# mozack/vdjer

Measured on AMD Instinct MI355X. Metric: M paired-reads/sec (k-mer build + contig score), IgH 50bp PE, higher is better.
Workload: dtype u8/u64 (2-bit packed bases, integer counts)

## Files before the change

### vdjer_amd/csrc/vdjx_kmer.hip

```cpp
#include "vdjx_common.h"
#include "vdjx_scan.h"
#include "vdjx_part.h"

#include <algorithm>
#include <numeric>
#include <type_traits>
#include <string.h>
#include <stdlib.h>

#define HIST_THREADS 512
#define HIST_BLOCKS 512u
#define LOCAL_SLOTS 2048u
#define K3_SUB_TUPLES g_sub_tuples
__device__ u32 g_sub_tuples = 262144u;
#define NONE32 0xFFFFFFFFu
#define INST_MASK 0x7FFFFFFFu

struct RecView {
	u64 bhi, blo, nm, lq;
};

__device__ inline RecView load_rec(const u64* __restrict__ bases, const u64* __restrict__ nmask,
                                   const u64* __restrict__ lowq, size_t r) {
	RecView v;
	const ulonglong2 b = ((const ulonglong2*) bases)[r];
	v.bhi = b.x; v.blo = b.y;
	v.nm = nmask[r];
	v.lq = lowq ? lowq[r] : 0ull;
	return v;
}

__global__ void k_pick_u32(const u32* __restrict__ src, u32 step, u32 n, u32* __restrict__ out) {
	const u32 i = blockIdx.x * blockDim.x + threadIdx.x;
	if (i < n) out[i] = src[(size_t) i * step];
}

template <typename THI, u32 SLOTS>
__device__ inline int lds_insert(u64* s_klo, THI* s_khi, u64 lo, THI hi, u32 h) {
	const THI EMPTY = (THI) ~(THI) 0, LOCKED = (THI) (EMPTY - 1);
	u32 slot = h & (SLOTS - 1);
	u32 probes = 0;
	while (probes < SLOTS) {
		THI cur = vdjx_peek_acquire(&s_khi[slot]);
		if (cur == EMPTY) {
			THI old = atomicCAS(&s_khi[slot], EMPTY, LOCKED);
			if (old == EMPTY) {
				vdjx_poke(&s_klo[slot], lo);
				vdjx_poke_release(&s_khi[slot], hi);
				return (int) slot;
			}
			cur = old;
			if (cur != LOCKED) cur = vdjx_peek_acquire(&s_khi[slot]);
		}
		if (cur == LOCKED) continue;
		if (cur == hi && vdjx_peek(&s_klo[slot]) == lo) return (int) slot;
		slot = (slot + 1) & (SLOTS - 1);
		probes++;
	}
	return -1;
}

template <typename THI, u32 SLOTS>
__device__ inline int lds_lookup(const u64* s_klo, const THI* s_khi, u64 lo, THI hi, u32 h) {
	const THI EMPTY = (THI) ~(THI) 0;
	u32 slot = h & (SLOTS - 1);
	for (u32 probes = 0; probes < SLOTS; probes++) {
		THI cur = s_khi[slot];
		if (cur == EMPTY) return -1;
		if (cur == hi && s_klo[slot] == lo) return (int) slot;
		slot = (slot + 1) & (SLOTS - 1);
	}
	return -1;
}

#define INST_BITS 38
#define INST_MASK64 ((1ull << INST_BITS) - 1ull)
#define NONE64 0xFFFFFFFFFFFFFFFFull

struct Tup16 {
	u64 lo, x;
	typedef u32 hi_t;
	__device__ inline u64 hi() const { return x >> INST_BITS; }
	__device__ inline u64 inst() const { return x & INST_MASK64; }
	__device__ static inline Tup16 make(u64 lo, u64 hi, u64 inst) { Tup16 t; t.lo = lo; t.x = (hi << INST_BITS) | inst; return t; }
	__device__ static inline Tup16 load(const Tup16* p) { const ulonglong2 v = *(const ulonglong2*) p; Tup16 t; t.lo = v.x; t.x = v.y; return t; }
	__device__ static inline void store(Tup16* p, const Tup16& t) { *(ulonglong2*) p = make_ulonglong2(t.lo, t.x); }
};
struct Tup24 {
	u64 lo, h, i;
	typedef u64 hi_t;
	__device__ inline u64 hi() const { return h; }
	__device__ inline u64 inst() const { return i; }
	__device__ static inline Tup24 make(u64 lo, u64 hi, u64 inst) { Tup24 t; t.lo = lo; t.h = hi; t.i = inst; return t; }
	__device__ static inline Tup24 load(const Tup24* p) { return *p; }
	__device__ static inline void store(Tup24* p, const Tup24& t) { *p = t; }
};

__device__ inline u64 vdjx_clean_offsets(u64 bad, int k, int P) {
	u64 inv = bad;
	int cur = 1;
	while (cur * 2 <= k) { inv |= inv >> cur; cur *= 2; }
	inv |= inv >> (k - cur);
	return ~inv & (P >= 64 ? ~0ull : (1ull << P) - 1ull);
}

#define GL_WAVE_BYTES 3072u

#define GL_ROW_LONG (VDJX_LONG_W + 2)
#define GL_WAVE_BYTES_LONG (64u * GL_ROW_LONG * 8u + 2048u)
struct GateView { u64 bhi, blo, bad; };
__device__ inline GateView load_gate(const u64* __restrict__ bases, const u64* __restrict__ gate, size_t r) {
	GateView v;
	const ulonglong2 b = ((const ulonglong2*) bases)[r];
	v.bhi = b.x; v.blo = b.y;
	v.bad = gate[r];
	return v;
}
__device__ inline vdjx_mask3 load_gate3(const u64* __restrict__ gate, size_t r) {
	vdjx_mask3 b;
	b.w0 = gate[r * VDJX_LONG_M]; b.w1 = gate[r * VDJX_LONG_M + 1]; b.w2 = gate[r * VDJX_LONG_M + 2];
	return b;
}
__device__ inline vdjx_mask3 load_bad3(const u64* __restrict__ nmask, const u64* __restrict__ lowq, size_t r) {
	vdjx_mask3 b;
	b.w0 = nmask[r * VDJX_LONG_M] | (lowq ? lowq[r * VDJX_LONG_M] : 0ull);
	b.w1 = nmask[r * VDJX_LONG_M + 1] | (lowq ? lowq[r * VDJX_LONG_M + 1] : 0ull);
	b.w2 = nmask[r * VDJX_LONG_M + 2] | (lowq ? lowq[r * VDJX_LONG_M + 2] : 0ull);
	return b;
}
__device__ inline void stage_row_long(u64* row, const u64* __restrict__ bases, size_t r) {
#pragma unroll
	for (int w = 0; w < VDJX_LONG_W; w++) row[w] = bases[r * VDJX_LONG_W + w];
	row[VDJX_LONG_W] = 0; row[VDJX_LONG_W + 1] = 0;
}

__device__ inline bool sym_canonical(const ulonglong2 f, int rl, int k, int o, u64& khi, u64& klo) {
	u64 xh, xl, yh, yl;
	vdjx_kmer_at_lane(f.x, f.y, rl, k, o, xh, xl);
	vdjx_kmer_rc(xh, xl, k, yh, yl);
	const bool flip = yh < xh || (yh == xh && yl < xl);
	khi = flip ? yh : xh;
	klo = flip ? yl : xl;
	return flip;
}

template <bool LONG, bool SYM = false>
__global__ __launch_bounds__(HIST_THREADS) void k_gated_hist(const u64* __restrict__ bases, const u64* __restrict__ nmask,
                                                             const u64* __restrict__ lowq, size_t R, int rl, int k, u32 nb_bits,
                                                             size_t rpb, u32* __restrict__ bucket_cnt, u32 dbg_in) {
#ifdef VDJX_ABLATE
	const u32 dbg = dbg_in;
#else
	const u32 dbg = 0u;
#endif
	u32 sink = 0;
	extern __shared__ __attribute__((aligned(16))) u32 hist[];
	const u32 NB = 1u << nb_bits;
	for (u32 i = threadIdx.x; i < NB; i += HIST_THREADS) hist[i] = 0;
	__syncthreads();
	static_assert(!(LONG && SYM), "SYM is the short-read form");
	uint8_t* wv = (uint8_t*) (hist + NB) + (threadIdx.x >> 6) * (LONG ? GL_WAVE_BYTES_LONG : GL_WAVE_BYTES);
	ulonglong2* wb = (ulonglong2*) wv;
	u64* wrow = (u64*) wv;
	uint16_t* wl = (uint16_t*) (wv + (LONG ? 64u * GL_ROW_LONG * 8u : 1024u));
	const u32 lane = threadIdx.x & 63u;
	const size_t r0 = (size_t) blockIdx.x * rpb;
	const size_t r1 = r0 + rpb < R ? r0 + rpb : R;
	const int P = rl - k + 1;
	for (size_t rb = r0; rb < r1; rb += HIST_THREADS) {
		const size_t r = rb + threadIdx.x;
		u64 G = 0;
		vdjx_mask3 bad{~0ull, ~0ull, ~0ull};
		if (r < r1) {
			if (LONG) { bad = load_gate3(lowq, r); stage_row_long(wrow + lane * GL_ROW_LONG, bases, r); }
			else {
				const GateView v = load_gate(bases, lowq, SYM ? 2 * r : r);
				G = vdjx_clean_offsets(v.bad, k, P);
				wb[lane] = make_ulonglong2(v.bhi, v.blo);
			}
		}
		constexpr int LSTEP = 16;
		for (int ob = 0; ob < P; ob += LSTEP) {
			const u32 g = LONG ? vdjx_clean16(bad, ob, k, P) : (u32) (G >> ob) & 0xFFFFu;
			const u32 c = (u32) __popc(g);
			const u32 incl = (u32) vdjx_wave_scan_add((int) c);
			const u32 total = (u32) __builtin_amdgcn_readlane((int) incl, 63);
			if (dbg == 1) { sink += incl; continue; }
			if (!total) continue;
			u32 at = incl - c;
			for (u32 gg = g; gg; gg &= gg - 1) wl[at++] = (uint16_t) ((lane << (LONG ? 8 : 6)) | (u32) (ob + __builtin_ctz(gg)));
			vdjx_wave_lds_fence();
			if (dbg == 2) { sink += wl[lane]; vdjx_wave_lds_fence(); continue; }
			for (u32 i = lane; i < total; i += 64) {
				const u32 e = wl[i];
				u64 khi, klo;
				if (LONG) vdjx_kmer_at_words(wrow + (e >> 8) * GL_ROW_LONG, k, (int) (e & 255u), khi, klo);
				else if (SYM) (void) sym_canonical(wb[e >> 6], rl, k, (int) (e & 63u), khi, klo);
				else {
					const ulonglong2 bb = wb[e >> 6];
					vdjx_kmer_at_lane(bb.x, bb.y, rl, k, (int) (e & 63u), khi, klo);
				}
				if (dbg == 3) { sink += (u32) (vdjx_bucket_mix(klo, khi) >> (64 - nb_bits)); continue; }
				atomicAdd(&hist[(u32) (vdjx_bucket_mix(klo, khi) >> (64 - nb_bits))], 1u);
			}
			vdjx_wave_lds_fence();
		}
	}
	__syncthreads();
	if (dbg) { if (sink == 0x12345u) bucket_cnt[0] = sink; return; }
	for (u32 i = threadIdx.x; i < NB; i += HIST_THREADS) if (hist[i]) atomicAdd(&bucket_cnt[i], hist[i]);
}

template <typename TUP> struct TupBucket {
	u32 shift, mask;
	__device__ inline u32 operator()(const TUP& t) const { return (u32) (vdjx_bucket_mix(t.lo, t.hi()) >> shift) & mask; }
};

#define PARTR_STAGE_BYTES 98304u
template <typename TUP, bool LONG, bool SYM = false>
__global__ __launch_bounds__(PART_THREADS) void k_part_records_g(const u64* __restrict__ bases, const u64* __restrict__ nmask,
                                                                 const u64* __restrict__ lowq, size_t R, u64 rec_base, int rl, int k,
                                                                 u32 shift, u32 nbk, size_t rpb, u32 rr0, u32* __restrict__ gcur,
                                                                 TUP* __restrict__ out) {
	extern __shared__ __attribute__((aligned(16))) uint8_t smem[];
	TUP* stage = (TUP*) smem;
	u32* desc = (u32*) (smem + PARTR_STAGE_BYTES);
	__shared__ part_round pr;
	__shared__ u32 s_n;
	constexpr u32 ROUND = PARTR_STAGE_BYTES / sizeof(TUP);
	constexpr int OB = LONG ? 8 : 6;
	const int P = rl - k + 1;
	const u32 rr_min = ROUND / (u32) P;
	u32 rr = rr0 > rr_min ? rr0 : rr_min;
	const u32 mask = nbk - 1;
	const u32 lane = threadIdx.x & 63u, wave = threadIdx.x >> 6;
	static_assert(!(LONG && SYM), "SYM is the short-read form");
	uint8_t* wv = smem + wave * (LONG ? GL_WAVE_BYTES_LONG : GL_WAVE_BYTES);
	ulonglong2* wb = (ulonglong2*) wv;
	u64* wrow = (u64*) wv;
	uint16_t* wl = (uint16_t*) (wv + (LONG ? 64u * GL_ROW_LONG * 8u : 1024u));
	const size_t r0 = (size_t) blockIdx.x * rpb;
	const size_t r1 = r0 + rpb < R ? r0 + rpb : R;
	size_t rs = r0;
	while (rs < r1) {
		const size_t re = rs + rr < r1 ? rs + rr : r1;
		if (threadIdx.x == 0) s_n = 0;
		pr.begin(nbk);
		for (size_t rb = rs; rb < re; rb += PART_THREADS) {
			const size_t r = rb + threadIdx.x;
			u64 G = 0;
			vdjx_mask3 bad{~0ull, ~0ull, ~0ull};
			if (r < re) {
				if (LONG) { bad = load_gate3(lowq, r); stage_row_long(wrow + lane * GL_ROW_LONG, bases, r); }
				else {
					const GateView v = load_gate(bases, lowq, SYM ? 2 * r : r);
					G = vdjx_clean_offsets(v.bad, k, P);
					wb[lane] = make_ulonglong2(v.bhi, v.blo);
				}
			}
			const u32 loc0 = (u32) (rb - rs) + wave * 64u;
			constexpr int LSTEP = 16;
			for (int ob = 0; ob < P; ob += LSTEP) {
				const u32 g = LONG ? vdjx_clean16(bad, ob, k, P) : (u32) (G >> ob) & 0xFFFFu;
				const u32 c = (u32) __popc(g);
				const u32 incl = (u32) vdjx_wave_scan_add((int) c);
				const u32 total = (u32) __builtin_amdgcn_readlane((int) incl, 63);
				if (!total) continue;
				u32 at = incl - c;
				for (u32 gg = g; gg; gg &= gg - 1) wl[at++] = (uint16_t) ((lane << OB) | (u32) (ob + __builtin_ctz(gg)));
				vdjx_wave_lds_fence();
				u32 dbase = 0;
				if (lane == 0) dbase = atomicAdd(&s_n, total);
				dbase = (u32) __builtin_amdgcn_readlane((int) dbase, 0);
				for (u32 i = lane; i < total; i += 64) {
					const u32 e = wl[i];
					u64 khi, klo;
					if (LONG) vdjx_kmer_at_words(wrow + (e >> 8) * GL_ROW_LONG, k, (int) (e & 255u), khi, klo);
					else if (SYM) (void) sym_canonical(wb[e >> 6], rl, k, (int) (e & 63u), khi, klo);
					else {
						const ulonglong2 bb = wb[e >> 6];
						vdjx_kmer_at_lane(bb.x, bb.y, rl, k, (int) (e & 63u), khi, klo);
					}
					const u32 b = (u32) (vdjx_bucket_mix(klo, khi) >> shift) & mask;
					pr.count(b);
					if (dbase + i < ROUND) desc[dbase + i] = ((loc0 + (e >> OB)) << (OB + 10)) | ((e & ((1u << OB) - 1u)) << 10) | b;
				}
				vdjx_wave_lds_fence();
			}
		}
		__syncthreads();
		if (s_n > ROUND) {
			rr = rr / 2 > rr_min ? rr / 2 : rr_min;
			__syncthreads();
			continue;
		}
		const u32 n = pr.reserve(nbk, gcur);
		for (u32 i = threadIdx.x; i < n; i += PART_THREADS) {
			const u32 d = desc[i];
			const size_t r = rs + (d >> (OB + 10));
			const u32 o = (d >> 10) & ((1u << OB) - 1u);
			u64 khi, klo;
			u64 inst = ((rec_base + (u64) r) << OB) | (u64) o;
			if (LONG) vdjx_kmer_at_words(bases + r * VDJX_LONG_W, k, (int) o, khi, klo);
			else if (SYM) {
				const bool flip = sym_canonical(((const ulonglong2*) bases)[2 * r], rl, k, (int) o, khi, klo);
				inst = flip ? ((rec_base + 2 * (u64) r + 1) << OB) | (u64) (rl - k - (int) o) : ((rec_base + 2 * (u64) r) << OB) | (u64) o;
			} else {
				const ulonglong2 bb = ((const ulonglong2*) bases)[r];
				vdjx_kmer_at_lane(bb.x, bb.y, rl, k, (int) o, khi, klo);
			}
			TUP::store(&stage[pr.slot(d & 1023u)], TUP::make(klo, khi, inst));
		}
		__syncthreads();
		pr.flush(stage, n, out, TupBucket<TUP>{shift, mask});
		rs = re;
	}
}

template <typename TUP>
__global__ __launch_bounds__(512) void k_seg_hist_g(const TUP* __restrict__ in, const u32* __restrict__ seg_start, u32 seg_shift, u32 slices,
                                                    u32 shift, u32 sub_bits, u32* __restrict__ fine_cnt) {
	__shared__ u32 h[PART_MAXB];
	const u32 nbk = 1u << sub_bits;
	for (u32 i = threadIdx.x; i < nbk; i += 512) h[i] = 0;
	__syncthreads();
	size_t t0, t1;
	const u32 seg = part_slice(seg_start, seg_shift, slices, t0, t1);
	for (size_t t = t0 + threadIdx.x; t < t1; t += 512) {
		const TUP x = TUP::load(&in[t]);
		atomicAdd(&h[(u32) (vdjx_bucket_mix(x.lo, x.hi()) >> shift) & (nbk - 1)], 1u);
	}
	__syncthreads();
	for (u32 i = threadIdx.x; i < nbk; i += 512) if (h[i]) atomicAdd(&fine_cnt[((size_t) seg << sub_bits) | i], h[i]);
}

#ifndef RD_THREADS
#define RD_THREADS 768
// ... 535 lines not shown
	__shared__ u32 s_over, s_ndist, s_total, s_ns, s_np, s_sbase, s_pbase;
	__shared__ u32 s_pend[MERGE_SLOTS / 32];
	const THI EMPTY = (THI) ~(THI) 0;
	const u32 b = blockIdx.x;
	const u32 tid = threadIdx.x;
	if (tid == 0) {
		u32 tot = 0;
		for (u32 s = 0; s < G; s++) tot += seg_off[(size_t) s * (NBo + 1) + (b + 1) * MG] - seg_off[(size_t) s * (NBo + 1) + b * MG];
		s_total = tot;
	}
	__syncthreads();
	const u32 total = s_total;
	if (total == 0) return;
	u32 S = 1;
	while ((u64) S * (MERGE_SLOTS * 3 / 4) < total) S <<= 1;
	S *= s_mult;
	if (SYM && S > PS_MAX_SPLIT) { if (tid == 0) atomicAdd(g_err, 1u); return; }
	auto key_of = [&](u32 at, u64& lo, u64& hi, u32& h) {
		if (SYM) { const PartialS q = ((const PartialS*) recv)[at]; lo = q.lo; hi = ps_hi(q); h = ps_h(q); }
		else { const Partial q = recv[at]; lo = q.lo; hi = q.hi; h = q.h; }
	};
	{
		if (tid == 0) { s_over = 0; s_ndist = 0; }
		for (u32 sp = 0; sp < S; sp++) {
			for (u32 i = tid; i < MERGE_SLOTS; i += MERGE_THREADS) { s_khi[i] = EMPTY; s_cg[i] = 0; s_mg[i] = NONE64; s_st[i] = 0; if (SYM) s_mgr[i] = NONE64; }
			__syncthreads();
			for (u32 s = 0; s < G; s++) {
				const u32 off = seg_off[(size_t) s * (NBo + 1) + b * MG], cnt = seg_off[(size_t) s * (NBo + 1) + (b + 1) * MG] - off;
				for (u32 i = tid; i < cnt; i += MERGE_THREADS) {
					u64 lo, hi, fg, fgr = 0;
					u32 h, cg;
					if (SYM) { const PartialS q = ((const PartialS*) recv)[off + i]; lo = q.lo; hi = ps_hi(q); h = ps_h(q); cg = ps_cg(q); fg = ps_fg(q); fgr = q.fgr; }
					else { const Partial q = recv[off + i]; lo = q.lo; hi = q.hi; h = q.h; cg = q.cg; fg = q.fg; }
					if (((h >> 12) & (S - 1)) != sp) continue;
					const int slot = lds_insert<THI, MERGE_SLOTS>(s_klo, s_khi, lo, (THI) hi, h);
					if (slot < 0) { s_over = 1; continue; }
					atomicAdd(&s_cg[slot], cg & ~PART_FLAG);
					atomicMin((unsigned long long*) &s_mg[slot], (unsigned long long) fg);
					if (SYM) atomicMin((unsigned long long*) &s_mgr[slot], (unsigned long long) fgr);
					atomicAdd(&s_st[slot], 1u | ((cg & PART_FLAG) ? MS_FLAG : 0u));
				}
			}
			__syncthreads();
			if (s_over) break;
			if (tid == 0) { s_ns = 0; s_np = 0; }
			for (u32 i = tid; i < MERGE_SLOTS / 32; i += MERGE_THREADS) s_pend[i] = 0;
			__syncthreads();
			for (u32 i0 = 0; i0 < MERGE_SLOTS; i0 += MERGE_THREADS) {
				const u32 i = i0 + tid;
				u32 need = 0, cg = 0;
				bool live = s_khi[i] != EMPTY;
				if (live) {
					cg = s_cg[i];
					atomicAdd(&s_ndist, SYM ? 2u : 1u);
					if (cg < cmin) live = false;
				}
				const u32 st0 = s_st[i];
				if (live && !(st0 >> 16)) {
					if ((st0 & 0xFFFFu) < 2) live = false;
					else need |= NEED_SEQ;
				}
				if (live && cg < tlow) need |= NEED_Q;
				if (live && !need) s_st[i] = atomicAdd(&s_ns, SYM ? 2u : 1u);
				else s_st[i] = NONE32;
				if (live && need) {
					s_st[i] = atomicAdd(&s_np, 1u) | (need << 30);
					const u32 hm = rd_hash(s_klo[i], (u64) s_khi[i]) & (MERGE_SLOTS - 1);
					atomicOr(&s_pend[hm >> 5], 1u << (hm & 31));
				}
			}
			__syncthreads();
			if (tid == 0) {
				s_sbase = s_ns ? atomicAdd(so.n, s_ns) : 0;
				s_pbase = s_np ? atomicAdd(po.n, s_np) : 0;
			}
			__syncthreads();
			for (u32 i0 = 0; i0 < MERGE_SLOTS; i0 += MERGE_THREADS) {
				const u32 i = i0 + tid;
				const u32 st = s_st[i];
				if (st != NONE32 && !(st >> 30)) {
					const u32 pos = s_sbase + st;
					if (pos < so.cap) {
						const u32 cg = s_cg[i];
						so.lo[pos] = s_klo[i]; so.hi[pos] = (u64) s_khi[i];
						so.gcnt[pos] = cg > CNT_CAP ? CNT_CAP : cg; so.gfirst[pos] = s_mg[i];
					}
					if (SYM && pos + 1 < so.cap) {
						const u32 cg = s_cg[i];
						u64 rh, rlo;
						vdjx_kmer_rc((u64) s_khi[i], s_klo[i], k, rh, rlo);
						so.lo[pos + 1] = rlo; so.hi[pos + 1] = rh;
						so.gcnt[pos + 1] = cg > CNT_CAP ? CNT_CAP : cg; so.gfirst[pos + 1] = s_mgr[i];
					}
				} else if (st != NONE32) {
					const u32 need = st >> 30;
					const u32 pid = s_pbase + (st & PID_MASK);
					if (pid < po.cap) {
						po.lo[pid] = s_klo[i]; po.hi[pid] = (u64) s_khi[i];
						po.cg[pid] = s_cg[i]; po.mg[pid] = s_mg[i];
						if (SYM) po.mgr[pid] = s_mgr[i];
						po.need[pid] = need;
					}
					s_st[i] = pid | (need << 30);
				}
			}
			__syncthreads();
			for (u32 s = 0; s < G; s++) {
				const u32 off = seg_off[(size_t) s * (NBo + 1) + b * MG], cnt = seg_off[(size_t) s * (NBo + 1) + (b + 1) * MG] - off;
				if (tid == 0) s_ns = 0;
				__syncthreads();
				u32 mine = 0;
				for (u32 i = tid; i < cnt; i += MERGE_THREADS) {
					u64 lo, hi;
					u32 h;
					key_of(off + i, lo, hi, h);
					if (((h >> 12) & (S - 1)) != sp) continue;
					if (!((s_pend[(h & (MERGE_SLOTS - 1)) >> 5] >> (h & 31)) & 1u)) continue;
					const int slot = lds_lookup<THI, MERGE_SLOTS>(s_klo, s_khi, lo, (THI) hi, h);
					if (slot >= 0 && ms_open(s_st[slot])) mine++;
				}
				if (mine) atomicAdd(&s_ns, mine);
				__syncthreads();
				if (tid == 0) { s_sbase = s_ns ? atomicAdd(&g_nq[s], s_ns) : 0; s_np = 0; }
				__syncthreads();
				if (s_ns) {
					for (u32 i = tid; i < cnt; i += MERGE_THREADS) {
						u64 lo, hi;
						u32 h;
						key_of(off + i, lo, hi, h);
						if (((h >> 12) & (S - 1)) != sp) continue;
						if (!((s_pend[(h & (MERGE_SLOTS - 1)) >> 5] >> (h & 31)) & 1u)) continue;
						const int slot = lds_lookup<THI, MERGE_SLOTS>(s_klo, s_khi, lo, (THI) hi, h);
						if (slot < 0) continue;
						const u32 pid = s_st[slot];
						if (ms_open(pid)) queries[src_base[s] + s_sbase + atomicAdd(&s_np, 1u)] = make_uint2(off + i - src_base[s], pid);
					}
				}
				__syncthreads();
			}
			__syncthreads();
		}
		if (s_over && tid == 0) atomicAdd(g_err, 1u);
	}
	if (tid == 0) atomicAdd(g_distinct, (u64) s_ndist);
}

#define REPLY_Q0 80
#define REPLY_R0 240
#define REPLY_RQ0 248
template <bool SYM>
__global__ __launch_bounds__(64) void k_shard_reply(const uint2* __restrict__ queries, u32 nq, const u32* __restrict__ owner_off, u32 G,
                                                    const Partial* __restrict__ dense, const u32* __restrict__ dense_ref,
                                                    const u32* __restrict__ dstart, u32 NBo, const u64* __restrict__ low_inst,
                                                    const u64* __restrict__ bases, const u64* __restrict__ nmask,
                                                    vdjx_qrows quals, u64 rec_base, const u32* __restrict__ scan, u32 n_local, int k, int rl, int ob,
                                                    uint8_t* __restrict__ replies) {
	const u32 qi = blockIdx.x;
	if (qi >= nq) return;
	const u32 lane = threadIdx.x;
	u32 o = 0;
	while (o + 1 < G && owner_off[o + 1] <= qi) o++;
	const uint2 q = queries[qi];
	const u32 di = dstart[(size_t) o * NBo] + q.x;
	u64 finst, finst_r = 0;
	u32 p_cg;
	if (SYM) { const PartialS p = ((const PartialS*) dense)[di]; finst = ps_fg(p); finst_r = p.fgr; p_cg = ps_cg(p); }
	else { const Partial p = dense[di]; finst = p.fg; p_cg = p.cg; }
	const u32 need = q.y >> 30;
	const u32 om = (1u << ob) - 1u;
	auto local_rec = [&](u64 inst) -> u64 {
		if (!scan) return (inst >> ob) - rec_base;
		const u32 g = (u32) (inst >> ob);
		u32 lo = 0, hi = n_local;
		while (lo + 1 < hi) { const u32 mid = lo + ((hi - lo) >> 1); if (scan[mid] <= g) lo = mid; else hi = mid; }
		return lo;
	};
	const u64 frec = local_rec(finst);
	const u32 foff = (u32) finst & om;
	const u64 finst_local = (frec << ob) | foff;
	const u64 frec_r = SYM ? local_rec(finst_r) : 0;
	const u32 foff_r = (u32) finst_r & om;
	const u64 finst_r_local = (frec_r << ob) | foff_r;
	uint8_t* out = replies + (size_t) qi * REPLY_BYTES;
	if (lane == 0) {
		((u32*) out)[0] = q.y;
		((u32*) out)[1] = 0;
		((u64*) out)[1] = finst;
		if (SYM) ((u64*) out)[REPLY_R0 / 8] = finst_r;
	}
	if (!SYM && lane < (REPLY_BYTES - REPLY_R0) / 4) ((u32*) (out + REPLY_R0))[lane] = 0;
	if (lane < 8) {
		const int W = rl <= VDJX_SHORT_READ_LEN ? 2 : VDJX_LONG_W, M = rl <= VDJX_SHORT_READ_LEN ? 1 : VDJX_LONG_M;
		((u64*) out)[2 + lane] = (int) lane < W ? bases[frec * W + lane] : ((int) lane < W + M ? nmask[frec * M + (lane - W)] : 0ull);
	}
	if ((int) lane >= k) return;
	u32 acc = 0, acc_r = 0;
	const u32 ref = dense_ref[di];
	if ((need & NEED_Q) && ref != NONE32) {
		const u32 cg = p_cg & ~PART_FLAG;
		for (u32 i = 0; i < cg; i++) {
			const u64 inst = low_inst[ref + i];
			if (inst != (scan ? finst_local : finst)) acc += (u32) (uint8_t) (quals.row((inst >> ob) - rec_base)[((u32) inst & om) + lane] - 33);
			if (SYM) {
				const u64 m = vdjx_inst_mirror(inst, ob, rl, k);
				if (m != (scan ? finst_r_local : finst_r)) acc_r += (u32) (uint8_t) (quals.row((m >> ob) - rec_base)[((u32) m & om) + lane] - 33);
			}
		}
	}
	const uint8_t* fr = quals.row(frec);
	out[REPLY_Q0 + lane] = (uint8_t) (acc > 255u ? 255u : acc);
	out[REPLY_Q0 + REPLY_KQ + lane] = (uint8_t) (fr[foff + lane] - 33);
	out[REPLY_Q0 + 2 * REPLY_KQ + lane] = (uint8_t) (fr[lane] - 33);
	if (SYM) {
		const uint8_t* frr = quals.row(frec_r);
		out[REPLY_RQ0 + lane] = (uint8_t) (acc_r > 255u ? 255u : acc_r);
		out[REPLY_RQ0 + REPLY_KQ + lane] = (uint8_t) (frr[foff_r + lane] - 33);
		out[REPLY_RQ0 + 2 * REPLY_KQ + lane] = (uint8_t) (frr[lane] - 33);
	}
}

__global__ void k_resolve_first(const uint8_t* __restrict__ replies, u32 nr, const u64* __restrict__ p_mg, u32* __restrict__ p_r0,
                                const u64* __restrict__ p_mgr, u32 np) {
	const u32 r = blockIdx.x * blockDim.x + threadIdx.x;
	if (r >= nr) return;
	const uint8_t* me = replies + (size_t) r * REPLY_BYTES;
	const u32 pid = ((const u32*) me)[0] & PID_MASK;
	if (((const u64*) me)[1] == p_mg[pid]) p_r0[pid] = r;
	if (p_mgr && ((const u64*) me)[REPLY_R0 / 8] == p_mgr[pid]) p_r0[np + pid] = r;
}

__global__ __launch_bounds__(256) void k_resolve_add(const uint8_t* __restrict__ replies, u32 nr, const u32* __restrict__ p_r0, int k, u32* __restrict__ p_fl,
                                                     u32* __restrict__ p_S, u32 np) {
	const u32 r = blockIdx.x * 4u + (threadIdx.x >> 6);
	const u32 lane = threadIdx.x & 63u;
	if (r >= nr) return;
	const uint8_t* me = replies + (size_t) r * REPLY_BYTES;
	const u32 w0 = ((const u32*) me)[0];
	const u32 pid = w0 & PID_MASK, need = w0 >> 30;
	const u32 r0 = p_r0[pid];
	if (r0 == NONE32) return;
	if ((need & NEED_SEQ) && r != r0 && lane == 0) {
		const u64* a = (const u64*) me;
		const u64* b = (const u64*) (replies + (size_t) r0 * REPLY_BYTES);
		u64 d = 0;
#pragma unroll
		for (int w = 2; w < 10; w++) d |= a[w] ^ b[w];
		if (d) p_fl[pid] = 1;
	}
	if ((need & NEED_Q) && (int) lane < k) {
		const uint8_t* first = me + REPLY_Q0 + (r == r0 ? 2 * REPLY_KQ : REPLY_KQ);
		atomicAdd(&p_S[(size_t) pid * 64 + lane], (u32) me[REPLY_Q0 + lane] + (u32) first[lane]);
		if (np) {
			const uint8_t* first_r = me + REPLY_RQ0 + (r == p_r0[np + pid] ? 2 * REPLY_KQ : REPLY_KQ);
			atomicAdd(&p_S[((size_t) np + pid) * 64 + lane], (u32) me[REPLY_RQ0 + lane] + (u32) first_r[lane]);
		}
	}
}

template <bool SYM>
__global__ void k_resolve_keep(PendOut po, u32 np, const u32* __restrict__ p_fl, const u32* __restrict__ p_S, int k, u32 mf, u32 mqq, u32 tlow,
                               SurvOutG so) {
	const u32 p = blockIdx.x * blockDim.x + threadIdx.x;
	const bool in = p < np;
	const u32 need = in ? po.need[p] : 0u;
	bool keep = in && ((need & NEED_SEQ) ? p_fl[p] != 0 : true);
	const u32 cg = in ? po.cg[p] : 0u;
	const u32 cgc = cg > CNT_CAP ? CNT_CAP : cg;
	keep = keep && cgc >= mf;
	bool keep_r = keep;
	if (keep && cg < tlow) {
		for (int j = 0; j < k; j++) if (p_S[(size_t) p * 64 + j] < mqq) { keep = false; break; }
		if (SYM) for (int j = 0; j < k; j++) if (p_S[((size_t) np + p) * 64 + j] < mqq) { keep_r = false; break; }
	}
	if (!SYM) {
		const u32 pos = vdjx_wave_inc(so.n, keep);
		if (keep && pos < so.cap) {
			so.lo[pos] = po.lo[p]; so.hi[pos] = po.hi[p];
			so.gcnt[pos] = cgc; so.gfirst[pos] = po.mg[p];
		}
		return;
	}
	const bool any = keep || keep_r;
	const u32 pos = vdjx_wave_inc(so.n, any, 2u);
	if (any && pos + 1 < so.cap) {
		so.lo[pos] = po.lo[p]; so.hi[pos] = po.hi[p];
		so.gcnt[pos] = cgc | (keep ? 0u : GC_SHADOW); so.gfirst[pos] = po.mg[p];
		u64 rh, rlo;
		vdjx_kmer_rc(po.hi[p], po.lo[p], k, rh, rlo);
		so.lo[pos + 1] = rlo; so.hi[pos + 1] = rh;
		so.gcnt[pos + 1] = cgc | (keep_r ? 0u : GC_SHADOW); so.gfirst[pos + 1] = po.mgr[p];
	}
}

__global__ void k_first_to_scan(u64* __restrict__ a, size_t na, u64* __restrict__ b, size_t nb, const u32* __restrict__ scan, int ob) {
	const size_t i = (size_t) blockIdx.x * blockDim.x + threadIdx.x;
	if (i >= na + nb) return;
	u64* p = i < na ? a + i : b + (i - na);
	const u64 v = *p;
	if (v != NONE64) *p = ((u64) scan[v >> ob] << ob) | (v & ((1ull << ob) - 1ull));
}

__global__ void k_node_flags(const u64* __restrict__ s_lo, const u64* __restrict__ s_hi, u32 n, int k,
                             const u32* __restrict__ vbits, const u32* __restrict__ jbits,
                             uint8_t* __restrict__ has_v, uint8_t* __restrict__ has_j) {
	u32 i = blockIdx.x * blockDim.x + threadIdx.x;
	if (i >= n) return;
	if (k <= 16) { has_v[i] = 1; has_j[i] = 1; return; }
	u128 key = ((u128) s_hi[i] << 64) | s_lo[i];
	u32 code = (u32) (key >> (2 * (k - 16)));
	has_v[i] = code ? (vbits[code >> 5] >> (code & 31)) & 1u : 0;
	has_j[i] = code ? (jbits[code >> 5] >> (code & 31)) & 1u : 0;
}


#define IT_INST_BITS 35
#define IT_INST_MASK ((1ull << IT_INST_BITS) - 1ull)
#define IT_SURV_SHIFT 38
#define IT_HOLE 0xFFFFFFFFFFFFFFFFull
#define WALK_THREADS 256

#define SLOT_HI_BITS 36
#define SLOT_HI_MASK ((1ull << SLOT_HI_BITS) - 1ull)
struct SurvTable { const ulonglong2* slots; u32 mask; const ulonglong2* skey; const u32* bloom; u32 bloom_mask; };

struct ItemFmt {
	u32 pmask;
	u32 len_shift;
	u32 maxlen;
	u32 mul, inv;
	u32 bmask;
	u32 ns;
};
__device__ inline u32 it_surv(const ItemFmt& f, u64 x) { return (u32) (x >> IT_SURV_SHIFT) & f.pmask; }
__device__ inline u32 it_len(const ItemFmt& f, u64 x) { return f.maxlen > 1 ? (u32) (x >> f.len_shift) + 1u : 1u; }
__device__ inline u32 it_scat(const ItemFmt& f, u32 p) { return ((((p >> 4) * f.mul) & f.bmask) << 4) | (p & 15u); }

__global__ void k_surv_table2(const u64* __restrict__ s_lo, const u64* __restrict__ s_hi, u32 n, ulonglong2* __restrict__ slots, u32 mask,
                              ulonglong2* __restrict__ skey, u32* __restrict__ bloom, u32 bloom_mask) {
	const u32 i = blockIdx.x * blockDim.x + threadIdx.x;
	if (i >= n) return;
	const u64 lo = s_lo[i], hi = s_hi[i];
	skey[i] = make_ulonglong2(lo, hi);
	const u64 h = vdjx_mix(lo, hi);
	{
		const u32 bit = (u32) (h >> 40) & bloom_mask;
		atomicOr(&bloom[bit >> 5], 1u << (bit & 31));
	}
	u32 slot = (u32) (h >> 20) & mask;
	const unsigned long long entry = hi | ((unsigned long long) (i + 1) << SLOT_HI_BITS);
	while (atomicCAS((unsigned long long*) &slots[slot].y, 0ull, entry) != 0ull) slot = (slot + 1) & mask;
	slots[slot].x = lo;
}

__device__ inline int surv_lookup2f(const SurvTable& t, u64 lo, u64 hi);

__device__ inline int surv_lookup2(const SurvTable& t, u64 lo, u64 hi) {
	u32 slot = (u32) (vdjx_mix(lo, hi) >> 20) & t.mask;
	for (;;) {
		const ulonglong2 v = t.slots[slot];
		if (!v.y) return -1;
		if (v.x == lo && (v.y & SLOT_HI_MASK) == hi) return (int) (v.y >> SLOT_HI_BITS) - 1;
		slot = (slot + 1) & t.mask;
	}
}

__device__ inline int surv_lookup2f(const SurvTable& t, u64 lo, u64 hi) {
	const u64 h = vdjx_mix(lo, hi);
	const u32 bit = (u32) (h >> 40) & t.bloom_mask;
	if (!((t.bloom[bit >> 5] >> (bit & 31)) & 1u)) return -1;
	return surv_lookup2(t, lo, hi);
}

__global__ void k_succ_links2(SurvTable t, u32 n, int k, const u32* __restrict__ gcnt, u32* __restrict__ succ, unsigned long long* __restrict__ pred,
                              u32* __restrict__ bestsucc) {
	const u32 u = blockIdx.x * blockDim.x + threadIdx.x;
	if (u >= n) return;
	const ulonglong2 kk = t.skey[u];
	const u128 base = (((u128) kk.y << 64) | kk.x) << 2;
	const u128 km = k < 64 ? (((u128) 1) << (2 * k)) - 1 : ~(u128) 0;
	const int sh = 2 * (k - 1);
	const u32 fb = (u32) (sh < 64 ? kk.x >> sh : kk.y >> (sh - 64)) & 3u;
	const unsigned long long mine = ((unsigned long long) (gcnt[u] & GC_MASK) << 32) | ((unsigned long long) (fb ^ 1u) << 30) | (unsigned long long) u;
	u32 best = NONE32, best_g = 0;
	for (u32 b = 0; b < 4; b++) {
		const u128 key = (base | (u128) b) & km;
		const int s = surv_lookup2(t, (u64) key, (u64) (key >> 64));
		succ[u * 4 + b] = s >= 0 ? (u32) s : NONE32;
		if (s >= 0 && (u32) s != u) {
			const u32 g = gcnt[s] & GC_MASK;
			if (best == NONE32 || g >= best_g) { best = (u32) s; best_g = g; }
			atomicMax(&pred[s], mine);
		}
	}
	bestsucc[u] = best;
}

#define CHAIN_JUMPS 31
__global__ void k_chain_init(const unsigned long long* __restrict__ pred, const u32* __restrict__ bestsucc, u32 n, u64* __restrict__ pd) {
	const u32 v = blockIdx.x * blockDim.x + threadIdx.x;
	if (v >= n) return;
	const unsigned long long x = pred[v];
	const u32 u = (u32) x & 0x3FFFFFFFu;
	pd[v] = x != 0ull && bestsucc[u] == v ? ((u64) u << 32) | 1ull : ((u64) NONE32 << 32);
}

__global__ void k_partner(SurvTable t, u32 n, int k, u32* __restrict__ partner) {
	const u32 p = blockIdx.x * blockDim.x + threadIdx.x;
	if (p >= n) return;
	const ulonglong2 kk = t.skey[p];
	u64 rh, rlo;
	vdjx_kmer_rc(kk.y, kk.x, k, rh, rlo);
	const int q = surv_lookup2(t, rlo, rh);
	partner[p] = q >= 0 ? (u32) q : NONE32;
}
__global__ void k_partner_check(const u32* __restrict__ partner, const u64* __restrict__ linw, u32 n, u32* __restrict__ bad) {
	const u32 p = blockIdx.x * blockDim.x + threadIdx.x;
	if (p >= n) return;
	bool wrong = partner[p] == NONE32;
	const bool linked = (linw[p >> 4] >> (15u - (p & 15u))) & 1ull;
	if (!wrong && linked && (p + 1 >= n || partner[p + 1] != partner[p] - 1u)) wrong = true;
	const u64 m = __ballot(wrong);
	if (m && __lane_id() == 0) atomicAdd(bad, (u32) __popcll(m));
}

__global__ void k_chain_jump(u64* __restrict__ pd, u32 n, const u32* __restrict__ open_prev, u32* __restrict__ open_now) {
	if (open_prev && *open_prev == 0) return;
	const u32 v = blockIdx.x * blockDim.x + threadIdx.x;
	bool open = false;
	if (v < n) {
		u64 x = __atomic_load_n(&pd[v], __ATOMIC_RELAXED);
		for (int it = 0; it < CHAIN_JUMPS; it++) {
			const u32 p = (u32) (x >> 32);
			if (p == NONE32) break;
			const u64 y = __atomic_load_n(&pd[p], __ATOMIC_RELAXED);
			const u32 pp = (u32) (y >> 32);
			if (pp == NONE32) break;
			x = ((u64) pp << 32) | (u64) ((u32) x + (u32) y);
			__atomic_store_n(&pd[v], x, __ATOMIC_RELAXED);
			open = true;
		}
	}
	if (__ballot(open) && __lane_id() == 0) atomicAdd(open_now, 1u);
}

__device__ inline void chain_of(const u64* pd, u32 v, u32& head, u32& dist) {
	const u64 x = pd[v];
	const u32 p = (u32) (x >> 32);
	head = v; dist = 0;
	if (p == NONE32) return;
	if ((u32) (pd[p] >> 32) != NONE32) return;
	head = p; dist = (u32) x;
}
__global__ void k_chain_len(const u64* __restrict__ pd, u32 n, u32* __restrict__ len) {
	const u32 v = blockIdx.x * blockDim.x + threadIdx.x;
	if (v >= n) return;
	u32 h, d;
	chain_of(pd, v, h, d);
	atomicAdd(&len[h], 1u);
}

__global__ void k_chain_place(const u64* __restrict__ pd, const u32* __restrict__ off, u32 n, u32* __restrict__ newidx) {
	const u32 v = blockIdx.x * blockDim.x + threadIdx.x;
	if (v >= n) return;
	u32 h, d;
	chain_of(pd, v, h, d);
	newidx[v] = off[h] + d;
}
__global__ void k_chain_permute(const u32* __restrict__ newidx, u32 n, const u64* __restrict__ lo, const u64* __restrict__ hi, const u32* __restrict__ gcnt,
                                const u64* __restrict__ gfirst, const u32* __restrict__ succ, u64* __restrict__ lo2, u64* __restrict__ hi2,
                                u32* __restrict__ gcnt2, u64* __restrict__ gfirst2, ulonglong2* __restrict__ skey2, u32* __restrict__ succ2) {
	const u32 v = blockIdx.x * blockDim.x + threadIdx.x;
	if (v >= n) return;
	const u32 q = newidx[v];
	const u64 l = lo[v], h = hi[v];
	lo2[q] = l; hi2[q] = h; gcnt2[q] = gcnt[v]; gfirst2[q] = gfirst[v];
	skey2[q] = make_ulonglong2(l, h);
	const uint4 s = *(const uint4*) &succ[(size_t) v * 4];
	uint4 r;
	r.x = s.x == NONE32 ? NONE32 : newidx[s.x];
	r.y = s.y == NONE32 ? NONE32 : newidx[s.y];
	r.z = s.z == NONE32 ? NONE32 : newidx[s.z];
	r.w = s.w == NONE32 ? NONE32 : newidx[s.w];
	*(uint4*) &succ2[(size_t) q * 4] = r;
}
__global__ void k_table_remap(ulonglong2* __restrict__ slots, u32 n_slots, const u32* __restrict__ newidx) {
	const u32 i = blockIdx.x * blockDim.x + threadIdx.x;
	if (i >= n_slots) return;
	const u64 y = slots[i].y;
	if (!y) return;
	slots[i].y = (y & SLOT_HI_MASK) | ((u64) (newidx[(u32) (y >> SLOT_HI_BITS) - 1] + 1u) << SLOT_HI_BITS);
}

__global__ void k_chain_words(const u32* __restrict__ succ, const ulonglong2* __restrict__ skey, u32 n, int k, u64* __restrict__ linw, u32* __restrict__ fbw,
                              const u32* __restrict__ partner) {
	const u32 p = blockIdx.x * blockDim.x + threadIdx.x;
	const u32 j = p & 15u;
	u64 w = 0;
	u32 fb = 0;
	if (p < n) {
		const uint4 s = *(const uint4*) &succ[(size_t) p * 4];
		const u32 sv[4] = {s.x, s.y, s.z, s.w};
		const bool mirrored = !partner || (p + 1 < n && partner[p] != NONE32 && partner[p + 1] == partner[p] - 1u);
		for (u32 b = 0; b < 4; b++) if (sv[b] != NONE32) {
			if (sv[b] == p + 1 && mirrored) w |= (1ull << (15u - j)) | ((u64) b << (32u + 2u * (15u - j)));
			else w |= 1ull << (31u - j);
		}
		const ulonglong2 kk = skey[p];
		const int sh = 2 * (k - 1);
		fb = (u32) (sh < 64 ? kk.x >> sh : kk.y >> (sh - 64)) & 3u;
	}
	u32 fw = fb << (2 * j);
	for (int d = 1; d < 16; d <<= 1) {
		w |= ((u64) (u32) __shfl_xor((int) (w >> 32), d) << 32) | (u32) __shfl_xor((int) (u32) w, d);
		fw |= (u32) __shfl_xor((int) fw, d);
	}
	if (j == 0 && p < n) { linw[p >> 4] = w; fbw[p >> 4] = fw; }
}

struct WalkRecS {
	u64 bhi, blo; int rl;
	__device__ inline void kmer_u(int k, int o, u64& hi, u64& lo) const { vdjx_kmer_at(bhi, blo, rl, k, o, hi, lo); }
	__device__ inline void kmer_l(int k, int o, u64& hi, u64& lo) const { vdjx_kmer_at_lane(bhi, blo, rl, k, o, hi, lo); }
	__device__ inline u32 bases16(int bi) const {
		const int sh = 2 * (rl - 16 - bi);
		const u32 rw_dn = vdjx_bits_at_lane(bhi, blo, (u32) (sh > 0 ? sh : 0));
		const u32 up = (u32) (sh < 0 ? -sh : 0);
		return (rw_dn << (up & 31u)) & (0u - (u32) (up < 32u));
	}
	__device__ inline u32 base(int i) const { return vdjx_base_at_lane(bhi, blo, rl, i); }
};
struct WalkRecL {
	const u64* row;
	__device__ inline void kmer_u(int k, int o, u64& hi, u64& lo) const { vdjx_kmer_at_words(row, k, o, hi, lo); }
	__device__ inline void kmer_l(int k, int o, u64& hi, u64& lo) const { vdjx_kmer_at_words(row, k, o, hi, lo); }
	__device__ inline u32 bases16(int bi) const { return vdjx_bases16_words(row, bi); }
	__device__ inline u32 base(int i) const { return vdjx_base_words(row, i); }
};
__device__ inline bool wm_test(u64 m, int i) { return (m >> i) & 1ull; }
__device__ inline bool wm_test(const vdjx_mask3& m, int i) { return m.test(i); }
__device__ inline void wm_set(u64& m, int i) { m |= 1ull << i; }
__device__ inline void wm_set(vdjx_mask3& m, int i) { m.set(i); }
__device__ inline int wm_next(u64 m, int from, int none) { const u64 x = from < 64 ? m & (~0ull << from) : 0ull; return x ? __builtin_ctzll(x) : none; }
__device__ inline int wm_next(const vdjx_mask3& m, int from, int none) { return m.next(from, none); }
__device__ inline u32 wm_slice32(u64 m, int from) { return from < 64 ? (u32) (m >> from) : 0u; }
__device__ inline u32 wm_slice32(const vdjx_mask3& m, int from) { return (u32) m.slice(from); }

template <bool LONG, bool SYM = false>
__global__ __launch_bounds__(WALK_THREADS) void k_walk_items(const u64* __restrict__ bases, const u64* __restrict__ nmask, size_t R, int rl, int ob_bits, int k,
                                                             SurvTable t, const u32* __restrict__ succ, const u64* __restrict__ linw, ItemFmt f,
                                                             u32 range_shift, u32 n_ranges,
                                                             u64* __restrict__ raw, u64 raw_cap, u32 blk_items,
                                                             unsigned long long* __restrict__ g_cursor,
                                                             u32* __restrict__ range_cnt, u32* __restrict__ g_err, u32 dbg_in,
                                                             const u32* __restrict__ partner) {
	static_assert(!(LONG && SYM), "SYM is the short-read form");
#ifdef VDJX_ABLATE
	const u32 dbg = dbg_in;
#else
	(void) dbg_in;
	constexpr u32 dbg = 0u;
#endif
	extern __shared__ u32 hist[];
	typedef typename std::conditional<LONG, vdjx_mask3, u64>::type MaskT;
	typedef typename std::conditional<LONG, WalkRecL, WalkRecS>::type RecT;
	for (u32 i = threadIdx.x; i < n_ranges; i += WALK_THREADS) hist[i] = 0;
	__syncthreads();
	u64* myrow = (u64*) (hist + ((n_ranges + 1u) & ~1u)) + threadIdx.x * GL_ROW_LONG;
	const int P = rl - k + 1;
	const size_t per = ((R + gridDim.x - 1) / gridDim.x + WALK_THREADS - 1) / WALK_THREADS * WALK_THREADS;
	const size_t r0 = (size_t) blockIdx.x * per;
	const size_t r1 = r0 + per < R ? r0 + per : R;
	const int lane = __lane_id();
	u64 blk = 0;
	u32 fill = blk_items;
#ifdef WALK_STATS
	u32 st_rows = 0, st_rounds = 0, st_filter = 0, st_lookup = 0, st_items = 0, st_chain = 0;
#define WST(x) x
#else
#define WST(x)
#endif
	bool have_blk = false, dead = false;
	__shared__ u64 dq[WALK_THREADS / 64][128];
	__shared__ ulonglong2 dq_b[LONG ? 1 : WALK_THREADS / 64][LONG ? 1 : 128];
	__shared__ u64 dq_v[LONG ? 1 : WALK_THREADS / 64][LONG ? 1 : 128];
	const u32 wq = threadIdx.x >> 6;
	u32 qn = 0;
	auto walk_row = [&](auto fresh_tag, const size_t r, const bool live, const int o_from, const ulonglong2 qb, const u64 qv) {
		constexpr bool FRESH = decltype(fresh_tag)::value;
		RecT v;
		MaskT V{};
		if constexpr (LONG) {
			v.row = myrow;
			if (live) {
				stage_row_long(myrow, bases, r);
				const vdjx_mask3 nm = load_bad3(nmask, nullptr, r);
				for (int o16 = 0; o16 < P; o16 += 16) {
					const u64 g = (u64) vdjx_clean16(nm, o16, k, P) << (o16 & 63);
					if ((o16 >> 6) == 0) V.w0 |= g; else if ((o16 >> 6) == 1) V.w1 |= g; else V.w2 |= g;
				}
			} else
				for (int w = 0; w < GL_ROW_LONG; w++) myrow[w] = 0;
		} else {
			v.bhi = v.blo = 0; v.rl = rl;
			if (!FRESH) { if (live) { v.bhi = qb.x; v.blo = qb.y; V = qv; } }
			else if (live) {
				const RecView rv = load_rec(bases, nmask, nullptr, r);
				v.bhi = rv.bhi; v.blo = rv.blo;
				u64 inv = rv.nm;
				int cur = 1;
				while (cur * 2 <= k) { inv |= inv >> cur; cur *= 2; }
				inv |= inv >> (k - cur);
				V = ~inv & (P >= 64 ? ~0ull : (1ull << P) - 1ull);
			}
		}
		int o = wm_next(V, o_from, P);
		int s = -1;
		u32 in = 0;
		bool first = FRESH, have_c = false;
		MaskT C{};
		WST(st_rows++;)
		while (__ballot(o < P)) {
			WST(st_rounds++;)
			bool need = o < P && s < 0;
			if (FRESH) {
				const bool later = need && !first;
				const u64 lm = __ballot(later);
				if (lm) {
					if (later) {
						const u32 qi = qn + (u32) __popcll(lm & ((1ull << lane) - 1ull));
						dq[wq][qi] = ((u64) r << 8) | (u64) (u32) o;
						if constexpr (!LONG) { dq_b[wq][qi] = make_ulonglong2(v.bhi, v.blo); dq_v[wq][qi] = V; }
						o = P; need = false;
					}
					qn += (u32) __popcll(lm);
				}
			}
			WST(if (__ballot(need)) st_lookup++;)
			if (!FRESH && __ballot(need && !first && !have_c)) {
				WST(st_filter++;)
				const bool mine = need && !first && !have_c;
				for (int ob = 0; ob < P; ob += 4) {
					u32 wv[4], bt[4];
#pragma unroll
					for (int j = 0; j < 4; j++) {
						const int oo = ob + j;
						wv[j] = 0; bt[j] = 0;
						if (mine && oo >= o && oo < P && wm_test(V, oo)) {
							u64 khi, klo;
							v.kmer_u(k, oo, khi, klo);
							const u32 bit = (u32) (vdjx_mix(klo, khi) >> 40) & t.bloom_mask;
							bt[j] = bit & 31u;
							wv[j] = (dbg & 8u) ? 0xFFFFFFFFu : t.bloom[bit >> 5];
						}
					}
#pragma unroll
					for (int j = 0; j < 4; j++) if ((wv[j] >> bt[j]) & 1u) wm_set(C, ob + j);
				}
				if (mine) have_c = true;
			}
			if (need) {
				bool filtered = false;
				if (!first) {
					o = wm_next(C, o, P);
					filtered = true;
				}
				first = false;
				if (o < P) {
					u64 khi, klo;
					v.kmer_l(k, o, khi, klo);
					if (dbg & 8u) s = (klo & 3u) ? (int) ((u32) vdjx_mix(klo, khi) % f.ns) : -1;
					else s = (filtered || (dbg & 16u)) ? surv_lookup2(t, klo, khi) : surv_lookup2f(t, klo, khi);
					in = 0;
					if (s < 0) o++;
				}
			}
			const bool act = o < P && s >= 0;
			WST(if (__ballot(act)) st_chain++;)
			u32 rem = 0, pp = 0, po = 0;
			if (act) {
				const u32 a = (u32) s & 15u;
				const u64 w0 = linw[(u32) s >> 4], w1 = linw[((u32) s >> 4) + 1];
				const u32 lw = (((((u32) w0 & 0xFFFFu) << 16) | ((u32) w1 & 0xFFFFu)) << a) >> 16;
				const u32 ow = ((((u32) w0 & 0xFFFF0000u) | ((u32) w1 >> 16)) << a) >> 16;
				const u32 bw = (u32) (((((w0 >> 32) << 32) | (w1 >> 32)) << (2 * a)) >> 32);
				const u32 rw = v.bases16(o + k);
				const u32 x = bw ^ rw;
				const u32 nl = ~lw & 0xFFFFu;
				const u32 m_base = x ? (u32) __builtin_clz(x) >> 1 : 16u;
				const u32 m_lin = nl ? (u32) __builtin_clz(nl) - 16u : 16u;
				const u32 nv = ~wm_slice32(V, o + 1);
				const u32 m_valid = nv ? (u32) __builtin_ctz(nv) : 32u;
				u32 steps = m_base < m_lin ? m_base : m_lin;
				steps = steps < m_valid ? steps : m_valid;
				const bool capped = steps >= 16u;
				if (capped) steps = 15u;
				rem = steps + 1u; pp = (u32) s; po = (u32) o;
				const int o2 = o + (int) rem;
				int s2 = -1;
				if (o2 < P && wm_test(V, o2)) {
					if (capped) s2 = s + 16;
					else if ((ow >> (15u - steps)) & 1u) {
						const u32 bb = v.base(o2 + k - 1);
						const u32 nx = succ[((u32) s + steps) * 4u + bb];
						s2 = nx == NONE32 ? -1 : (int) nx;
					}
				}
				o = s2 >= 0 || o2 >= P ? o2 : o2 + 1;
				s = s2;
			}
			const u32 pin0 = in;
			if (act) in = s >= 0 ? (4u | v.base(o - 1)) : 0u;
			const u32 run_len = rem, run_pp = pp, run_po = po;
			u32 q_last = 0;
			if (SYM && act) q_last = partner[run_pp];
			auto emit = [&](auto mir_tag, u32 rem_, u32 pp_, u32 po_, u32 pin_, const size_t rec_) {
				constexpr bool MIR = decltype(mir_tag)::value;
				while (__ballot(rem_ > 0)) {
					WST(st_items++;)
					const bool close = rem_ > 0;
					u32 len = 16u - (pp_ & 15u);
					len = len < rem_ ? len : rem_;
					len = len < f.maxlen ? len : f.maxlen;
					const u64 item = (f.maxlen > 1 ? (u64) (len - 1) << f.len_shift : 0ull) | ((u64) pp_ << IT_SURV_SHIFT) | ((u64) pin_ << 35) | ((u64) rec_ << ob_bits) | (u64) po_;
					const u64 m = __ballot(close);
					const u32 cnt = (u32) __popcll(m);
					if (fill + cnt > blk_items) {
						if (have_blk) for (u32 i = fill + (u32) lane; i < blk_items; i += 64) raw[blk + i] = IT_HOLE;
						unsigned long long nb = 0;
						if (lane == 0) nb = atomicAdd(g_cursor, (unsigned long long) blk_items);
						nb = ((unsigned long long) (u32) __builtin_amdgcn_readlane((int) (nb >> 32), 0) << 32) | (u32) __builtin_amdgcn_readlane((int) nb, 0);
						if (nb + blk_items > raw_cap) { if (lane == 0 && !dead) atomicAdd(g_err, 1u); dead = true; have_blk = false; }
						else { blk = nb; have_blk = true; }
						fill = 0;
					}
					if (close && !dead) {
						if (!(dbg & 1u)) raw[blk + fill + (u32) __popcll(m & ((1ull << lane) - 1ull))] = item;
						if (!(dbg & 2u)) atomicAdd(&hist[it_scat(f, pp_) >> range_shift], 1u);
					}
					fill += cnt;
					if (close) {
						rem_ -= len; pp_ += len; po_ += len;
						pin_ = 4u | (MIR ? (v.base(rl - (int) po_) ^ 1u) : v.base((int) po_ - 1));
					}
				}
			};
			emit(std::false_type{}, rem, pp, po, pin0, r);
			if constexpr (SYM) {
				u32 mrem = 0, mpp = 0, mpo = 0, mpin = 0;
				if (act) {
					if (q_last == NONE32 || q_last + 1u < run_len) { if (!dead) atomicAdd(g_err + 2, 1u); }
					else {
						mrem = run_len; mpp = q_last - (run_len - 1u);
						mpo = (u32) (rl - k) - (run_po + run_len - 1u);
						mpin = s >= 0 ? (4u | (v.base(rl - (int) mpo) ^ 1u)) : 0u;
					}
				}
				emit(std::true_type{}, mrem, mpp, mpo, mpin, r + 1);
			}
		}
	};
	auto walk_queued = [&](u32 take) {
		vdjx_wave_lds_fence();
		const bool live = (u32) lane < take;
		const u64 e = live ? dq[wq][qn - take + (u32) lane] : 0ull;
		ulonglong2 qb = make_ulonglong2(0ull, 0ull);
		u64 qv = 0;
		if constexpr (!LONG) if (live) { qb = dq_b[wq][qn - take + (u32) lane]; qv = dq_v[wq][qn - take + (u32) lane]; }
		vdjx_wave_lds_fence();
		qn -= take;
		walk_row(std::false_type{}, (size_t) (e >> 8), live, (int) (e & 255u), qb, qv);
	};
	for (size_t rb = r0; rb < r1; rb += WALK_THREADS) {
		const size_t r = rb + threadIdx.x;
		walk_row(std::true_type{}, SYM ? 2 * r : r, r < r1, 0, make_ulonglong2(0ull, 0ull), 0ull);
		while (qn >= 64) walk_queued(64);
	}
	if (qn) walk_queued(qn);
	if (have_blk) for (u32 i = fill + (u32) lane; i < blk_items; i += 64) raw[blk + i] = IT_HOLE;
#ifdef WALK_STATS
	if ((dbg & 32u) && lane == 0) {
		atomicAdd(&g_cursor[1], (unsigned long long) st_rows); atomicAdd(&g_cursor[2], (unsigned long long) st_rounds); atomicAdd(&g_cursor[3], (unsigned long long) st_filter);
		atomicAdd(&g_cursor[4], (unsigned long long) st_lookup); atomicAdd(&g_cursor[5], (unsigned long long) st_chain); atomicAdd(&g_cursor[6], (unsigned long long) st_items);
	}
#endif
	__syncthreads();
	for (u32 i = threadIdx.x; i < n_ranges; i += WALK_THREADS) if (hist[i]) atomicAdd(&range_cnt[i], hist[i]);
}

static_assert(IT_HOLE == PART_HOLE, "the holes of the walk's blocks are what the partition drops");
struct ItemRange {
	ItemFmt f;
	u32 range_shift, mask;
	__device__ inline u32 operator()(u64 x) const { return (it_scat(f, it_surv(f, x)) >> range_shift) & mask; }
};

#define RC_THREADS 1024
#define RC_UNR 4
template <typename IT> struct RcNone;
template <> struct RcNone<u32> { static constexpr u32 v = 0xFFFFFFFFu; };
template <> struct RcNone<u64> { static constexpr u64 v = 0xFFFFFFFFFFFFFFFFull; };
__device__ inline void rc_min(u32* p, u32 v) { atomicMin(p, v); }
__device__ inline void rc_min(u64* p, u64 v) { atomicMin((unsigned long long*) p, (unsigned long long) v); }

#define RC_CS 17u
#define RC_MS 77u
__device__ inline u32 rc_win(u32 k, u32 s) { return 31u + ((0x261B0E00u >> (8u * k)) & 0xFFu) + s - 1u; }
template <u32 SB, typename IT>
__global__ __launch_bounds__(RC_THREADS) void k_recount(const u64* __restrict__ items, const u32* __restrict__ range_start, ItemFmt f, u32 ns, u64 rec_base, int ob,
                                                        const u32* __restrict__ fbw, u32* __restrict__ ucnt, u64* __restrict__ ufirst, u64* __restrict__ in_first,
                                                        unsigned long long* __restrict__ n_inst) {
	__shared__ u32 c[SB / 16 * RC_CS];
	__shared__ IT mv[SB / 16 * RC_MS];
	__shared__ IT ef[SB * 4];
	__shared__ u32 fbl[SB / 16];
	__shared__ unsigned long long tot;
	constexpr IT NONE = RcNone<IT>::v;
	const u32 b = blockIdx.x;
	const u32 s0 = b * SB;
	const u32 nb = (ns + 15u) >> 4;
	for (u32 i = threadIdx.x; i < SB / 16 * RC_CS; i += RC_THREADS) c[i] = 0;
	for (u32 i = threadIdx.x; i < SB / 16 * RC_MS; i += RC_THREADS) mv[i] = NONE;
	for (u32 i = threadIdx.x; i < SB * 4; i += RC_THREADS) ef[i] = NONE;
	for (u32 i = threadIdx.x; i < SB / 16; i += RC_THREADS) {
		const u32 sb = (s0 >> 4) + i;
		const u32 blk = (sb * f.inv) & f.bmask;
		fbl[i] = sb <= f.bmask && blk < nb ? fbw[blk] : 0u;
	}
	if (threadIdx.x == 0) tot = 0;
	__syncthreads();
	const u32 i0 = range_start[b], i1 = range_start[b + 1];
	const u32 iend = i0 + (i1 - i0 + RC_THREADS * RC_UNR - 1) / (RC_THREADS * RC_UNR) * (RC_THREADS * RC_UNR);
	for (u32 ib = i0 + threadIdx.x; ib < iend; ib += RC_THREADS * RC_UNR) {
		u64 xs[RC_UNR];
#pragma unroll
		for (int u = 0; u < RC_UNR; u++) { const u32 i = ib + (u32) u * RC_THREADS; xs[u] = i < i1 ? items[i] : IT_HOLE; }
#pragma unroll
		for (int u = 0; u < RC_UNR; u++) {
			const u64 x = xs[u];
			const bool live = x != IT_HOLE;
			const u32 p = it_surv(f, x);
			const u32 len = live ? it_len(f, x) : 1u;
			const u32 sl = live ? it_scat(f, p) - s0 : 0u;
			const u32 a = sl & 15u, e = a + len - 1u;
			const u64 inst = x & IT_INST_MASK;
			const bool shaped = live && (a == 0u || e == 15u);
			const u32 cb = (sl >> 4) * RC_CS, mb = (sl >> 4) * RC_MS;
			const u32 slot = mb + (a == 0u ? e : 15u + a);
			const IT val = (IT) (inst + 15u - a);
			bool mine = shaped;
			const u64 act = __ballot(shaped);
			if (act) {
				const int leader = __ffsll((long long) act) - 1;
				const u32 lslot = (u32) __builtin_amdgcn_readlane((int) slot, leader);
				const bool same = shaped && slot == lslot;
				const u64 m = __ballot(same);
				if (__popcll(m) >= 8) {
					const u64 v64 = inst + 15u - a;
					const u32 hi_min = vdjx_wave_min(same ? (u32) (v64 >> 32) : 0xFFFFFFFFu);
					const u32 lo_min = vdjx_wave_min(same && (u32) (v64 >> 32) == hi_min ? (u32) v64 : 0xFFFFFFFFu);
					if (__lane_id() == leader) {
						const u32 n = (u32) __popcll(m);
						atomicAdd(&c[cb + e], n);
						if (a) atomicAdd(&c[cb + a - 1u], 0u - n);
						rc_min(&mv[lslot], (IT) (((u64) hi_min << 32) | lo_min));
					}
					mine = shaped && !same;
				}
			}
			if (live && (mine || !shaped)) {
				atomicAdd(&c[cb + e], 1u);
				if (a) atomicAdd(&c[cb + a - 1u], 0xFFFFFFFFu);
			}
			if (mine) rc_min(&mv[slot], val);
			if (live && !shaped) {
				const u32 k = 31u - (u32) __builtin_clz(len), w = 1u << k;
				rc_min(&mv[mb + rc_win(k, a)], val);
				if (len != w) rc_min(&mv[mb + rc_win(k, e + 1u - w)], val);
			}
			if (live && ((x >> 37) & 1ull)) {
				IT* ep = &ef[sl * 4 + (u32) ((x >> 35) & 3ull)];
				if (vdjx_peek(ep) > (IT) inst) rc_min(ep, (IT) inst);
			}
		}
	}
	__syncthreads();
	const u64 add = rec_base << ob;
	u32 my_cnt = 0;
	for (u32 i = threadIdx.x; i < SB; i += RC_THREADS) {
		const u32 sb = (s0 + i) >> 4;
		const u32 blk = (sb * f.inv) & f.bmask;
		const u32 x = i & 15u, p = (blk << 4) | x;
		if (sb > f.bmask || blk >= nb || p >= ns) continue;
		const u32 cbase = (i >> 4) * RC_CS, mbase = (i >> 4) * RC_MS;
		u32 cc = 0;
		IT mm = NONE;
		IT me = NONE;
		for (u32 e = x; e < 16; e++) { cc += c[cbase + e]; const IT t = mv[mbase + e]; mm = t < mm ? t : mm; if (x) me = t < me ? t : me; }
		for (u32 a = 1; a <= x; a++) { const IT t = mv[mbase + 15 + a]; mm = t < mm ? t : mm; if (a < x) me = t < me ? t : me; }
#pragma unroll
		for (u32 k = 0; k < 4; k++) {
			const u32 w = 1u << k;
			const u32 lo = x >= w ? x - w + 1u : 1u, hi = x < 15u - w ? x : 15u - w;
			for (u32 s = lo ? lo : 1u; s <= hi; s++) { const IT t = mv[mbase + rc_win(k, s)]; mm = t < mm ? t : mm; if (s < x) me = t < me ? t : me; }
		}
		my_cnt += cc;
		ucnt[p] = cc;
		ufirst[p] = mm == NONE ? NONE64 : (u64) mm - 15u + x + add;
		IT e4[4] = {ef[i * 4], ef[i * 4 + 1], ef[i * 4 + 2], ef[i * 4 + 3]};
		if (x && me != NONE) {
			const u32 pa = (fbl[i >> 4] >> (2 * (x - 1))) & 3u;
			const IT t = (IT) (me - 15u + x);
			if (t < e4[pa]) e4[pa] = t;
		}
		for (u32 q = 0; q < 4; q++) in_first[(size_t) p * 4 + q] = e4[q] == NONE ? NONE64 : (u64) e4[q] + add;
	}
	if (my_cnt) atomicAdd(&tot, (unsigned long long) my_cnt);
	__syncthreads();
	if (threadIdx.x == 0 && tot) atomicAdd(n_inst, tot);
}

__global__ void k_count_unseen(const u64* __restrict__ ufirst, u32 n, u32* __restrict__ out) {
	const u32 i = blockIdx.x * blockDim.x + threadIdx.x;
	const bool un = i < n && ufirst[i] == NONE64;
	const u64 m = __ballot(un);
	if (m && __lane_id() == 0) atomicAdd(out, (u32) __popcll(m));
}

__global__ void k_edges_from_in(SurvTable t, u32 n, int k, const u64* __restrict__ in_first, u32* __restrict__ in_from,
                                u64* __restrict__ edge_first, u32* __restrict__ edge_to) {
	const u32 e = blockIdx.x * blockDim.x + threadIdx.x;
	if (e >= n * 4u) return;
	const u64 fs = in_first[e];
	if (fs == NONE64) { in_from[e] = NONE32; return; }
	const u32 v = e >> 2, a = e & 3u;
	const ulonglong2 kk = t.skey[v];
	const u128 kv = ((u128) kk.y << 64) | kk.x;
	const u128 ku = (kv >> 2) | ((u128) a << (2 * (k - 1)));
	const int u = surv_lookup2(t, (u64) ku, (u64) (ku >> 64));
	in_from[e] = u >= 0 ? (u32) u : NONE32;
	if (u >= 0) {
		const u32 oe = (u32) u * 4u + ((u32) kk.x & 3u);
		edge_first[oe] = fs;
		edge_to[oe] = v;
	}
}

struct SurvRec { u64 lo, hi; u32 gcnt, pad; u64 gfirst; };

__global__ void k_surv_pack(const u64* __restrict__ lo, const u64* __restrict__ hi, const u32* __restrict__ gcnt,
                            const u64* __restrict__ gfirst, u32 n, SurvRec* __restrict__ out) {
	u32 i = blockIdx.x * blockDim.x + threadIdx.x;
	if (i >= n) return;
	SurvRec r{lo[i], hi[i], gcnt[i], 0u, gfirst[i]};
	out[i] = r;
}

__global__ void k_surv_unpack(const SurvRec* __restrict__ in, u32 n, u64* __restrict__ lo, u64* __restrict__ hi, u32* __restrict__ gcnt,
                              u64* __restrict__ gfirst, u32* __restrict__ n_real) {
	u32 i = blockIdx.x * blockDim.x + threadIdx.x;
	const bool in_range = i < n;
	SurvRec r{0, 0, GC_SHADOW, 0, 0};
	if (in_range) {
		r = in[i];
		lo[i] = r.lo; hi[i] = r.hi; gcnt[i] = r.gcnt; gfirst[i] = r.gfirst;
	}
	(void) vdjx_wave_inc(n_real, in_range && !(r.gcnt & GC_SHADOW));
}

struct NodeOut {
	u64* first_inst; u32* gcnt; u32* freq; uint8_t* hv; uint8_t* hj; u64* klo; u64* khi; char* kmers;
	uint8_t* to_deg; u32* to_ids; uint8_t* from_deg; u32* from_ids;
};

__global__ void k_rank_keys(const u64* __restrict__ ufirst, const u32* __restrict__ gcnt, u32 n, u64* __restrict__ key, u32* __restrict__ idx) {
	const u32 i = blockIdx.x * blockDim.x + threadIdx.x;
	if (i < n) { key[i] = (gcnt[i] & GC_SHADOW) ? NONE64 : ufirst[i]; idx[i] = i; }
}
__global__ void k_rank_scatter(const u64* __restrict__ key, const u32* __restrict__ idx, u32 n, u32* __restrict__ rank) {
	const u32 j = blockIdx.x * blockDim.x + threadIdx.x;
	if (j >= n) return;
	const u32 i = idx[j];
	rank[i] = key[j] == NONE64 ? i : j;
}

__global__ __launch_bounds__(256) void k_root_count(const uint8_t* __restrict__ from_deg, u32 n, u32* __restrict__ block_cnt) {
	__shared__ u32 cnt;
	if (threadIdx.x == 0) cnt = 0;
	__syncthreads();
	const u32 i = blockIdx.x * 256 + threadIdx.x;
	const bool r = i < n && from_deg[i] == 0;
	const u64 b = __ballot(r);
	if ((threadIdx.x & 63) == 0 && b) atomicAdd(&cnt, (u32) __popcll(b));
	__syncthreads();
	if (threadIdx.x == 0) block_cnt[blockIdx.x] = cnt;
}

__global__ __launch_bounds__(256) void k_root_list(const uint8_t* __restrict__ from_deg, u32 n, const u32* __restrict__ block_start,
                                                   u32* __restrict__ roots) {
	__shared__ u32 wave_cnt[4];
	const u32 i = blockIdx.x * 256 + threadIdx.x;
	const bool r = i < n && from_deg[i] == 0;
	const u64 b = __ballot(r);
	const u32 w = threadIdx.x >> 6, lane = threadIdx.x & 63;
	if (lane == 0) wave_cnt[w] = (u32) __popcll(b);
	__syncthreads();
	u32 base = block_start[blockIdx.x];
	for (u32 j = 0; j < w; j++) base += wave_cnt[j];
	if (r) roots[base + (u32) __popcll(b & ((1ull << lane) - 1))] = i;
}

__device__ inline void sort4_desc64(u64 (&f)[4], u32 (&id)[4]) {
#define CSW(a, b) { const bool sw = kk[a] < kk[b]; if (sw) { u64 t = kk[a]; kk[a] = kk[b]; kk[b] = t; u32 u = id[a]; id[a] = id[b]; id[b] = u; } }
	u64 kk[4];
	for (int i = 0; i < 4; i++) kk[i] = f[i] == NONE64 ? 0ull : f[i] + 1;
	CSW(0, 1) CSW(2, 3) CSW(0, 2) CSW(1, 3) CSW(1, 2)
	for (int i = 0; i < 4; i++) f[i] = kk[i] ? kk[i] - 1 : NONE64;
#undef CSW
}

__global__ void k_node_emit2(const u64* __restrict__ s_lo, const u64* __restrict__ s_hi, const u32* __restrict__ s_gcnt,
                             const u32* __restrict__ s_ucnt, const u64* __restrict__ s_ufirst, const uint8_t* __restrict__ hv,
                             const uint8_t* __restrict__ hj, const u32* __restrict__ rank, const u64* __restrict__ edge_first,
                             const u32* __restrict__ edge_to, const u64* __restrict__ in_first, const u32* __restrict__ in_from,
                             u32 n, int k, NodeOut o) {
	const u32 s = blockIdx.x * blockDim.x + threadIdx.x;
	if (s >= n) return;
	if (s_gcnt[s] & GC_SHADOW) return;
	const u32 r = rank[s];
	o.first_inst[r] = s_ufirst[s];
	o.gcnt[r] = s_gcnt[s];
	o.freq[r] = s_ucnt[s] > 32765u ? 32765u : s_ucnt[s];
	o.hv[r] = hv[s];
	o.hj[r] = hj[s];
	const u128 key = ((u128) s_hi[s] << 64) | s_lo[s];
	for (int j = 0; j < k; j++) {
		const u32 b = (u32) (key >> (2 * (k - 1 - j))) & 3u;
		o.kmers[(size_t) r * k + j] = b == 0 ? 'A' : (b == 1 ? 'T' : (b == 2 ? 'C' : 'G'));
	}
	u64 f[4];
	u32 id[4];
	for (int e = 0; e < 4; e++) {
		f[e] = edge_first[(size_t) s * 4 + e];
		if (f[e] != NONE64 && (s_gcnt[edge_to[(size_t) s * 4 + e]] & GC_SHADOW)) f[e] = NONE64;
		id[e] = f[e] != NONE64 ? rank[edge_to[(size_t) s * 4 + e]] + 1 : 0;
	}
	sort4_desc64(f, id);
	u32 deg = 0;
	for (int e = 0; e < 4; e++) { o.to_ids[(size_t) r * 4 + e] = f[e] != NONE64 ? id[e] : 0; deg += f[e] != NONE64; }
	o.to_deg[r] = (uint8_t) deg;
	for (int e = 0; e < 4; e++) {
		f[e] = in_first[(size_t) s * 4 + e];
		if (f[e] != NONE64 && (in_from[(size_t) s * 4 + e] == NONE32 || (s_gcnt[in_from[(size_t) s * 4 + e]] & GC_SHADOW))) f[e] = NONE64;
		id[e] = f[e] != NONE64 ? rank[in_from[(size_t) s * 4 + e]] + 1 : 0;
	}
	sort4_desc64(f, id);
	deg = 0;
	for (int e = 0; e < 4; e++) { o.from_ids[(size_t) r * 4 + e] = f[e] != NONE64 ? id[e] : 0; deg += f[e] != NONE64; }
	o.from_deg[r] = (uint8_t) deg;
}

namespace {

struct PersistAlloc {
	vdjx_ctx* c;
	explicit PersistAlloc(vdjx_ctx* ctx) : c(ctx) {}
	template <typename T> hipError_t alloc(T** out, size_t n) {
		*out = (T*) c->shard_arena.alloc((n ? n : 1) * sizeof(T));
		return *out ? hipSuccess : hipErrorOutOfMemory;
	}
	vdjx_arena::mark_t mark() const { return c->shard_arena.mark(); }
	void release_to(vdjx_arena::mark_t m) { c->shard_arena.release_to(m); }
};

struct PoolView { const u64* bases; const u64* nmask; vdjx_qrows quals; int rl; int ob; };

template <typename TUP> struct GTuples {
	TUP* t = nullptr;
	u32* bucket_start = nullptr;
	u32 NB = 0, N = 0;
};

struct SurvivorsG {
	u64 *lo = nullptr, *hi = nullptr, *gfirst = nullptr, *ufirst = nullptr;
	u32 *gcnt = nullptr, *ucnt = nullptr;
	u32 n = 0, n_real = 0;
	u64 ndist = 0;
};

inline u32 ceil_log2_u64(u64 x) { u32 b = 0; while ((1ull << b) < x) b++; return b; }

static bool sync_debug() { static const bool on = vdjx_env_set("VDJX_SYNC_DEBUG"); return on; }
static void dbg_sync(vdjx_ctx* c, const char* what) {
	if (!sync_debug()) return;
	const hipError_t e = hipStreamSynchronize(c->stream);
	fprintf(stderr, "[vdjx] %s: %s\n", what, hipGetErrorString(e));
}

struct GatedHist { u32 HB = 0, NBH = 0, N = 0; u32* hstart = nullptr; bool sym = false; };
static bool build_sym(const vdjx_pool* pool, int k) {
	return pool->sym && pool->W == 2 && (k & 1) && pool->n_records % 2 == 0;
}
static bool sym_walk_wanted() { static const bool on = !vdjx_env_set("VDJX_NO_SYM_WALK"); return on; }
static size_t gated_bucket_default() { static const size_t v = (size_t) vdjx_env_num("VDJX_GATED_BUCKET", 3072, 1, 1ll << 32); return v; }
template <typename A>
int stage_gated_hist(vdjx_ctx* c, A& db, const vdjx_pool* pool, int k, size_t per_bucket, u64 geometry_instances, GatedHist* gh, bool sym = false) {
	hipStream_t st = c->stream;
	const size_t R = sym ? pool->n_records / 2 : pool->n_records;
	const int P = pool->rl - k + 1;
	const u64 NI = geometry_instances ? geometry_instances : (u64) R * (u64) P;
	const size_t per = per_bucket ? per_bucket : gated_bucket_default();
	const u32 hb_max = pool->W > 2 ? 14u : 15u;
	u32 HB = ceil_log2_u64((NI + per - 1) / per);
	HB = std::max(8u, std::min(hb_max, HB));
	const u32 NBH = 1u << HB;
#ifdef VDJX_ABLATE
	static const u32 hist_dbg = (u32) vdjx_env_num("VDJX_HIST_DBG", 0, 0, 4);
#else
	constexpr u32 hist_dbg = 0;
#endif
	u32 nblk = (u32) std::min<size_t>(HIST_BLOCKS, (R + 4095) / 4096);
	if (nblk == 0) nblk = 1;
	size_t rpb = (R + nblk - 1) / nblk;
	u32 *hcnt, *hstart;
	HIP_TRY(db.alloc(&hcnt, NBH));
	HIP_TRY(db.alloc(&hstart, NBH + 1));
	HIP_TRY(hipMemsetAsync(hcnt, 0, (size_t) NBH * 4, st));
	const bool lng = pool->W > 2;
	const size_t lds_hist = (size_t) NBH * 4 + (HIST_THREADS / 64) * (lng ? GL_WAVE_BYTES_LONG : GL_WAVE_BYTES);
	HIP_TRY(hipFuncSetAttribute((const void*) k_gated_hist<false>, hipFuncAttributeMaxDynamicSharedMemorySize, (int) lds_hist));
	HIP_TRY(hipFuncSetAttribute((const void*) k_gated_hist<true>, hipFuncAttributeMaxDynamicSharedMemorySize, (int) lds_hist));
	HIP_TRY(hipFuncSetAttribute((const void*) k_gated_hist<false, true>, hipFuncAttributeMaxDynamicSharedMemorySize, (int) lds_hist));
	{
		vdjx_prof_scope ps(c, "k_gated_hist");
		if (lng) hipLaunchKernelGGL(k_gated_hist<true>, dim3(nblk), dim3(HIST_THREADS), lds_hist, st, pool->d_bases, pool->d_nmask, pool->d_lowq, R, pool->rl, k, HB, rpb, hcnt, hist_dbg);
		else if (sym) hipLaunchKernelGGL((k_gated_hist<false, true>), dim3(nblk), dim3(HIST_THREADS), lds_hist, st, pool->d_bases, pool->d_nmask, pool->d_lowq, R, pool->rl, k, HB, rpb, hcnt, hist_dbg);
		else hipLaunchKernelGGL(k_gated_hist<false>, dim3(nblk), dim3(HIST_THREADS), lds_hist, st, pool->d_bases, pool->d_nmask, pool->d_lowq, R, pool->rl, k, HB, rpb, hcnt, hist_dbg);
	}
	dbg_sync(c, "k_gated_hist");
	vdjx_scan_one(st, hcnt, NBH, hstart);
	HIP_TRY(hipMemcpyAsync(c->h_pin, hstart + NBH, 4, hipMemcpyDeviceToHost, st));
	HIP_TRY(hipStreamSynchronize(st));
	HIP_TRY(hipGetLastError());
#ifdef VDJX_ABLATE
	if (hist_dbg) return VDJX_ESTATE;
#endif
	const u32 N = *(const u32*) c->h_pin;
	c->stats["gated_instances"] = sym ? 2ull * N : N;
	gh->HB = HB; gh->NBH = NBH; gh->N = N; gh->hstart = hstart; gh->sym = sym;
	return VDJX_OK;
}

template <typename TUP, typename A>
int stage_gated_cut(vdjx_ctx* c, A& db, const vdjx_pool* pool, u64 rec_base, int k, size_t per_bucket, u64 geometry_instances, const GatedHist& gh, GTuples<TUP>* out) {
	hipStream_t st = c->stream;
	const bool sym = gh.sym;
	const size_t R = sym ? pool->n_records / 2 : pool->n_records;
	const int P = pool->rl - k + 1;
	const size_t per = per_bucket ? per_bucket : gated_bucket_default();
	const u32 hb_max = pool->W > 2 ? 14u : 15u;
	const bool lng = pool->W > 2;
	const u32 HB = gh.HB, NBH = gh.NBH, N = gh.N;
	u32* hstart = gh.hstart;
	size_t rpb;
	out->N = N;
	const u64 Ng = geometry_instances ? geometry_instances : (u64) N;
	static const size_t refine = (size_t) vdjx_env_num("VDJX_REFINE_TUPLES", 4096, 1, 1ll << 32);
	u32 T = 8;
	while (T < HB && ((u64) per << T) < Ng) T++;
	u32 extra = 0;
	const size_t refine_at = per_bucket ? std::max<size_t>(per_bucket, refine / 2) : refine;
	if (T == HB && HB == hb_max && Ng / NBH > refine_at) {
		extra = 1;
		while (extra < 5 && (Ng >> extra) / NBH > refine_at) extra++;
	}
	const u32 Tt = T + extra;
	const u32 NBt = 1u << Tt;
	HIP_TRY(db.alloc(&out->t, (size_t) N + 1));
	constexpr u32 stage_tuples = PARTR_STAGE_BYTES / (u32) sizeof(TUP);
	constexpr u32 lds_partr = PARTR_STAGE_BYTES + stage_tuples * 4;
	u32 cbits = Tt, fbits = 0;
	if (Tt > 10) { cbits = extra ? Tt - 10 : 8; fbits = Tt - cbits; }
	const u32 NBc = 1u << cbits;
	u32 nblk2 = (u32) std::min<size_t>(1024, (R + 2047) / 2048);
	if (nblk2 == 0) nblk2 = 1;
	rpb = (R + nblk2 - 1) / nblk2;
	u32* gcur;
	HIP_TRY(db.alloc(&gcur, NBc));
	TUP* l1 = out->t;
	if (fbits) HIP_TRY(db.alloc(&l1, (size_t) N + 1));
	{
		vdjx_prof_scope ps(c, "k_part_records");
		const u64 NIl = (u64) R * (u64) P;
		u64 rr = N ? (u64) stage_tuples * 3 / 4 * NIl / ((u64) N * (u64) P) : 1u << 16;
		rr = std::max<u64>(PART_THREADS, std::min<u64>(rr / PART_THREADS * PART_THREADS, lng ? 1u << 14 : 1u << 16));
		auto* part_records = lng ? k_part_records_g<TUP, true> : sym ? k_part_records_g<TUP, false, true> : k_part_records_g<TUP, false>;
		HIP_TRY(part_launch(st, part_records, nblk2, lds_partr, hstart, NBc, HB - cbits, gcur, l1, pool->d_bases, pool->d_nmask, pool->d_lowq, R, rec_base,
		                    pool->rl, k, 64 - cbits, NBc, rpb, (u32) rr));
	}
	dbg_sync(c, "k_part_records");
	u32* tstart;
	HIP_TRY(db.alloc(&tstart, NBt + 1));
	out->NB = NBt;
	out->bucket_start = tstart;
	constexpr u32 slices = PART_SLICES;
	if (extra) {
		u32* fine_cnt;
		HIP_TRY(db.alloc(&fine_cnt, NBt));
		HIP_TRY(hipMemsetAsync(fine_cnt, 0, (size_t) NBt * 4, st));
		vdjx_prof_scope ps(c, "k_seg_hist");
		hipLaunchKernelGGL(k_seg_hist_g<TUP>, dim3(NBc * slices), dim3(512), 0, st, l1, hstart, HB - cbits, slices, 64 - Tt, fbits, fine_cnt);
		vdjx_scan_one(st, fine_cnt, NBt, tstart);
	} else {
		hipLaunchKernelGGL(k_pick_u32, dim3((NBt + 1 + 255) / 256), dim3(256), 0, st, hstart, 1u << (HB - Tt), NBt + 1, tstart);
	}
	if (fbits) {
		u32* gcur2;
		HIP_TRY(db.alloc(&gcur2, NBt));
		vdjx_prof_scope ps(c, "k_part_tuples");
		HIP_TRY(part_launch(st, k_part<TUP, TupBucket<TUP>, part_segs>, NBc * slices, PART_LDS_BYTES, tstart, NBt, 0u, gcur2, out->t,
		                    l1, part_segs{hstart, HB - cbits, slices, fbits}, TupBucket<TUP>{64 - Tt, (1u << fbits) - 1u}));
	}
	return VDJX_OK;
}

template <typename TUP, typename A>
int stage_gated_partition(vdjx_ctx* c, A& db, const vdjx_pool* pool, u64 rec_base, int k, size_t per_bucket, u64 geometry_instances, GTuples<TUP>* out, bool sym = false) {
	GatedHist gh;
	int rc = stage_gated_hist(c, db, pool, k, per_bucket, geometry_instances, &gh, sym);
	if (rc) return rc;
	return stage_gated_cut<TUP>(c, db, pool, rec_base, k, per_bucket, geometry_instances, gh, out);
}

static int set_sub_tuples(vdjx_ctx* c) {
	static const u32 sub = (u32) vdjx_env_num("VDJX_SUB_TUPLES", 262144, 1, 0xFFFFFFFFll);
	if (c->sub_tuples_set != sub) {
		HIP_TRY(hipMemcpyToSymbolAsync(HIP_SYMBOL(g_sub_tuples), &sub, 4, 0, hipMemcpyHostToDevice, c->stream));
		c->sub_tuples_set = sub;
	}
	return VDJX_OK;
}
template <typename TUP, typename A>
int bucket_order(vdjx_ctx* c, A& db, const GTuples<TUP>& t, u32** order) {
	*order = nullptr;
	if (t.NB < 1024) return VDJX_OK;
	HIP_TRY(db.alloc(order, t.NB));
	hipLaunchKernelGGL(k_bucket_order, dim3(1), dim3(1024), 0, c->stream, t.bucket_start, t.NB, *order);
	return VDJX_OK;
}

template <typename TUP, typename A>
int stage_gated_reduce(vdjx_ctx* c, A& db, const GTuples<TUP>& t, const PoolView& pv, u64 rec_base, int k, int mf, int mq, SurvivorsG* sv, bool sym = false) {
	hipStream_t st = c->stream;
	int rc = set_sub_tuples(c);
	if (rc) return rc;
	if (mq >= 255) mq = 254;
	const u32 mqq = (u32) (mq < 0 ? 0 : (mq > 214 ? 214 : mq));
	const u32 tlow = 1 + (mqq + 19) / 20;
	const u32 cmin = (u32) std::max(mf, 2);
	const u32 mfu = (u32) std::max(mf, 0);
	const u32 cap = (sym ? t.N : t.N / 2) + 16;
	u32 *g_err, *n_surv;
	u64* g_distinct;
	HIP_TRY(db.alloc(&sv->lo, cap)); HIP_TRY(db.alloc(&sv->hi, cap)); HIP_TRY(db.alloc(&sv->gcnt, cap)); HIP_TRY(db.alloc(&sv->gfirst, cap));
	HIP_TRY(db.alloc(&g_distinct, 64 * 16 + 2));
	g_err = (u32*) (g_distinct + 64 * 16);
	n_surv = g_err + 1;
	u32* n_real = g_err + 2;
	HIP_TRY(hipMemsetAsync(g_distinct, 0, (64 * 16 + 2) * 8, st));
	SurvOutG so{sv->lo, sv->hi, sv->gcnt, sv->gfirst, n_surv, cap, n_real};
	static const u32 rd_dbg = (u32) vdjx_env_num("VDJX_RD_DBG", 0, 0, 9);
	if (t.N) {
		vdjx_prof_scope ps(c, "k_gated_reduce");
		u32* order;
		if ((rc = bucket_order(c, db, t, &order))) return rc;
		if (sym) hipLaunchKernelGGL((k_gated_reduce<TUP, true>), dim3(t.NB), dim3(RD_THREADS), 0, st, t.t, t.bucket_start, pv.bases, pv.nmask, pv.quals, pv.rl, pv.ob, k, rec_base,
		                            mfu, cmin, mqq, tlow, so, g_distinct, g_err, rd_dbg, (const u32*) order);
		else hipLaunchKernelGGL(k_gated_reduce<TUP>, dim3(t.NB), dim3(RD_THREADS), 0, st, t.t, t.bucket_start, pv.bases, pv.nmask, pv.quals, pv.rl, pv.ob, k, rec_base,
		                        mfu, cmin, mqq, tlow, so, g_distinct, g_err, rd_dbg, (const u32*) order);
	}
	u64* spread = (u64*) c->h_pin;
	u32* tail = (u32*) (spread + 64 * 16);
	static_assert((64 * 16 + 2) * 8 == VDJX_HPIN_SYNC_BYTES, "h_pin layout (vdjx_common.h)");
	HIP_TRY(hipMemcpyAsync(spread, g_distinct, VDJX_HPIN_SYNC_BYTES, hipMemcpyDeviceToHost, st));
	HIP_TRY(hipStreamSynchronize(st));
	HIP_TRY(hipGetLastError());
	const u32 ns = tail[1], err = tail[0];
	if (err) { vdjx_set_error("k_gated_reduce: %u buckets could not be split to fit LDS", err); return VDJX_EHIP; }
	if (ns > cap) { vdjx_set_error("survivor capacity logic failed (%u > %u)", ns, cap); return VDJX_EHIP; }
	sv->ndist = 0;
	for (int i = 0; i < 64; i++) sv->ndist += spread[i * 16];
	sv->n = ns;
	sv->n_real = sym ? tail[2] : ns;
	c->stats["kmer_build_shadows"] = ns - sv->n_real;
	return VDJX_OK;
}

struct RecountOut { u32* ucnt; u64* ufirst; u64* in_first; u32* in_from; u64* edge_first; u32* edge_to; };
struct RecountStatus { const u32* g_err = nullptr; const u32* n_items = nullptr; const unsigned long long* n_inst = nullptr; u32 ns = 0; };
#define VDJX_ESYMWALK (-1000)
static int recount_status_check(vdjx_ctx* c, const u32* hp, u32 ns) {
	if (hp[6] || hp[7]) { vdjx_set_error("the mirrored walk found %u + %u places where the chains are not mirror images", hp[6], hp[7]); return VDJX_ESYMWALK; }
	if (hp[0]) { vdjx_set_error("k_walk_items: item buffer too small (%u waves stopped)", hp[0]); return VDJX_EHIP; }
	if (hp[1]) { vdjx_set_error("internal error: %u of %u surviving k-mers were not met again in the records (VDJX_SYNC_DEBUG=1 names them)", hp[1], ns); return VDJX_EHIP; }
	c->stats["recount_items"] = hp[2];
	c->stats["recount_instances"] = *(const unsigned long long*) (hp + 4);
	return VDJX_OK;
}

template <typename A>
int stage_recount(vdjx_ctx* c, A& db, const vdjx_pool* pool, u64 rec_base, int k, SurvivorsG& sv, const RecountOut& ro,
                  bool derive_edges, SurvTable* table_out = nullptr, RecountStatus* defer = nullptr, bool sym_walk = false) {
	hipStream_t st = c->stream;
	const size_t R = pool->n_records;
	const int P = pool->rl - k + 1;
	const u32 ns = sv.n;
	if (ns >= (1u << 26)) { vdjx_set_error("more than 2^26 surviving k-mers: not supported by the recount items"); return VDJX_ELIMIT; }
	if (R >= (1ull << 29)) { vdjx_set_error("more than 2^29 records on one GPU: not supported by the recount items"); return VDJX_ELIMIT; }
	if ((u64) R * (u64) P >= (1ull << 32)) { vdjx_set_error("records*offsets = %llu >= 2^32 on one GPU: shard the pool over more GPUs", (unsigned long long) ((u64) R * (u64) P)); return VDJX_ELIMIT; }
	u32 tmask = 1023;
	while ((size_t) tmask + 1 < (size_t) ns * 2) tmask = tmask * 2 + 1;
	unsigned long long* pred;
	ulonglong2* table;
	u32 *succ0, *succ, *bloom, *clen, *coff, *newidx, *jump_open, *fbw, *gcnt2, *bestsucc, *partner = nullptr;
	u64 *pd, *lo2, *hi2, *gfirst2, *linw;
	ulonglong2 *skey0, *skey;
	u32 bloom_bits = 1u << 16;
	while (bloom_bits < (1u << 30) && (size_t) bloom_bits < (size_t) ns * 16) bloom_bits <<= 1;
	const u32 nb16 = (ns + 15u) >> 4;
	const u32 n_jump = (ceil_log2_u64((u64) ns + 1) + 4) / 5 + 1;
	{
		auto up = [](size_t b) { return (b + 255) & ~(size_t) 255; };
		const size_t b_bloom = up(bloom_bits / 8), b_table = up(((size_t) tmask + 1) * 16), b_pred = up((size_t) ns * 8), b_clen = up((size_t) ns * 4),
		             b_jump = up((size_t) (n_jump + 1) * 4), b_linw = up(((size_t) nb16 + 1) * 8);
		uint8_t* z;
		const size_t zb = b_bloom + b_table + b_pred + b_clen + b_jump + b_linw;
		HIP_TRY(db.alloc(&z, zb));
		HIP_TRY(hipMemsetAsync(z, 0, zb, st));
		table = (ulonglong2*) z; z += b_table;
		bloom = (u32*) z; z += b_bloom;
		pred = (unsigned long long*) z; z += b_pred;
		clen = (u32*) z; z += b_clen;
		jump_open = (u32*) z; z += b_jump;
		linw = (u64*) z;
	}
	HIP_TRY(db.alloc(&skey0, ns)); HIP_TRY(db.alloc(&skey, ns));
	HIP_TRY(db.alloc(&succ0, (size_t) ns * 4)); HIP_TRY(db.alloc(&succ, (size_t) ns * 4));
	HIP_TRY(db.alloc(&pd, ns)); HIP_TRY(db.alloc(&coff, (size_t) ns + 1)); HIP_TRY(db.alloc(&newidx, ns));
	HIP_TRY(db.alloc(&lo2, ns)); HIP_TRY(db.alloc(&hi2, ns)); HIP_TRY(db.alloc(&gcnt2, ns)); HIP_TRY(db.alloc(&gfirst2, ns));
	HIP_TRY(db.alloc(&fbw, nb16));
	HIP_TRY(db.alloc(&bestsucc, ns));
	if (sym_walk) HIP_TRY(db.alloc(&partner, ns));
	const SurvTable tb0{table, tmask, skey0, bloom, bloom_bits - 1};
	const SurvTable tb{table, tmask, skey, bloom, bloom_bits - 1};
	if (table_out) *table_out = tb;
	const dim3 gs((ns + 255) / 256), bs(256);
	{
		vdjx_prof_scope ps(c, "k_surv_table");
		hipLaunchKernelGGL(k_surv_table2, gs, bs, 0, st, sv.lo, sv.hi, ns, table, tmask, skey0, bloom, bloom_bits - 1);
		hipLaunchKernelGGL(k_succ_links2, gs, bs, 0, st, tb0, ns, k, sv.gcnt, succ0, pred, bestsucc);
	}
	{
		vdjx_prof_scope ps(c, "k_chain_order");
		hipLaunchKernelGGL(k_chain_init, gs, bs, 0, st, pred, bestsucc, ns, pd);
		for (u32 j = 0; j < n_jump; j++) hipLaunchKernelGGL(k_chain_jump, gs, bs, 0, st, pd, ns, j ? jump_open + j - 1 : (const u32*) nullptr, jump_open + j);
		hipLaunchKernelGGL(k_chain_len, gs, bs, 0, st, pd, ns, clen);
		{ const int rc_ = vdjx_scan_wide(db, st, clen, ns, coff); if (rc_) return rc_; }
		hipLaunchKernelGGL(k_chain_place, gs, bs, 0, st, pd, coff, ns, newidx);
		hipLaunchKernelGGL(k_chain_permute, gs, bs, 0, st, newidx, ns, sv.lo, sv.hi, sv.gcnt, sv.gfirst, succ0, lo2, hi2, gcnt2, gfirst2, skey, succ);
		hipLaunchKernelGGL(k_table_remap, dim3(tmask / 256 + 1), bs, 0, st, table, tmask + 1, newidx);
		if (sym_walk) hipLaunchKernelGGL(k_partner, gs, bs, 0, st, tb, ns, k, partner);
		hipLaunchKernelGGL(k_chain_words, gs, bs, 0, st, succ, skey, ns, k, linw, fbw, (const u32*) partner);
	}
	dbg_sync(c, "k_chain_order");
	if (sync_debug()) {
		std::vector<u32> ni(ns), seen(ns, 0);
		(void) hipMemcpy(ni.data(), newidx, (size_t) ns * 4, hipMemcpyDeviceToHost);
		u32 dup = 0, oob = 0;
		for (u32 i = 0; i < ns; i++) { if (ni[i] >= ns) oob++; else if (seen[ni[i]]++) dup++; }
		std::vector<u64> pdh(ns);
		std::vector<unsigned long long> prh(ns);
		(void) hipMemcpy(pdh.data(), pd, (size_t) ns * 8, hipMemcpyDeviceToHost);
		(void) hipMemcpy(prh.data(), pred, (size_t) ns * 8, hipMemcpyDeviceToHost);
		u32 unresolved = 0;
		for (u32 i = 0; i < ns; i++) { const u32 p0 = (u32) (pdh[i] >> 32); if (p0 != NONE32 && (u32) (pdh[p0] >> 32) != NONE32) unresolved++; }
		fprintf(stderr, "[vdjx] chain order: %u survivors, %u duplicate new indices, %u out of range, %u unresolved (cycles), %u jump launches\n", ns, dup, oob, unresolved, n_jump);
		for (u32 i = 0, shown = 0; i < ns && shown < 6; i++) if (ni[i] < ns && seen[ni[i]] > 1) {
			fprintf(stderr, "[vdjx]   old %u -> new %u: pd = (%u, %u), pred word %llx\n", i, ni[i], (u32) (pdh[i] >> 32), (u32) pdh[i], prh[i]);
			shown++;
		}
	}
	sv.lo = lo2; sv.hi = hi2; sv.gcnt = gcnt2; sv.gfirst = gfirst2;
	ItemFmt f;
	{
		const u32 sb = ceil_log2_u64(ns);
		static const u32 force_lb = (u32) vdjx_env_num("VDJX_RC_LEN_BITS", 4, 0, 4);
		const u32 lb = std::min(std::min(4u, 26u - sb), force_lb);
		const u32 pb = 26u - lb;
		f.pmask = (1u << pb) - 1u;
		f.len_shift = IT_SURV_SHIFT + pb;
		f.maxlen = 1u << lb;
		const u32 t = ceil_log2_u64(nb16);
		f.bmask = (1u << t) - 1u;
		f.mul = t ? ((0x9E3779B9u >> (32 - t)) | 1u) : 1u;
		u32 x = f.mul;
		for (int i = 0; i < 5; i++) x *= 2u - f.mul * x;
		f.inv = x & f.bmask;
		f.ns = ns;
	}
	const u32 nsp = (f.bmask + 1u) << 4;
	static const bool force_wide = vdjx_env_num("VDJX_RC_WIDE", 0, 0, 1) != 0;
	static const u32 cap_shift = (u32) vdjx_env_num("VDJX_RC_MAX_SHIFT", 12, 8, 12);
	const bool narrow = R < (1ull << (32 - pool->ob)) && !force_wide;
	static const u32 max_ranges = (u32) vdjx_env_num("VDJX_RC_MAX_RANGES", PART_MAXB, 2, PART_MAXB);
	const u32 max_shift = std::max(8u, std::min(narrow ? 11u : 10u, cap_shift));
	u32 range_shift = 8;
	while (range_shift < max_shift && (nsp >> range_shift) > max_ranges) range_shift++;
	const u32 n_ranges = std::max(1u, nsp >> range_shift);
	u32 l2bits = 0;
	while (((n_ranges + (1u << l2bits) - 1) >> l2bits) > max_ranges) l2bits++;
	if (l2bits) l2bits = std::min(10u, std::max(l2bits, (ceil_log2_u64(n_ranges) + 1u) / 2u));
	const u32 n_coarse = (n_ranges + (1u << l2bits) - 1) >> l2bits;
	const u32 n_ranges_p = n_coarse << l2bits;
	constexpr size_t walk_blocks = 7168;
	const size_t Rw = sym_walk ? R / 2 : R;
	u32 nblk = (u32) std::min<size_t>(walk_blocks, (Rw + WALK_THREADS * 8 - 1) / (WALK_THREADS * 8));
	constexpr u32 walk_resident = 1536;
	if (nblk > walk_resident && nblk < walk_blocks) nblk = nblk / walk_resident * walk_resident;
	if (nblk < walk_resident) nblk = (u32) std::min<size_t>(walk_resident, (Rw + WALK_THREADS - 1) / WALK_THREADS);
	if (nblk == 0) nblk = 1;
	const size_t nwaves = (size_t) nblk * (WALK_THREADS / 64);
	const size_t NI = R * (size_t) P;
	u32 blk_items = 4096;
	while (blk_items > 256 && nwaves * blk_items > NI / 2 + 65536) blk_items >>= 1;
	const u64 raw_cap = (u64) NI + (u64) NI / (blk_items / 64) + nwaves * (u64) blk_items + blk_items;
	u64 *raw, *items;
	unsigned long long *g_cursor, *n_inst;
	u32 *range_cnt, *range_start, *g_err, *gcur;
	const vdjx_arena::mark_t tmp_mark = db.mark();
	HIP_TRY(db.alloc(&raw, (size_t) raw_cap));
	HIP_TRY(db.alloc(&g_cursor, 4 + ((size_t) n_ranges_p + 1) / 2));
	n_inst = g_cursor + 1;
	g_err = (u32*) (g_cursor + 2);
	range_cnt = (u32*) (g_cursor + 4);
	HIP_TRY(db.alloc(&range_start, n_ranges_p + 1));
	HIP_TRY(hipMemsetAsync(g_cursor, 0, 32 + (size_t) n_ranges_p * 4, st));
	if (sym_walk) {
		vdjx_prof_scope ps(c, "k_chain_order");
		hipLaunchKernelGGL(k_partner_check, gs, bs, 0, st, partner, linw, ns, g_err + 3);
	}
	const bool lng = pool->W > 2;
	if (lng && R >= (1ull << 27)) { vdjx_set_error("more than 2^27 records of long reads on one GPU: not supported by the recount items"); return VDJX_ELIMIT; }
	const size_t lds_walk = (((size_t) n_ranges_p + 1) & ~(size_t) 1) * 4 + (lng ? (size_t) WALK_THREADS * GL_ROW_LONG * 8 : 0);
	if ((size_t) n_ranges_p * 4 > 64 * 1024) { vdjx_set_error("too many survivor ranges for the walk histogram"); return VDJX_ELIMIT; }
	HIP_TRY(hipFuncSetAttribute((const void*) k_walk_items<false>, hipFuncAttributeMaxDynamicSharedMemorySize, (int) lds_walk));
	HIP_TRY(hipFuncSetAttribute((const void*) k_walk_items<true>, hipFuncAttributeMaxDynamicSharedMemorySize, (int) lds_walk));
	HIP_TRY(hipFuncSetAttribute((const void*) k_walk_items<false, true>, hipFuncAttributeMaxDynamicSharedMemorySize, (int) lds_walk));
#ifdef VDJX_ABLATE
	static const u32 walk_dbg = (u32) vdjx_env_num("VDJX_WALK_DBG", 0, 0, 63);
#else
	constexpr u32 walk_dbg = 0;
#endif
	if (R && walk_dbg != 0u) {
		u64* raw2;
		unsigned long long* cur2;
		u32* cnt2;
		HIP_TRY(db.alloc(&raw2, (size_t) raw_cap));
		HIP_TRY(db.alloc(&cur2, 8));
		HIP_TRY(db.alloc(&cnt2, n_ranges_p));
		HIP_TRY(hipMemsetAsync(cur2, 0, 64, st));
		HIP_TRY(hipMemsetAsync(cnt2, 0, (size_t) n_ranges_p * 4, st));
		vdjx_prof_scope ps(c, "k_walk_dbg");
		if (lng) hipLaunchKernelGGL(k_walk_items<true>, dim3(nblk), dim3(WALK_THREADS), lds_walk, st, pool->d_bases, pool->d_nmask, R, pool->rl, pool->ob, k, tb, succ, linw, f, range_shift,
		                            n_ranges_p, raw2, raw_cap, blk_items, cur2, cnt2, g_err, walk_dbg, (const u32*) nullptr);
		else hipLaunchKernelGGL(k_walk_items<false>, dim3(nblk), dim3(WALK_THREADS), lds_walk, st, pool->d_bases, pool->d_nmask, R, pool->rl, pool->ob, k, tb, succ, linw, f, range_shift,
		                        n_ranges_p, raw2, raw_cap, blk_items, cur2, cnt2, g_err, walk_dbg, (const u32*) nullptr);
		HIP_TRY(hipMemsetAsync(g_err, 0, 4, st));
		if (walk_dbg & 32u) {
			unsigned long long hs[8];
			HIP_TRY(hipMemcpyAsync(hs, cur2, 64, hipMemcpyDeviceToHost, st));
			HIP_TRY(hipStreamSynchronize(st));
			const char* nm[] = {"", "rows", "rounds", "filter", "lookup", "chain", "item_trips"};
			for (int i = 1; i < 7; i++) c->stats[std::string("walk_dbg_") + nm[i]] = hs[i];
		}
	}
	if (R) {
		vdjx_prof_scope ps(c, "k_walk_items");
		if (lng) hipLaunchKernelGGL(k_walk_items<true>, dim3(nblk), dim3(WALK_THREADS), lds_walk, st, pool->d_bases, pool->d_nmask, R, pool->rl, pool->ob, k, tb, succ, linw, f, range_shift,
		                            n_ranges_p, raw, raw_cap, blk_items, g_cursor, range_cnt, g_err, 0u, (const u32*) nullptr);
		else if (sym_walk) hipLaunchKernelGGL((k_walk_items<false, true>), dim3(nblk), dim3(WALK_THREADS), lds_walk, st, pool->d_bases, pool->d_nmask, R / 2, pool->rl, pool->ob, k, tb, succ, linw, f, range_shift,
		                                      n_ranges_p, raw, raw_cap, blk_items, g_cursor, range_cnt, g_err, 0u, (const u32*) partner);
		else hipLaunchKernelGGL(k_walk_items<false>, dim3(nblk), dim3(WALK_THREADS), lds_walk, st, pool->d_bases, pool->d_nmask, R, pool->rl, pool->ob, k, tb, succ, linw, f, range_shift,
		                        n_ranges_p, raw, raw_cap, blk_items, g_cursor, range_cnt, g_err, 0u, (const u32*) nullptr);
	}
	dbg_sync(c, "k_walk_items");
	vdjx_scan_one(st, range_cnt, n_ranges_p, range_start);
	size_t items_cap = NI + 1;
	if (!defer) {
		u32* hp = (u32*) c->h_pin;
		HIP_TRY(hipMemcpyAsync(hp, range_start + n_ranges_p, 4, hipMemcpyDeviceToHost, st));
		HIP_TRY(hipStreamSynchronize(st));
		HIP_TRY(hipGetLastError());
		items_cap = (size_t) hp[0] + 1;
	}
	HIP_TRY(db.alloc(&items, items_cap));
	HIP_TRY(db.alloc(&gcur, n_ranges_p));
	{
		vdjx_prof_scope ps(c, "k_part_items");
		u32 npb = (u32) std::min<size_t>(1024, (NI / 4 + 65535) / 65536);
		if (npb == 0) npb = 1;
		const auto k_part_items = k_part<u64, ItemRange, part_share, true>;
		if (!l2bits) {
			HIP_TRY(part_launch(st, k_part_items, npb, PART_LDS_BYTES, range_start, n_ranges_p, 0u, gcur, items, raw, part_share{g_cursor, n_ranges_p},
			                    ItemRange{f, range_shift, ~0u}));
		} else {
			u64* l1;
			u32* gcur1;
			HIP_TRY(db.alloc(&l1, items_cap));
			HIP_TRY(db.alloc(&gcur1, n_coarse));
			HIP_TRY(part_launch(st, k_part_items, npb, PART_LDS_BYTES, range_start, n_coarse, l2bits, gcur1, l1, raw, part_share{g_cursor, n_coarse},
			                    ItemRange{f, range_shift + l2bits, ~0u}));
			const u32 sl2 = std::max(8u, std::min(64u, 2048u / n_coarse));
			HIP_TRY(part_launch(st, k_part<u64, ItemRange, part_segs>, n_coarse * sl2, PART_LDS_BYTES, range_start, n_ranges_p, 0u, gcur, items,
			                    l1, part_segs{range_start, l2bits, sl2, l2bits}, ItemRange{f, range_shift, (1u << l2bits) - 1u}));
		}
	}
	dbg_sync(c, "k_part_items");
	{
		vdjx_prof_scope ps(c, "k_recount");
#define RC_LAUNCH(SB, IT) hipLaunchKernelGGL((k_recount<SB, IT>), dim3(n_ranges), dim3(RC_THREADS), 0, st, items, range_start, f, ns, rec_base, pool->ob, fbw, ro.ucnt, ro.ufirst, ro.in_first, n_inst)
		if (narrow) {
			switch (range_shift) {
				case 8: RC_LAUNCH(256, u32); break;
				case 9: RC_LAUNCH(512, u32); break;
				case 10: RC_LAUNCH(1024, u32); break;
				default: RC_LAUNCH(2048, u32); break;
			}
		} else {
			switch (range_shift) {
				case 8: RC_LAUNCH(256, u64); break;
				case 9: RC_LAUNCH(512, u64); break;
				default: RC_LAUNCH(1024, u64); break;
			}
		}
#undef RC_LAUNCH
	}
	dbg_sync(c, "k_recount");
	if (derive_edges) {
		hipLaunchKernelGGL(k_count_unseen, dim3((ns + 255) / 256), dim3(256), 0, st, ro.ufirst, ns, g_err + 1);
		HIP_TRY(hipMemsetAsync(ro.edge_first, 0xFF, (size_t) ns * 32, st));
		hipLaunchKernelGGL(k_edges_from_in, dim3((ns * 4 + 255) / 256), dim3(256), 0, st, tb, ns, k, ro.in_first, ro.in_from, ro.edge_first, ro.edge_to);
	}
	if (defer && !sync_debug()) {
		defer->g_err = g_err; defer->n_items = range_start + n_ranges_p; defer->n_inst = n_inst; defer->ns = ns;
		return VDJX_OK;
	}
	if (defer) defer->g_err = nullptr;
	u32* hp = (u32*) c->h_pin;
	HIP_TRY(hipMemcpyAsync(hp, g_err, 8, hipMemcpyDeviceToHost, st));
	HIP_TRY(hipMemcpyAsync(hp + 2, range_start + n_ranges_p, 4, hipMemcpyDeviceToHost, st));
	HIP_TRY(hipMemcpyAsync(hp + 4, n_inst, 8, hipMemcpyDeviceToHost, st));
	HIP_TRY(hipMemcpyAsync(hp + 6, g_err + 2, 8, hipMemcpyDeviceToHost, st));
	HIP_TRY(hipStreamSynchronize(st));
	HIP_TRY(hipGetLastError());
	if (hp[6] || hp[7]) { vdjx_set_error("the mirrored walk found %u + %u places where the chains are not mirror images", hp[6], hp[7]); return VDJX_ESYMWALK; }
	const u32 err[2] = {hp[0], hp[1]}, n_items = hp[2];
	const unsigned long long inst = *(const unsigned long long*) (hp + 4);
	if (err[0]) { vdjx_set_error("k_walk_items: item buffer too small (%u waves stopped)", err[0]); return VDJX_EHIP; }
	if (err[1]) {
		if (sync_debug()) {
			std::vector<u64> uf(ns), lo(ns), hi(ns), gf(ns);
			std::vector<u32> gc(ns);
			(void) hipMemcpy(uf.data(), ro.ufirst, (size_t) ns * 8, hipMemcpyDeviceToHost);
			(void) hipMemcpy(lo.data(), sv.lo, (size_t) ns * 8, hipMemcpyDeviceToHost);
			(void) hipMemcpy(hi.data(), sv.hi, (size_t) ns * 8, hipMemcpyDeviceToHost);
			(void) hipMemcpy(gf.data(), sv.gfirst, (size_t) ns * 8, hipMemcpyDeviceToHost);
			(void) hipMemcpy(gc.data(), sv.gcnt, (size_t) ns * 4, hipMemcpyDeviceToHost);
			for (u32 i = 0, shown = 0; i < ns && shown < 8; i++) if (uf[i] == NONE64) {
				char txt[65];
				for (int j = 0; j < k; j++) { const int sh = 2 * (k - 1 - j); const u32 c2 = (u32) (sh < 64 ? lo[i] >> sh : hi[i] >> (sh - 64)) & 3u; txt[j] = "ATCG"[c2]; }
				txt[k] = 0;
				fprintf(stderr, "[vdjx] unseen survivor %u: %s gated count %u first gated instance record %llu offset %llu\n", i, txt, gc[i],
				        (unsigned long long) (gf[i] >> 6), (unsigned long long) (gf[i] & 63));
				shown++;
			}
		}
		vdjx_set_error("internal error: %u of %u surviving k-mers were not met again in the records", err[1], ns);
		return VDJX_EHIP;
	}
	c->stats["recount_items"] = n_items;
	c->stats["recount_instances"] = inst;
	db.release_to(tmp_mark);
	return VDJX_OK;
}

template <typename A>
int stage_finish2(vdjx_ctx* c, A& db, const SurvivorsG& sv, const RecountOut& ro, u64 n_records_total, int k, int P, int ob, vdjx_graph* g) {
	hipStream_t st = c->stream;
	const u32 ns = sv.n;
	const u32 nr = sv.n_real <= ns ? sv.n_real : ns;
	g->n = nr;
	g->k = k;
	g->ctx = c;
	g->device = c->device;
	if (ns == 0) return VDJX_OK;
	uint8_t *d_hv, *d_hj;
	HIP_TRY(db.alloc(&d_hv, ns));
	HIP_TRY(db.alloc(&d_hj, ns));
	{
		vdjx_prof_scope ps(c, "k_node_flags");
		hipLaunchKernelGGL(k_node_flags, dim3((ns + 255) / 256), dim3(256), 0, st, sv.lo, sv.hi, ns, k, c->d_vbits, c->d_jbits, d_hv, d_hj);
	}
	u64 *rk_key, *rk_key2;
	u32 *rk_idx, *rk_idx2, *rank;
	HIP_TRY(db.alloc(&rk_key, ns));
	HIP_TRY(db.alloc(&rk_key2, ns));
	HIP_TRY(db.alloc(&rk_idx, ns));
	HIP_TRY(db.alloc(&rk_idx2, ns));
	HIP_TRY(db.alloc(&rank, ns));
	unsigned rk_bits = 1;
	while (rk_bits < 64 && (1ull << rk_bits) <= ((n_records_total << ob) | 1ull)) rk_bits++;
	auto up = [](size_t b) { return (b + 255) & ~(size_t) 255; };
	const size_t need = up((size_t) ns * 8) + 5 * up((size_t) ns * 4) + 4 * up(ns) + 2 * up((size_t) ns * 16) + up((size_t) ns * k);
	{
		hipError_t e = c->blocks.acquire(need, &g->d_block, &g->block_cap);
		if (e != hipSuccess) { vdjx_set_error("graph alloc (%zu bytes): %s", need, hipGetErrorString(e)); return VDJX_EHIP; }
	}
	char* bp = g->d_block;
	auto carve = [&](size_t b) { char* r = bp; bp += up(b); return r; };
	NodeOut no;
	no.klo = no.khi = nullptr;
	no.first_inst = g->d_first_inst = (u64*) carve((size_t) ns * 8);
	no.gcnt = g->d_gcnt = (u32*) carve((size_t) ns * 4);
	no.freq = g->d_freq = (u32*) carve((size_t) ns * 4);
	no.to_ids = g->d_to_ids = (u32*) carve((size_t) ns * 16);
	no.from_ids = g->d_from_ids = (u32*) carve((size_t) ns * 16);
	no.hv = g->d_hv = (uint8_t*) carve(ns);
	no.hj = g->d_hj = (uint8_t*) carve(ns);
	no.to_deg = g->d_to_deg = (uint8_t*) carve(ns);
	no.from_deg = g->d_from_deg = (uint8_t*) carve(ns);
	no.kmers = g->d_kmers = carve((size_t) ns * k);
	g->export_bytes = (size_t) (bp - g->d_block);
	g->d_roots = (u32*) carve((size_t) ns * 4);
	{
		vdjx_prof_scope ps(c, "k_node_order");
		hipLaunchKernelGGL(k_rank_keys, dim3((ns + 255) / 256), dim3(256), 0, st, sv.ufirst, sv.gcnt, ns, rk_key, rk_idx);
		{
			size_t tb = 0;
			int rc_ = vdjx_sort_pairs_raw(nullptr, &tb, st, rk_key, rk_key2, rk_idx, rk_idx2, ns, rk_bits);
			if (rc_) return rc_;
			char* tmp;
			HIP_TRY(db.alloc(&tmp, tb + 256));
			if ((rc_ = vdjx_sort_pairs_raw(tmp, &tb, st, rk_key, rk_key2, rk_idx, rk_idx2, ns, rk_bits))) return rc_;
		}
		hipLaunchKernelGGL(k_rank_scatter, dim3((ns + 255) / 256), dim3(256), 0, st, rk_key2, rk_idx2, ns, rank);
		hipLaunchKernelGGL(k_node_emit2, dim3((ns + 255) / 256), dim3(256), 0, st, sv.lo, sv.hi, sv.gcnt, sv.ucnt, sv.ufirst, d_hv, d_hj, rank,
		                   ro.edge_first, ro.edge_to, ro.in_first, ro.in_from, ns, k, no);
	}
	u32 n_roots = 0;
	{
		const u32 nrb = (nr + 255) / 256;
		u32 *rb_cnt, *rb_start;
		HIP_TRY(db.alloc(&rb_cnt, nrb + 1));
		HIP_TRY(db.alloc(&rb_start, nrb + 1));
		vdjx_prof_scope ps(c, "k_root_list");
		if (nrb) hipLaunchKernelGGL(k_root_count, dim3(nrb), dim3(256), 0, st, no.from_deg, nr, rb_cnt);
		vdjx_scan_one(st, rb_cnt, nrb, rb_start);
		if (nrb) hipLaunchKernelGGL(k_root_list, dim3(nrb), dim3(256), 0, st, no.from_deg, nr, rb_start, g->d_roots);
		HIP_TRY(hipMemcpyAsync(c->h_pin, rb_start + nrb, 4, hipMemcpyDeviceToHost, st));
	}
	HIP_TRY(hipStreamSynchronize(st));
	HIP_TRY(hipGetLastError());
	n_roots = *(const u32*) c->h_pin;
	g->n_roots = n_roots;
	vdjx_prof_collect(c, false);
	return VDJX_OK;
}

template <typename TUP>
int kmer_build_impl2(vdjx_ctx* c, const vdjx_pool* pool, int k, int mf, int mq, vdjx_graph* g) {
	const int P = pool->rl - k + 1;
	vdjx_work db(c);
	GTuples<TUP> t;
	const bool sym = build_sym(pool, k);
	c->stats["kmer_build_sym"] = sym ? 1 : 0;
	int rc = stage_gated_partition<TUP>(c, db, pool, 0, k, 0, 0, &t, sym);
	if (rc) return rc;
	PoolView pv{pool->d_bases, pool->d_nmask, vdjx_qrows{pool->d_quals, pool->d_quals2, pool->q_split, pool->qstride}, pool->rl, pool->ob};
	SurvivorsG sv;
	rc = stage_gated_reduce<TUP>(c, db, t, pv, 0, k, mf, mq, &sv, sym);
	if (rc) return rc;
	vdjx_ri_open_gate(c);
	dbg_sync(c, "gated_reduce");
	g->pre_nodes = (size_t) sv.ndist;
	RecountOut ro{};
	if (sv.n) {
		HIP_TRY(db.alloc(&sv.ucnt, sv.n)); HIP_TRY(db.alloc(&sv.ufirst, sv.n));
		HIP_TRY(db.alloc(&ro.in_first, (size_t) sv.n * 4)); HIP_TRY(db.alloc(&ro.in_from, (size_t) sv.n * 4));
		HIP_TRY(db.alloc(&ro.edge_first, (size_t) sv.n * 4)); HIP_TRY(db.alloc(&ro.edge_to, (size_t) sv.n * 4));
		ro.ucnt = sv.ucnt; ro.ufirst = sv.ufirst;
		for (int attempt = 0; attempt < 2; attempt++) {
			const bool sym_walk = sym && sym_walk_wanted() && attempt == 0;
			c->stats["kmer_build_sym_walk"] = sym_walk ? 1 : 0;
			RecountStatus rs;
			rc = stage_recount(c, db, pool, 0, k, sv, ro, true, nullptr, &rs, sym_walk);
			if (rc == VDJX_ESYMWALK && sym_walk) { c->stats["kmer_build_sym_walk_retries"] += 1; continue; }
			if (rc) return rc;
			u32* hp = (u32*) c->h_pin + 1024;
			hp[6] = hp[7] = 0;
			if (rs.g_err) {
				HIP_TRY(hipMemcpyAsync(hp + 8, rs.n_inst, 24, hipMemcpyDeviceToHost, c->stream));
				HIP_TRY(hipMemcpyAsync(hp + 2, rs.n_items, 4, hipMemcpyDeviceToHost, c->stream));
			}
			rc = stage_finish2(c, db, sv, ro, pool->n_records, k, P, pool->ob, g);
			if (rc) return rc;
			if (rs.g_err) { hp[4] = hp[8]; hp[5] = hp[9]; hp[0] = hp[10]; hp[1] = hp[11]; hp[6] = hp[12]; hp[7] = hp[13]; }
			rc = rs.g_err ? recount_status_check(c, hp, rs.ns) : VDJX_OK;
			if (rc != VDJX_ESYMWALK || !sym_walk) return rc == VDJX_ESYMWALK ? VDJX_EHIP : rc;
			c->stats["kmer_build_sym_walk_retries"] += 1;
			if (g->d_block) { c->blocks.release(g->d_block, g->block_cap); g->d_block = nullptr; g->block_cap = 0; }
		}
		return VDJX_EHIP;
	}
	return stage_finish2(c, db, sv, ro, pool->n_records, k, P, pool->ob, g);
}

}

extern "C" int vdjx_kmer_build(vdjx_ctx* c, const vdjx_pool* pool, int k, int mf, int mq, vdjx_graph** out) {
	if (!c || !pool || !out) { vdjx_set_error("vdjx_kmer_build: NULL argument"); return VDJX_EINVAL; }
	*out = nullptr;
	if (pool->ctx != c) { vdjx_set_error("vdjx_kmer_build: pool belongs to another context"); return VDJX_EINVAL; }
	if (k < 1 || k > VDJX_MAX_KMER || k > pool->rl) { vdjx_set_error("k=%d outside [1,min(%d,rl=%d)]", k, VDJX_MAX_KMER, pool->rl); return VDJX_ELIMIT; }
	if (k > 16 && !c->anchors_loaded) { vdjx_set_error("vdjx_kmer_build: call vdjx_anchor_sets_load first (k > 16)"); return VDJX_ESTATE; }
	HIP_TRY(hipSetDevice(c->device));
	vdjx_clear_errors();
	vdjx_graph* g = new vdjx_graph();
	const int rc = k <= 45 ? kmer_build_impl2<Tup16>(c, pool, k, mf, mq, g) : kmer_build_impl2<Tup24>(c, pool, k, mf, mq, g);
	if (rc != VDJX_OK) { vdjx_graph_free(g); return rc; }
	*out = g;
	return VDJX_OK;
}

struct vdjx_shard {
	vdjx_ctx* c = nullptr;
	const vdjx_pool* pool = nullptr;
	int k = 0, mf = 0, mq = 0, rank = 0, nranks = 1;
	u64 rec_stride = 0;
	const u32* scan = nullptr;
	u64 total_records = 0;
	u64 rec_base() const { return scan ? 0 : rec_stride * (u64) rank; }
	u64 records_in_all() const { return scan ? total_records : rec_stride * (u64) nranks; }
	bool sym_capable = false, sym = false;
	bool wide = false;
	u32 NBf = 0, NBo = 0;
	u32 *nd = nullptr, *dstart = nullptr;
	Partial* dense = nullptr;
	u32* dense_ref = nullptr;
	u64* low_inst = nullptr;
	u32 n_dense = 0;
	SurvivorsG local_sv, all_sv;
	u32 sv_cap = 0;
	u32* n_surv = nullptr;
	PendOut po{};
	u32 n_pend = 0;
	uint2* queries = nullptr;
	std::vector<u32> src_base, nq;
	u32 *p_fl = nullptr, *p_S = nullptr, *p_r0 = nullptr;
	u32 mqq = 0, tlow = 0;
	SurvTable tb{};
	int phase = 0;
	bool have_hist = false;
	GatedHist gh;
	u64 agreed = 0;
	Partial* sparse = nullptr;
	u32* sparse_ref = nullptr;
	vdjx_arena::mark_t fill_mark{0, 0};
	const u32* tuple_bucket_start = nullptr;
	u32 NBt = 0;
};

static int shard_begin_impl(vdjx_ctx* c, const vdjx_pool* pool, int k, int mf, int mq, int rank, int nranks,
                            uint64_t rec_stride, const uint32_t* d_scan, uint64_t total_records, vdjx_shard** out) {
	if (!c || !pool || !out) { vdjx_set_error("vdjx_shard_begin: NULL argument"); return VDJX_EINVAL; }
	*out = nullptr;
	if (c->live_shard) { vdjx_set_error("vdjx_shard_begin: a sharded build is already in flight on this context"); return VDJX_ESTATE; }
	if (nranks < 1 || nranks > 256 || rank < 0 || rank >= nranks) { vdjx_set_error("1 <= nranks <= 256, 0 <= rank < nranks"); return VDJX_EINVAL; }
	if (k < 1 || k > VDJX_MAX_KMER || k > pool->rl) { vdjx_set_error("k=%d outside [1,min(%d,rl=%d)]", k, VDJX_MAX_KMER, pool->rl); return VDJX_ELIMIT; }
	if (d_scan) {
		if (total_records < pool->n_records) { vdjx_set_error("total_records %llu < local records %zu", (unsigned long long) total_records, pool->n_records); return VDJX_EINVAL; }
		if (total_records >= (1ull << 32) || total_records >= (1ull << (INST_BITS - pool->ob))) { vdjx_set_error("global record count %llu: scan positions are 32 bits and instance ids record << %d | offset in %d bits", (unsigned long long) total_records, pool->ob, INST_BITS); return VDJX_ELIMIT; }
		rec_stride = (total_records + (uint64_t) nranks - 1) / (uint64_t) nranks;
	} else {
		if (rec_stride < pool->n_records) { vdjx_set_error("rec_stride %llu < local records %zu", (unsigned long long) rec_stride, pool->n_records); return VDJX_EINVAL; }
		if (rec_stride * (uint64_t) nranks >= (1ull << (INST_BITS - pool->ob))) { vdjx_set_error("global record count %llu >= 2^%d (instance ids are record << %d | offset in %d bits)", (unsigned long long) (rec_stride * nranks), INST_BITS - pool->ob, pool->ob, INST_BITS); return VDJX_ELIMIT; }
	}
	if (k > 16 && !c->anchors_loaded) { vdjx_set_error("vdjx_shard_begin: call vdjx_anchor_sets_load first (k > 16)"); return VDJX_ESTATE; }
	if (pool->W > 2 && pool->n_records >= (1ull << 27)) { vdjx_set_error("more than 2^27 records of long reads on one GPU: not supported by the recount items"); return VDJX_ELIMIT; }
	vdjx_shard* s = new vdjx_shard();
	s->c = c; s->pool = pool; s->k = k; s->mf = mf; s->mq = mq; s->rank = rank; s->nranks = nranks;
	s->rec_stride = rec_stride;
	s->scan = d_scan; s->total_records = total_records;
	s->sym_capable = build_sym(pool, k) && s->rec_base() % 2 == 0;
	s->wide = k > 45;
	if (mq >= 255) mq = 254;
	s->mqq = (u32) (mq < 0 ? 0 : (mq > 214 ? 214 : mq));
	s->tlow = 1 + (s->mqq + 19) / 20;
	c->live_shard = s;
	*out = s;
	return VDJX_OK;
}

extern "C" int vdjx_shard_begin(vdjx_ctx* c, const vdjx_pool* pool, int k, int mf, int mq, int rank, int nranks,
                                uint64_t rec_stride, vdjx_shard** out) {
	return shard_begin_impl(c, pool, k, mf, mq, rank, nranks, rec_stride, nullptr, 0, out);
}

extern "C" int vdjx_shard_begin_share(vdjx_ctx* c, const vdjx_pool* pool, int k, int mf, int mq, int rank, int nranks,
                                      const uint32_t* d_scan_index, uint64_t total_records, vdjx_shard** out) {
	if (pool && pool->n_records && !d_scan_index) { vdjx_set_error("vdjx_shard_begin_share: NULL scan index"); return VDJX_EINVAL; }
	static const uint32_t none = 0;
	return shard_begin_impl(c, pool, k, mf, mq, rank, nranks, 0, d_scan_index ? d_scan_index : &none, total_records, out);
}

extern "C" void vdjx_shard_free(vdjx_shard* s) {
	if (!s) return;
	(void) hipSetDevice(s->c->device);
	(void) hipStreamSynchronize(s->c->stream);
	s->c->shard_arena.reset();
	s->c->live_shard = nullptr;
	delete s;
}

extern "C" size_t vdjx_shard_record_bytes(int kind) {
	return kind == 0 ? sizeof(Partial) : kind == 1 ? sizeof(uint2) : kind == 2 ? REPLY_BYTES : kind == 3 ? sizeof(SurvRec) : 0;
}

static u64 shard_geometry_bound(const vdjx_shard* s) {
	const int P = s->pool->rl - s->k + 1;
	return std::max<u64>(1, s->rec_stride * (u64) P / 4);
}

template <typename TUP>
static int shard_local_impl(vdjx_shard* s) {
	vdjx_ctx* c = s->c;
	hipStream_t st = c->stream;
	PersistAlloc db(c);
	const u64 rec_base = s->rec_base();
	GTuples<TUP> t;
	int rc = VDJX_OK;
	if (s->have_hist && s->gh.sym != s->sym) s->have_hist = false;
	const size_t per_b = 0;
	if (!s->have_hist) rc = stage_gated_hist(c, db, s->pool, s->k, per_b, shard_geometry_bound(s) / (s->sym ? 2 : 1), &s->gh, s->sym);
	if (rc) return rc;
	s->have_hist = true;
	const size_t cap = (size_t) s->gh.N + 1;
	const size_t nb_max = ((size_t) 1 << 20) + 16 * (size_t) s->nranks + 2;
	Partial* sparse;
	u32 *g_err, *sparse_ref;
	HIP_TRY(db.alloc(&s->low_inst, cap));
	HIP_TRY(db.alloc(&s->dense_ref, cap));
	HIP_TRY(db.alloc(&s->nd, nb_max));
	HIP_TRY(db.alloc(&s->dstart, nb_max + 1));
	HIP_TRY(db.alloc(&g_err, 1));
	u32* keep_starts;
	HIP_TRY(db.alloc(&keep_starts, nb_max + 1));
	s->fill_mark = db.mark();
	HIP_TRY(db.alloc(&sparse, cap));
	HIP_TRY(db.alloc(&sparse_ref, cap));
	const vdjx_arena::mark_t tuple_mark = db.mark();
	rc = stage_gated_cut<TUP>(c, db, s->pool, rec_base, s->k, per_b, (s->agreed ? s->agreed : shard_geometry_bound(s)) / (s->sym ? 2 : 1), s->gh, &t);
	if (rc) return rc;
	if (t.NB < (u32) s->nranks) { vdjx_set_error("vdjx_shard_local: fewer buckets (%u) than ranks", t.NB); return VDJX_ELIMIT; }
	s->NBo = t.NB / (u32) s->nranks;
	if (s->NBo * (u32) s->nranks != t.NB) s->NBo = (s->NBo + 1 + 15) & ~15u;
	s->NBf = s->NBo * (u32) s->nranks;
	if ((size_t) s->NBf + 1 > nb_max) { vdjx_set_error("vdjx_shard_local: %u buckets", s->NBf); return VDJX_ELIMIT; }
	HIP_TRY(hipMemsetAsync(g_err, 0, 4, st));
	if (s->NBf > t.NB) HIP_TRY(hipMemsetAsync(s->nd + t.NB, 0, (size_t) (s->NBf - t.NB) * 4, st));
	if ((rc = set_sub_tuples(c))) return rc;
	{
		vdjx_prof_scope ps(c, "k_gated_local");
		u32* order;
		if ((rc = bucket_order(c, db, t, &order))) return rc;
		if (s->sym) hipLaunchKernelGGL((k_gated_local<TUP, true>), dim3(t.NB), dim3(LG_THREADS), 0, st, t.t, t.bucket_start, s->pool->d_bases, s->pool->d_nmask, rec_base,
		                               s->k, s->pool->rl, s->pool->ob, s->tlow, sparse, sparse_ref, s->nd, s->low_inst, g_err, (const u32*) order);
		else hipLaunchKernelGGL(k_gated_local<TUP>, dim3(t.NB), dim3(LG_THREADS), 0, st, t.t, t.bucket_start, s->pool->d_bases, s->pool->d_nmask, rec_base,
		                        s->k, s->pool->rl, s->pool->ob, s->tlow, sparse, sparse_ref, s->nd, s->low_inst, g_err, (const u32*) order);
	}
	vdjx_scan_one(st, s->nd, s->NBf, s->dstart);
	u32* d_pick;
	const u32 G = (u32) s->nranks;
	HIP_TRY(db.alloc(&d_pick, G + 1));
	hipLaunchKernelGGL(k_pick_u32, dim3(1), dim3(512), 0, st, s->dstart, s->NBo, G + 1, d_pick);
	std::vector<u32> pick(G + 1);
	u32 err = 0;
	HIP_TRY(hipMemcpyAsync(pick.data(), d_pick, (G + 1) * 4, hipMemcpyDeviceToHost, st));
	HIP_TRY(hipMemcpyAsync(&err, g_err, 4, hipMemcpyDeviceToHost, st));
	HIP_TRY(hipMemcpyAsync(keep_starts, t.bucket_start, ((size_t) t.NB + 1) * 4, hipMemcpyDeviceToDevice, st));
	HIP_TRY(hipStreamSynchronize(st));
	HIP_TRY(hipGetLastError());
	if (err) { vdjx_set_error("k_gated_local: %u buckets could not be split to fit LDS", err); return VDJX_EHIP; }
	s->src_base.assign(pick.begin(), pick.end());
	s->n_dense = pick[G];
	s->sparse = sparse; s->sparse_ref = sparse_ref; s->NBt = t.NB;
	s->dense = nullptr;
	db.release_to(tuple_mark);
	s->tuple_bucket_start = keep_starts;
	return VDJX_OK;
}

extern "C" int vdjx_shard_local(vdjx_shard* s, uint64_t* send_counts, uint32_t* dir_len) {
	if (!s || !send_counts || !dir_len) { vdjx_set_error("vdjx_shard_local: NULL argument"); return VDJX_EINVAL; }
	if (s->phase != 0) { vdjx_set_error("vdjx_shard_local: already called"); return VDJX_ESTATE; }
	HIP_TRY(hipSetDevice(s->c->device));
	vdjx_clear_errors();
	int rc = s->wide ? shard_local_impl<Tup24>(s) : shard_local_impl<Tup16>(s);
	if (rc) return rc;
	vdjx_ri_open_gate(s->c);
	for (int g = 0; g < s->nranks; g++) send_counts[g] = s->src_base[g + 1] - s->src_base[g];
	*dir_len = s->NBo;
	s->phase = 1;
	return VDJX_OK;
}

extern "C" int vdjx_shard_local_fill(vdjx_shard* s, void* d_dir, void* d_partials) {
	if (!s || s->phase < 1) { vdjx_set_error("vdjx_shard_local_fill: call vdjx_shard_local first"); return VDJX_ESTATE; }
	if (!d_dir || (s->n_dense && !d_partials)) { vdjx_set_error("vdjx_shard_local_fill: NULL buffer"); return VDJX_EINVAL; }
	if (((uintptr_t) d_partials & 15u) != 0) { vdjx_set_error("vdjx_shard_local_fill: d_partials must be 16-byte aligned"); return VDJX_EINVAL; }
	HIP_TRY(hipSetDevice(s->c->device));
	vdjx_clear_errors();
	hipStream_t st = s->c->stream;
	HIP_TRY(hipMemcpyAsync(d_dir, s->nd, (size_t) s->NBf * 4, hipMemcpyDeviceToDevice, st));
	if (s->n_dense) {
		vdjx_prof_scope ps(s->c, "k_compact_partials");
		hipLaunchKernelGGL(k_compact_partials, dim3(s->NBt), dim3(256), 0, st, s->sparse, s->sparse_ref, s->tuple_bucket_start, s->nd, s->dstart, (Partial*) d_partials, s->dense_ref, s->scan, s->pool->ob, s->sym);
	}
	s->dense = (Partial*) d_partials;
	HIP_TRY(hipStreamSynchronize(st));
	HIP_TRY(hipGetLastError());
	if (s->sparse) {
		PersistAlloc db(s->c);
		db.release_to(s->fill_mark);
		s->sparse = nullptr; s->sparse_ref = nullptr; s->tuple_bucket_start = nullptr;
	}
	return VDJX_OK;
}

extern "C" int vdjx_shard_count(vdjx_shard* s, uint64_t* gated_instances) {
	if (!s || !gated_instances) { vdjx_set_error("vdjx_shard_count: NULL argument"); return VDJX_EINVAL; }
	if (s->phase != 0) { vdjx_set_error("vdjx_shard_count: call it before vdjx_shard_local"); return VDJX_ESTATE; }
	HIP_TRY(hipSetDevice(s->c->device));
	vdjx_clear_errors();
	if (!s->have_hist) {
		PersistAlloc db(s->c);
		const int rc = stage_gated_hist(s->c, db, s->pool, s->k, 0, shard_geometry_bound(s) / (s->sym_capable ? 2 : 1), &s->gh, s->sym_capable);
		if (rc) return rc;
		s->have_hist = true;
	}
	*gated_instances = (u64) s->gh.N * (s->gh.sym ? 2 : 1);
	return VDJX_OK;
}
extern "C" int vdjx_shard_symmetric(const vdjx_shard* s) { return s && s->sym_capable ? 1 : 0; }
extern "C" int vdjx_shard_geometry2(vdjx_shard* s, uint64_t agreed_instances, int all_symmetric) {
	if (!s) { vdjx_set_error("vdjx_shard_geometry2: NULL argument"); return VDJX_EINVAL; }
	if (all_symmetric && !s->sym_capable) { vdjx_set_error("vdjx_shard_geometry2: this rank's pool is not made of couples"); return VDJX_EINVAL; }
	const int rc = vdjx_shard_geometry(s, agreed_instances);
	if (rc) return rc;
	s->sym = all_symmetric != 0;
	s->c->stats["kmer_build_sym"] = s->sym ? 1 : 0;
	return VDJX_OK;
}
extern "C" int vdjx_shard_geometry(vdjx_shard* s, uint64_t agreed_instances) {
	if (!s) { vdjx_set_error("vdjx_shard_geometry: NULL argument"); return VDJX_EINVAL; }
	if (s->phase != 0) { vdjx_set_error("vdjx_shard_geometry: call it before vdjx_shard_local"); return VDJX_ESTATE; }
	if (agreed_instances < (u64) s->gh.N * (s->gh.sym ? 2 : 1)) { vdjx_set_error("vdjx_shard_geometry: %llu is less than this rank's own %llu gated instances", (unsigned long long) agreed_instances, (unsigned long long) s->gh.N * (s->gh.sym ? 2 : 1)); return VDJX_EINVAL; }
	s->agreed = agreed_instances ? agreed_instances : 1;
	return VDJX_OK;
}

template <typename THI>
static int shard_merge_impl(vdjx_shard* s, const u32* d_recv_dir, const Partial* d_recv, const uint64_t* recv_counts, uint64_t* query_counts) {
	vdjx_ctx* c = s->c;
	hipStream_t st = c->stream;
	PersistAlloc db(c);
	const u32 G = (u32) s->nranks, NBo = s->NBo;
	s->src_base.assign(G + 1, 0);
	for (u32 g = 0; g < G; g++) s->src_base[g + 1] = s->src_base[g] + (u32) recv_counts[g];
	const u32 total = s->src_base[G];
	u32 *d_src_base, *seg_off, *g_nq, *g_err, *n_pend;
	u64* g_distinct;
	HIP_TRY(db.alloc(&d_src_base, G + 1));
	HIP_TRY(db.alloc(&seg_off, (size_t) G * (NBo + 1)));
	HIP_TRY(db.alloc(&g_nq, G));
	HIP_TRY(db.alloc(&g_err, 1));
	HIP_TRY(db.alloc(&n_pend, 1));
	HIP_TRY(db.alloc(&s->n_surv, 1));
	HIP_TRY(db.alloc(&g_distinct, 1));
	HIP_TRY(db.alloc(&s->queries, (size_t) total + 1));
	const u32 cap = (s->sym ? 2 : 1) * total + 2;
	s->sv_cap = cap;
	SurvivorsG& v = s->local_sv;
	HIP_TRY(db.alloc(&v.lo, cap)); HIP_TRY(db.alloc(&v.hi, cap)); HIP_TRY(db.alloc(&v.gcnt, cap)); HIP_TRY(db.alloc(&v.gfirst, cap));
	PendOut& po = s->po;
	HIP_TRY(db.alloc(&po.lo, cap)); HIP_TRY(db.alloc(&po.hi, cap)); HIP_TRY(db.alloc(&po.cg, cap)); HIP_TRY(db.alloc(&po.mg, cap));
	HIP_TRY(db.alloc(&po.need, cap));
	po.mgr = nullptr;
	if (s->sym) HIP_TRY(db.alloc(&po.mgr, cap));
	po.n = n_pend; po.cap = cap;
	HIP_TRY(hipMemcpyAsync(d_src_base, s->src_base.data(), (G + 1) * 4, hipMemcpyHostToDevice, st));
	hipLaunchKernelGGL(k_seg_offsets, dim3(G), dim3(1024), 0, st, d_recv_dir, d_src_base, G, NBo, seg_off);
	const u32 cmin = (u32) std::max(s->mf, 2);
	SurvOutG so{v.lo, v.hi, v.gcnt, v.gfirst, s->n_surv, cap, nullptr};
	s->nq.assign(G, 0);
	u32 MG = 1;
	while (MG < NBo && NBo % (MG * 2) == 0 && (u64) total * (MG * 2) <= (u64) NBo * (MERGE_SLOTS * 3 / 8)) MG <<= 1;
	u32 np = 0, ns = 0, err = 0;
	u64 ndist = 0;
	for (u32 s_mult = 1;; s_mult *= 4) {
		HIP_TRY(hipMemsetAsync(g_nq, 0, (size_t) G * 4, st));
		HIP_TRY(hipMemsetAsync(g_err, 0, 4, st));
		HIP_TRY(hipMemsetAsync(n_pend, 0, 4, st));
		HIP_TRY(hipMemsetAsync(s->n_surv, 0, 4, st));
		HIP_TRY(hipMemsetAsync(g_distinct, 0, 8, st));
		if (total) {
			vdjx_prof_scope ps(c, "k_bucket_merge");
			if (s->sym) hipLaunchKernelGGL((k_bucket_merge<THI, true>), dim3(NBo / MG), dim3(MERGE_THREADS), 0, st, d_recv, seg_off, MG, G, NBo, d_src_base, s_mult, cmin,
			                               s->tlow, so, po, s->queries, g_nq, g_distinct, g_err, s->k);
			else hipLaunchKernelGGL(k_bucket_merge<THI>, dim3(NBo / MG), dim3(MERGE_THREADS), 0, st, d_recv, seg_off, MG, G, NBo, d_src_base, s_mult, cmin,
			                        s->tlow, so, po, s->queries, g_nq, g_distinct, g_err, s->k);
		}
		HIP_TRY(hipMemcpyAsync(s->nq.data(), g_nq, (size_t) G * 4, hipMemcpyDeviceToHost, st));
		HIP_TRY(hipMemcpyAsync(&np, n_pend, 4, hipMemcpyDeviceToHost, st));
		HIP_TRY(hipMemcpyAsync(&ns, s->n_surv, 4, hipMemcpyDeviceToHost, st));
		HIP_TRY(hipMemcpyAsync(&err, g_err, 4, hipMemcpyDeviceToHost, st));
		HIP_TRY(hipMemcpyAsync(&ndist, g_distinct, 8, hipMemcpyDeviceToHost, st));
		HIP_TRY(hipStreamSynchronize(st));
		HIP_TRY(hipGetLastError());
		if (!err) break;
		if (s_mult >= (1u << 16)) { vdjx_set_error("k_bucket_merge: %u buckets could not be split to fit LDS", err); return VDJX_EHIP; }
	}
	s->n_pend = np;
	c->stats["shard_partials_received"] = total;
	c->stats["shard_open_kmers"] = np;
	c->stats["shard_decided_at_merge"] = ns;
	{
		u64 nqs = 0;
		for (u32 q : s->nq) nqs += q;
		c->stats["shard_questions"] = nqs;
	}
	v.n = ns;
	v.ndist = ndist;
	for (u32 g = 0; g < G; g++) query_counts[g] = s->nq[g];
	const size_t sides = s->sym ? 2 : 1;
	HIP_TRY(db.alloc(&s->p_fl, (size_t) np + 1));
	HIP_TRY(db.alloc(&s->p_r0, sides * np + 1));
	HIP_TRY(db.alloc(&s->p_S, sides * np * 64 + 1));
	if (np) {
		HIP_TRY(hipMemsetAsync(s->p_fl, 0, (size_t) np * 4, st));
		HIP_TRY(hipMemsetAsync(s->p_r0, 0xFF, sides * np * 4, st));
		HIP_TRY(hipMemsetAsync(s->p_S, 0, sides * np * 256, st));
	}
	return VDJX_OK;
}

extern "C" int vdjx_shard_merge(vdjx_shard* s, const void* d_recv_dir, const void* d_recv_partials, const uint64_t* recv_counts,
                                uint64_t* query_counts) {
	if (!s || !recv_counts || !query_counts || !d_recv_dir) { vdjx_set_error("vdjx_shard_merge: NULL argument"); return VDJX_EINVAL; }
	if (s->phase != 1) { vdjx_set_error("vdjx_shard_merge: call vdjx_shard_local first (once)"); return VDJX_ESTATE; }
	uint64_t tot = 0;
	for (int g = 0; g < s->nranks; g++) tot += recv_counts[g];
	if (tot >= (1ull << 30)) { vdjx_set_error("vdjx_shard_merge: too many partial aggregates for one owner (%llu): use more ranks", (unsigned long long) tot); return VDJX_ELIMIT; }
	if (tot && !d_recv_partials) { vdjx_set_error("vdjx_shard_merge: NULL buffer"); return VDJX_EINVAL; }
	HIP_TRY(hipSetDevice(s->c->device));
	vdjx_clear_errors();
	int rc = s->wide ? shard_merge_impl<u64>(s, (const u32*) d_recv_dir, (const Partial*) d_recv_partials, recv_counts, query_counts)
	                 : shard_merge_impl<u32>(s, (const u32*) d_recv_dir, (const Partial*) d_recv_partials, recv_counts, query_counts);
	if (rc) return rc;
	s->phase = 2;
	return VDJX_OK;
}

extern "C" int vdjx_shard_queries(vdjx_shard* s, void* d_out) {
	if (!s || s->phase < 2) { vdjx_set_error("vdjx_shard_queries: call vdjx_shard_merge first"); return VDJX_ESTATE; }
	HIP_TRY(hipSetDevice(s->c->device));
	vdjx_clear_errors();
	hipStream_t st = s->c->stream;
	size_t at = 0;
	for (int g = 0; g < s->nranks; g++) {
		if (!s->nq[g]) continue;
		if (!d_out) { vdjx_set_error("vdjx_shard_queries: NULL buffer"); return VDJX_EINVAL; }
		HIP_TRY(hipMemcpyAsync((uint2*) d_out + at, s->queries + s->src_base[g], (size_t) s->nq[g] * sizeof(uint2), hipMemcpyDeviceToDevice, st));
		at += s->nq[g];
	}
	HIP_TRY(hipStreamSynchronize(st));
	return VDJX_OK;
}

extern "C" int vdjx_shard_reply(vdjx_shard* s, const void* d_queries, const uint64_t* counts, void* d_replies) {
	if (!s || !counts) { vdjx_set_error("vdjx_shard_reply: NULL argument"); return VDJX_EINVAL; }
	if (s->phase < 1 || (s->n_dense && !s->dense)) { vdjx_set_error("vdjx_shard_reply: call vdjx_shard_local and vdjx_shard_local_fill first"); return VDJX_ESTATE; }
	vdjx_ctx* c = s->c;
	HIP_TRY(hipSetDevice(c->device));
	vdjx_clear_errors();
	const u32 G = (u32) s->nranks;
	std::vector<u32> off(G + 1, 0);
	for (u32 g = 0; g < G; g++) off[g + 1] = off[g] + (u32) counts[g];
	const u32 nq = off[G];
	if (!nq) return VDJX_OK;
	if (!d_queries || !d_replies) { vdjx_set_error("vdjx_shard_reply: NULL buffer"); return VDJX_EINVAL; }
	PersistAlloc db(c);
	u32* d_off;
	HIP_TRY(db.alloc(&d_off, G + 1));
	hipStream_t st = c->stream;
	HIP_TRY(hipMemcpyAsync(d_off, off.data(), (G + 1) * 4, hipMemcpyHostToDevice, st));
	const vdjx_pool* p = s->pool;
	{
		vdjx_prof_scope ps(c, "k_shard_reply");
		if (s->sym) hipLaunchKernelGGL(k_shard_reply<true>, dim3(nq), dim3(64), 0, st, (const uint2*) d_queries, nq, d_off, G, s->dense, s->dense_ref, s->dstart, s->NBo,
		                               s->low_inst, p->d_bases, p->d_nmask, vdjx_qrows{p->d_quals, p->d_quals2, p->q_split, p->qstride}, s->rec_base(), s->scan, (u32) p->n_records, s->k, p->rl, p->ob, (uint8_t*) d_replies);
		else hipLaunchKernelGGL(k_shard_reply<false>, dim3(nq), dim3(64), 0, st, (const uint2*) d_queries, nq, d_off, G, s->dense, s->dense_ref, s->dstart, s->NBo,
		                        s->low_inst, p->d_bases, p->d_nmask, vdjx_qrows{p->d_quals, p->d_quals2, p->q_split, p->qstride}, s->rec_base(), s->scan, (u32) p->n_records, s->k, p->rl, p->ob, (uint8_t*) d_replies);
	}
	HIP_TRY(hipStreamSynchronize(st));
	HIP_TRY(hipGetLastError());
	return VDJX_OK;
}

extern "C" int vdjx_shard_resolve(vdjx_shard* s, const void* d_replies, uint64_t n_replies, uint64_t* n_survivors, uint64_t* n_distinct) {
	if (!s || !n_survivors || !n_distinct) { vdjx_set_error("vdjx_shard_resolve: NULL argument"); return VDJX_EINVAL; }
	if (s->phase != 2) { vdjx_set_error("vdjx_shard_resolve: call vdjx_shard_merge first (once)"); return VDJX_ESTATE; }
	uint64_t expect = 0;
	for (u32 q : s->nq) expect += q;
	if (n_replies != expect) { vdjx_set_error("vdjx_shard_resolve: %llu answers for %llu questions", (unsigned long long) n_replies, (unsigned long long) expect); return VDJX_EINVAL; }
	vdjx_ctx* c = s->c;
	HIP_TRY(hipSetDevice(c->device));
	vdjx_clear_errors();
	hipStream_t st = c->stream;
	SurvivorsG& v = s->local_sv;
	if (s->n_pend) {
		if (!d_replies) { vdjx_set_error("vdjx_shard_resolve: NULL buffer"); return VDJX_EINVAL; }
		const u32 nr = (u32) n_replies;
		SurvOutG so{v.lo, v.hi, v.gcnt, v.gfirst, s->n_surv, s->sv_cap, nullptr};
		vdjx_prof_scope ps(c, "k_shard_resolve");
		hipLaunchKernelGGL(k_resolve_first, dim3((nr + 255) / 256), dim3(256), 0, st, (const uint8_t*) d_replies, nr, s->po.mg, s->p_r0, (const u64*) s->po.mgr, s->n_pend);
		hipLaunchKernelGGL(k_resolve_add, dim3((nr + 3) / 4), dim3(256), 0, st, (const uint8_t*) d_replies, nr, s->p_r0, s->k, s->p_fl, s->p_S, s->sym ? s->n_pend : 0u);
		if (s->sym) hipLaunchKernelGGL(k_resolve_keep<true>, dim3((s->n_pend + 255) / 256), dim3(256), 0, st, s->po, s->n_pend, s->p_fl, s->p_S, s->k,
		                               (u32) std::max(s->mf, 0), s->mqq, s->tlow, so);
		else hipLaunchKernelGGL(k_resolve_keep<false>, dim3((s->n_pend + 255) / 256), dim3(256), 0, st, s->po, s->n_pend, s->p_fl, s->p_S, s->k,
		                        (u32) std::max(s->mf, 0), s->mqq, s->tlow, so);
	}
	u32 ns = 0;
	HIP_TRY(hipMemcpyAsync(&ns, s->n_surv, 4, hipMemcpyDeviceToHost, st));
	HIP_TRY(hipStreamSynchronize(st));
	HIP_TRY(hipGetLastError());
	c->stats["shard_kept_after_answers"] = ns - v.n;
	v.n = ns;
	*n_survivors = ns;
	*n_distinct = v.ndist;
	s->phase = 3;
	return VDJX_OK;
}

extern "C" int vdjx_shard_survivors(vdjx_shard* s, void* d_out) {
	if (!s || s->phase < 3) { vdjx_set_error("vdjx_shard_survivors: call vdjx_shard_resolve first"); return VDJX_ESTATE; }
	const SurvivorsG& v = s->local_sv;
	if (!v.n) return VDJX_OK;
	if (!d_out) { vdjx_set_error("vdjx_shard_survivors: NULL buffer"); return VDJX_EINVAL; }
	HIP_TRY(hipSetDevice(s->c->device));
	vdjx_clear_errors();
	hipLaunchKernelGGL(k_surv_pack, dim3((v.n + 255) / 256), dim3(256), 0, s->c->stream, v.lo, v.hi, v.gcnt, v.gfirst, v.n, (SurvRec*) d_out);
	HIP_TRY(hipStreamSynchronize(s->c->stream));
	HIP_TRY(hipGetLastError());
	return VDJX_OK;
}

extern "C" int vdjx_shard_edges(vdjx_shard* s, const void* d_surv_all, uint64_t ns_total, void* d_in_first, void* d_ucnt, void* d_ufirst) {
	if (!s || s->phase < 3) { vdjx_set_error("vdjx_shard_edges: call vdjx_shard_resolve first"); return VDJX_ESTATE; }
	if (ns_total >= (1ull << 26)) { vdjx_set_error("vdjx_shard_edges: too many survivors"); return VDJX_ELIMIT; }
	vdjx_ctx* c = s->c;
	HIP_TRY(hipSetDevice(c->device));
	vdjx_clear_errors();
	PersistAlloc db(c);
	SurvivorsG& a = s->all_sv;
	a.n = (u32) ns_total;
	a.n_real = a.n;
	s->phase = 4;
	if (!ns_total) return VDJX_OK;
	if (!d_surv_all || !d_in_first || !d_ucnt || !d_ufirst) { vdjx_set_error("vdjx_shard_edges: NULL buffer"); return VDJX_EINVAL; }
	HIP_TRY(db.alloc(&a.lo, a.n)); HIP_TRY(db.alloc(&a.hi, a.n)); HIP_TRY(db.alloc(&a.gcnt, a.n)); HIP_TRY(db.alloc(&a.gfirst, a.n));
	u32* d_nreal;
	HIP_TRY(db.alloc(&d_nreal, 1));
	HIP_TRY(hipMemsetAsync(d_nreal, 0, 4, c->stream));
	hipLaunchKernelGGL(k_surv_unpack, dim3((a.n + 255) / 256), dim3(256), 0, c->stream, (const SurvRec*) d_surv_all, a.n, a.lo, a.hi, a.gcnt, a.gfirst, d_nreal);
	u32* h_nreal = (u32*) c->h_pin + 1536;
	HIP_TRY(hipMemcpyAsync(h_nreal, d_nreal, 4, hipMemcpyDeviceToHost, c->stream));
	RecountOut ro{(u32*) d_ucnt, (u64*) d_ufirst, (u64*) d_in_first, nullptr, nullptr, nullptr};
	const bool sym_walk = s->sym && sym_walk_wanted();
	c->stats["kmer_build_sym_walk"] = sym_walk ? 1 : 0;
	const SurvivorsG a_in = a;
	int rc = stage_recount(c, db, s->pool, s->rec_base(), s->k, a, ro, false, &s->tb, nullptr, sym_walk);
	if (rc == VDJX_ESYMWALK && sym_walk) {
		c->stats["kmer_build_sym_walk_retries"] += 1;
		a = a_in;
		rc = stage_recount(c, db, s->pool, s->rec_base(), s->k, a, ro, false, &s->tb, nullptr, false);
	}
	if (rc == VDJX_OK) a.n_real = *h_nreal;
	if (rc || !s->scan) return rc == VDJX_ESYMWALK ? VDJX_EHIP : rc;
	hipLaunchKernelGGL(k_first_to_scan, dim3((a.n * 5 + 255) / 256), dim3(256), 0, c->stream, (u64*) d_in_first, (size_t) a.n * 4, (u64*) d_ufirst, (size_t) a.n, s->scan, s->pool->ob);
	HIP_TRY(hipStreamSynchronize(c->stream));
	HIP_TRY(hipGetLastError());
	return VDJX_OK;
}

extern "C" int vdjx_shard_finish(vdjx_shard* s, const void* d_in_first, const void* d_ucnt, const void* d_ufirst,
                                 uint64_t pre_nodes_total, vdjx_graph** out) {
	if (!s || !out || s->phase < 4) { vdjx_set_error("vdjx_shard_finish: call vdjx_shard_edges first"); return VDJX_ESTATE; }
	*out = nullptr;
	vdjx_ctx* c = s->c;
	HIP_TRY(hipSetDevice(c->device));
	vdjx_clear_errors();
	PersistAlloc db(c);
	const int P = s->pool->rl - s->k + 1;
	SurvivorsG& a = s->all_sv;
	RecountOut ro{};
	if (a.n) {
		if (!d_ucnt || !d_ufirst || !d_in_first) { vdjx_set_error("vdjx_shard_finish: NULL buffer"); return VDJX_EINVAL; }
		a.ucnt = (u32*) d_ucnt;
		a.ufirst = (u64*) d_ufirst;
		ro.ucnt = a.ucnt; ro.ufirst = a.ufirst; ro.in_first = (u64*) d_in_first;
		HIP_TRY(db.alloc(&ro.in_from, (size_t) a.n * 4));
		HIP_TRY(db.alloc(&ro.edge_first, (size_t) a.n * 4));
		HIP_TRY(db.alloc(&ro.edge_to, (size_t) a.n * 4));
		HIP_TRY(hipMemsetAsync(ro.edge_first, 0xFF, (size_t) a.n * 32, c->stream));
		hipLaunchKernelGGL(k_edges_from_in, dim3((a.n * 4 + 255) / 256), dim3(256), 0, c->stream, s->tb, a.n, s->k, ro.in_first, ro.in_from, ro.edge_first, ro.edge_to);
	}
	vdjx_graph* g = new vdjx_graph();
	g->pre_nodes = (size_t) pre_nodes_total;
	int rc = stage_finish2(c, db, a, ro, s->records_in_all(), s->k, P, s->pool->ob, g);
	if (rc) { vdjx_graph_free(g); return rc; }
	*out = g;
	return VDJX_OK;
}

extern "C" size_t vdjx_graph_nodes(const vdjx_graph* g) { return g ? g->n : 0; }
extern "C" size_t vdjx_graph_pre_nodes(const vdjx_graph* g) { return g ? g->pre_nodes : 0; }
extern "C" size_t vdjx_graph_roots(const vdjx_graph* g) { return g ? g->n_roots : 0; }

static int graph_export_on(const vdjx_graph* g, hipStream_t st, uint64_t* first_inst, uint32_t* gated_count, uint32_t* freq, uint8_t* has_v,
                           uint8_t* has_j, uint8_t* to_deg, uint32_t* to_ids, uint8_t* from_deg, uint32_t* from_ids, char* kmers) {
	const size_t n = g->n;
	if (first_inst) HIP_TRY(hipMemcpyAsync(first_inst, g->d_first_inst, n * 8, hipMemcpyDeviceToHost, st));
	if (gated_count) HIP_TRY(hipMemcpyAsync(gated_count, g->d_gcnt, n * 4, hipMemcpyDeviceToHost, st));
	if (freq) HIP_TRY(hipMemcpyAsync(freq, g->d_freq, n * 4, hipMemcpyDeviceToHost, st));
	if (has_v) HIP_TRY(hipMemcpyAsync(has_v, g->d_hv, n, hipMemcpyDeviceToHost, st));
	if (has_j) HIP_TRY(hipMemcpyAsync(has_j, g->d_hj, n, hipMemcpyDeviceToHost, st));
	if (to_deg) HIP_TRY(hipMemcpyAsync(to_deg, g->d_to_deg, n, hipMemcpyDeviceToHost, st));
	if (from_deg) HIP_TRY(hipMemcpyAsync(from_deg, g->d_from_deg, n, hipMemcpyDeviceToHost, st));
	if (to_ids) HIP_TRY(hipMemcpyAsync(to_ids, g->d_to_ids, n * 16, hipMemcpyDeviceToHost, st));
	if (from_ids) HIP_TRY(hipMemcpyAsync(from_ids, g->d_from_ids, n * 16, hipMemcpyDeviceToHost, st));
	if (kmers) HIP_TRY(hipMemcpyAsync(kmers, g->d_kmers, n * (size_t) g->k, hipMemcpyDeviceToHost, st));
	return VDJX_OK;
}

extern "C" int vdjx_graph_export(const vdjx_graph* g, uint64_t* first_inst, uint32_t* gated_count, uint32_t* freq,
                                 uint8_t* has_v, uint8_t* has_j, uint8_t* to_deg, uint32_t* to_ids,
                                 uint8_t* from_deg, uint32_t* from_ids, char* kmers) {
	if (!g) { vdjx_set_error("vdjx_graph_export: NULL graph"); return VDJX_EINVAL; }
	if (g->n == 0) return VDJX_OK;
	if (!g->d_block || !vdjx_ctx_alive(g->ctx)) { vdjx_set_error("vdjx_graph_export: the graph's context is gone"); return VDJX_ESTATE; }
	HIP_TRY(hipSetDevice(g->device));
	int rc = graph_export_on(g, g->ctx->stream, first_inst, gated_count, freq, has_v, has_j, to_deg, to_ids, from_deg, from_ids, kmers);
	if (rc) return rc;
	HIP_TRY(hipStreamSynchronize(g->ctx->stream));
	return VDJX_OK;
}

extern "C" int vdjx_graph_export_begin(const vdjx_graph* g, uint64_t* first_inst, uint32_t* gated_count, uint32_t* freq,
                                       uint8_t* has_v, uint8_t* has_j, uint8_t* to_deg, uint32_t* to_ids,
                                       uint8_t* from_deg, uint32_t* from_ids, char* kmers) {
	if (!g) { vdjx_set_error("vdjx_graph_export_begin: NULL graph"); return VDJX_EINVAL; }
	if (g->n == 0) return VDJX_OK;
	if (!g->d_block || !vdjx_ctx_alive(g->ctx)) { vdjx_set_error("vdjx_graph_export_begin: the graph's context is gone"); return VDJX_ESTATE; }
	HIP_TRY(hipSetDevice(g->device));
	return graph_export_on(g, g->ctx->copy_stream, first_inst, gated_count, freq, has_v, has_j, to_deg, to_ids, from_deg, from_ids, kmers);
}

extern "C" int vdjx_graph_block_layout(const vdjx_graph* g, uint64_t* offsets, uint64_t* bytes) {
	if (!g || !offsets || !bytes) { vdjx_set_error("vdjx_graph_block_layout: NULL argument"); return VDJX_EINVAL; }
	const char* b = g->d_block;
	const void* at[10] = {g->d_first_inst, g->d_gcnt, g->d_freq, g->d_hv, g->d_hj, g->d_to_deg, g->d_to_ids, g->d_from_deg, g->d_from_ids, g->d_kmers};
	for (int i = 0; i < 10; i++) offsets[i] = g->n ? (uint64_t) ((const char*) at[i] - b) : 0;
	*bytes = g->n ? g->export_bytes : 0;
	return VDJX_OK;
}
static int graph_block_on(const vdjx_graph* g, bool copy_stream, void* host_block, const char* who) {
	if (!g) { vdjx_set_error("%s: NULL graph", who); return VDJX_EINVAL; }
	if (g->n == 0) return VDJX_OK;
	if (!host_block) { vdjx_set_error("%s: NULL buffer", who); return VDJX_EINVAL; }
	if (!g->d_block || !vdjx_ctx_alive(g->ctx)) { vdjx_set_error("%s: the graph's context is gone", who); return VDJX_ESTATE; }
	HIP_TRY(hipSetDevice(g->device));
	HIP_TRY(hipMemcpyAsync(host_block, g->d_block, g->export_bytes, hipMemcpyDeviceToHost, copy_stream ? g->ctx->copy_stream : g->ctx->stream));
	return VDJX_OK;
}
extern "C" int vdjx_graph_export_block(const vdjx_graph* g, void* host_block) {
	const int rc = graph_block_on(g, false, host_block, "vdjx_graph_export_block");
	if (rc || !g || g->n == 0) return rc;
	HIP_TRY(hipStreamSynchronize(g->ctx->stream));
	return VDJX_OK;
}
extern "C" int vdjx_graph_export_block_begin(const vdjx_graph* g, void* host_block) {
	return graph_block_on(g, true, host_block, "vdjx_graph_export_block_begin");
}

extern "C" int vdjx_graph_export_end(const vdjx_graph* g) {
	if (!g) { vdjx_set_error("vdjx_graph_export_end: NULL graph"); return VDJX_EINVAL; }
	if (!vdjx_ctx_alive(g->ctx)) { vdjx_set_error("vdjx_graph_export_end: the graph's context is gone"); return VDJX_ESTATE; }
	HIP_TRY(hipSetDevice(g->device));
	HIP_TRY(hipStreamSynchronize(g->ctx->copy_stream));
	return VDJX_OK;
}

extern "C" void vdjx_graph_free(vdjx_graph* g) {
	if (!g) return;
	if (g->d_block) {
		(void) hipSetDevice(g->device);
		if (vdjx_ctx_alive(g->ctx)) {
			(void) hipStreamSynchronize(g->ctx->copy_stream);
			g->ctx->blocks.release(g->d_block, g->block_cap);
		}
		else vdjx_block_cache::discard(g->d_block);
	}
	delete g;
}

struct PartTestKey {
	u32 shift, mask;
	__device__ inline u32 operator()(u64 x) const { return ((u32) (x >> 40) >> shift) & mask; }
	__device__ inline u32 operator()(const Tup16& t) const { return (*this)(t.lo); }
};

template <typename T, bool PAIRED>
static int part_test(vdjx_ctx* c, const void* host_in, size_t n, const std::vector<u32>& cnt, int levels, u32 fine_bits, u32 slices, u32 workgroups,
                     u32* host_starts, void* host_out) {
	hipStream_t st = c->stream;
	vdjx_work db(c);
	const u32 nb = (u32) cnt.size(), coarse = nb >> fine_bits;
	const unsigned long long n_raw = n;
	T *d_in, *d_l1, *d_out;
	u32 *d_cnt, *d_starts, *gcur, *gcur1;
	unsigned long long* d_n;
	HIP_TRY(db.alloc(&d_in, n + 1));
	HIP_TRY(db.alloc(&d_l1, n + 1));
	HIP_TRY(db.alloc(&d_out, n + 1));
	HIP_TRY(db.alloc(&d_cnt, nb));
	HIP_TRY(db.alloc(&d_starts, nb + 1));
	HIP_TRY(db.alloc(&gcur, nb));
	HIP_TRY(db.alloc(&gcur1, coarse));
	HIP_TRY(db.alloc(&d_n, 1));
	if (n) HIP_TRY(hipMemcpyAsync(d_in, host_in, n * sizeof(T), hipMemcpyHostToDevice, st));
	HIP_TRY(hipMemcpyAsync(d_cnt, cnt.data(), (size_t) nb * 4, hipMemcpyHostToDevice, st));
	HIP_TRY(hipMemcpyAsync(d_n, &n_raw, 8, hipMemcpyHostToDevice, st));
	vdjx_scan_one(st, (const u32*) d_cnt, nb, d_starts);
	const auto level1 = k_part<T, PartTestKey, part_share, PAIRED>;
	if (levels == 1) {
		HIP_TRY(part_launch(st, level1, workgroups, PART_LDS_BYTES, d_starts, nb, 0u, gcur, d_out, d_in, part_share{d_n, nb}, PartTestKey{0u, ~0u}));
	} else {
		HIP_TRY(part_launch(st, level1, workgroups, PART_LDS_BYTES, d_starts, coarse, fine_bits, gcur1, d_l1, d_in, part_share{d_n, coarse},
		                    PartTestKey{fine_bits, ~0u}));
		HIP_TRY(part_launch(st, k_part<T, PartTestKey, part_segs>, coarse * slices, PART_LDS_BYTES, d_starts, nb, 0u, gcur, d_out, d_l1,
		                    part_segs{d_starts, fine_bits, slices, fine_bits}, PartTestKey{0u, (1u << fine_bits) - 1u}));
	}
	const size_t kept = std::accumulate(cnt.begin(), cnt.end(), (size_t) 0);
	HIP_TRY(hipMemcpyAsync(host_starts, d_starts, ((size_t) nb + 1) * 4, hipMemcpyDeviceToHost, st));
	if (kept) HIP_TRY(hipMemcpyAsync(host_out, d_out, kept * sizeof(T), hipMemcpyDeviceToHost, st));
	HIP_TRY(hipStreamSynchronize(st));
	HIP_TRY(hipGetLastError());
	return VDJX_OK;
}

extern "C" int vdjx_part_u64(vdjx_ctx* c, const void* host_in, size_t n, int elem_bytes, uint32_t nb, int levels, uint32_t fine_bits, uint32_t slices,
                             uint32_t workgroups, uint32_t* host_starts, void* host_out) {
	const auto refuse = [](const char* what) { vdjx_set_error("vdjx_part_u64: %s", what); return VDJX_EINVAL; };
	if (!c || !host_starts || (n && (!host_in || !host_out)) || n >= (1ull << 31)) return refuse("bad argument");
	if (elem_bytes != 8 && elem_bytes != 16) return refuse("elements of 8 or 16 bytes");
	if (levels != 1 && levels != 2) return refuse("one level or two");
	if (slices == 0 || slices > 1024 || workgroups == 0 || workgroups > 65536) return refuse("1 .. 1024 slices, 1 .. 65536 workgroups");
	if (levels == 1) fine_bits = 0;
	if (fine_bits > 10) return refuse("at most 10 fine bits");
	if (nb == 0 || (nb >> fine_bits) > PART_MAXB || (nb >> fine_bits) << fine_bits != nb) return refuse("nb is at most 1024, or coarse << fine_bits with coarse <= 1024");
	std::vector<u32> cnt(nb, 0u);
	const u64* w = (const u64*) host_in;
	for (size_t i = 0; i < n; i++) {
		const u64 x = w[i * (size_t) (elem_bytes / 8)];
		if (elem_bytes == 8 && x == PART_HOLE) continue;
		if ((x >> 40) >= nb) return refuse("the bucket of an element is not below nb");
		cnt[(size_t) (x >> 40)]++;
	}
	HIP_TRY(hipSetDevice(c->device));
	vdjx_clear_errors();
	if (elem_bytes == 8) return part_test<u64, true>(c, host_in, n, cnt, levels, fine_bits, slices, workgroups, host_starts, host_out);
	return part_test<Tup16, false>(c, host_in, n, cnt, levels, fine_bits, slices, workgroups, host_starts, host_out);
}
```

Baseline: 916.4.

## Fold buffer clears and small kernels into neighbouring kernels to cut launches

Replaces several hipMemsetAsync calls with a custom clear kernel and fuses initialisations into existing kernels: pred/clen zeroing into k_surv_table2, edge_first fill into k_count_unseen, rank-key setup into k_node_flags, table remap into k_chain_permute, and the partner check into k_chain_words. Small zeroed counters for the build are merged into one shared allocation cleared once. It also drops one chain-jump iteration from the count. The aim is to remove fill-buffer launches and per-kernel launch overhead in the survivor stage, at the cost of more coupling and a risk from the reduced jump count and the reused zeroed buffers.

```diff
diff --git a/profiles/r07_trace_summary.py b/profiles/r07_trace_summary.py
--- /dev/null
+++ b/profiles/r07_trace_summary.py
@@ -0,0 +1,56 @@
+#!/usr/bin/env python3
+import collections
+import csv
+import glob
+import json
+import os
+import sys
+
+SURVIVOR_STAGE = ("k_surv_table2", "k_succ_links2", "k_chain_init", "k_chain_jump", "k_chain_len", "k_chain_place", "k_chain_permute",
+                  "k_table_remap", "k_partner", "k_chain_words", "k_partner_check", "k_count_unseen", "k_edges_from_in",
+                  "k_node_flags", "k_rank_keys", "k_rank_scatter", "k_node_emit2", "k_root_count", "k_root_list", "k_clear16")
+
+
+def short(name):
+    return name.replace("void ", "").replace("(anonymous namespace)::", "").split("(")[0].split("<")[0]
+
+
+def main():
+    steps = int(sys.argv[2]) if len(sys.argv) > 2 else 2
+    rows = []
+    for f in glob.glob(os.path.join(sys.argv[1], "**", "*kernel_trace.csv"), recursive=True):
+        rows += list(csv.DictReader(open(f)))
+    rows.sort(key=lambda r: int(r["Start_Timestamp"]))
+    names = [short(r["Kernel_Name"]) for r in rows]
+    packs = [i for i, n in enumerate(names) if n.startswith("k_pool_pack")]
+    walks = [i for i, n in enumerate(names) if n == "k_walk_items"]
+    per = max(1, round(len(packs) / max(1, len(walks))))
+    first = packs[-per * steps]
+    agg = collections.defaultdict(lambda: [0, 0])
+    fill_us = []
+    for r, n in zip(rows[first:], names[first:]):
+        a = agg[n]
+        a[0] += 1
+        a[1] += int(r["End_Timestamp"]) - int(r["Start_Timestamp"])
+        if "fillBuffer" in n:
+            fill_us.append(round((int(r["End_Timestamp"]) - int(r["Start_Timestamp"])) / 1e3, 1))
+    table = {n: {"launches_per_step": a[0] / steps, "ms_per_step": round(a[1] / steps / 1e6, 4)} for n, a in agg.items()}
+    fills = {n: v for n, v in table.items() if "fillBuffer" in n}
+    surv = {n: table[n] for n in SURVIVOR_STAGE if n in table}
+    out = {"steps": steps,
+           "fill_kernels": fills,
+           "fill_ms_per_step": round(sum(v["ms_per_step"] for v in fills.values()), 4),
+           "fill_launches_per_step": sum(v["launches_per_step"] for v in fills.values()),
+           "fill_launch_us_all_steps": sorted(fill_us, reverse=True),
+           "survivor_stage": surv,
+           "survivor_stage_ms_per_step": round(sum(v["ms_per_step"] for v in surv.values()), 4),
+           "survivor_stage_launches_per_step": sum(v["launches_per_step"] for v in surv.values()),
+           "all_kernels_ms_per_step": round(sum(v["ms_per_step"] for v in table.values()), 4),
+           "all_kernels_launches_per_step": sum(v["launches_per_step"] for v in table.values()),
+           "kernels": dict(sorted(table.items(), key=lambda kv: -kv[1]["ms_per_step"]))}
+    json.dump(out, sys.stdout, indent=1)
+    print()
+
+
+if __name__ == "__main__":
+    main()
diff --git a/vdjer_amd/csrc/vdjx_kmer.hip b/vdjer_amd/csrc/vdjx_kmer.hip
--- a/vdjer_amd/csrc/vdjx_kmer.hip
+++ b/vdjer_amd/csrc/vdjx_kmer.hip
@@ -33,6 +33,18 @@
 __global__ void k_pick_u32(const u32* __restrict__ src, u32 step, u32 n, u32* __restrict__ out) {
 	const u32 i = blockIdx.x * blockDim.x + threadIdx.x;
 	if (i < n) out[i] = src[(size_t) i * step];
+}
+
+__global__ __launch_bounds__(256) void k_clear16(uint4* __restrict__ p, size_t n16, u32 word) {
+	const uint4 v = make_uint4(word, word, word, word);
+	const size_t stride = (size_t) gridDim.x * 256;
+	for (size_t i = (size_t) blockIdx.x * 256 + threadIdx.x; i < n16; i += stride) p[i] = v;
+}
+static void clear16_async(hipStream_t st, void* p, size_t bytes, u32 word = 0) {
+	const size_t n16 = (bytes + 15) / 16;
+	if (!n16) return;
+	const u32 blocks = (u32) std::min<size_t>(2048, (n16 + 1023) / 1024);
+	hipLaunchKernelGGL(k_clear16, dim3(blocks), dim3(256), 0, st, (uint4*) p, n16, word);
 }
 
 template <typename THI, u32 SLOTS>
@@ -1174,9 +1186,12 @@
 
 __global__ void k_node_flags(const u64* __restrict__ s_lo, const u64* __restrict__ s_hi, u32 n, int k,
                              const u32* __restrict__ vbits, const u32* __restrict__ jbits,
-                             uint8_t* __restrict__ has_v, uint8_t* __restrict__ has_j) {
+                             uint8_t* __restrict__ has_v, uint8_t* __restrict__ has_j,
+                             const u64* __restrict__ ufirst, const u32* __restrict__ gcnt, u64* __restrict__ rk_key, u32* __restrict__ rk_idx) {
 	u32 i = blockIdx.x * blockDim.x + threadIdx.x;
 	if (i >= n) return;
+	rk_key[i] = (gcnt[i] & GC_SHADOW) ? NONE64 : ufirst[i];
+	rk_idx[i] = i;
 	if (k <= 16) { has_v[i] = 1; has_j[i] = 1; return; }
 	u128 key = ((u128) s_hi[i] << 64) | s_lo[i];
 	u32 code = (u32) (key >> (2 * (k - 16)));
@@ -1208,11 +1223,14 @@
 __device__ inline u32 it_scat(const ItemFmt& f, u32 p) { return ((((p >> 4) * f.mul) & f.bmask) << 4) | (p & 15u); }
 
 __global__ void k_surv_table2(const u64* __restrict__ s_lo, const u64* __restrict__ s_hi, u32 n, ulonglong2* __restrict__ slots, u32 mask,
-                              ulonglong2* __restrict__ skey, u32* __restrict__ bloom, u32 bloom_mask) {
+                              ulonglong2* __restrict__ skey, u32* __restrict__ bloom, u32 bloom_mask, unsigned long long* __restrict__ pred,
+                              u32* __restrict__ clen) {
 	const u32 i = blockIdx.x * blockDim.x + threadIdx.x;
 	if (i >= n) return;
 	const u64 lo = s_lo[i], hi = s_hi[i];
 	skey[i] = make_ulonglong2(lo, hi);
+	pred[i] = 0ull;
+	clen[i] = 0u;
 	const u64 h = vdjx_mix(lo, hi);
 	{
 		const u32 bit = (u32) (h >> 40) & bloom_mask;
@@ -1285,14 +1303,10 @@
 	const int q = surv_lookup2(t, rlo, rh);
 	partner[p] = q >= 0 ? (u32) q : NONE32;
 }
-__global__ void k_partner_check(const u32* __restrict__ partner, const u64* __restrict__ linw, u32 n, u32* __restrict__ bad) {
-	const u32 p = blockIdx.x * blockDim.x + threadIdx.x;
-	if (p >= n) return;
+__device__ inline bool partner_wrong(const u32* __restrict__ partner, u32 p, u32 n, bool linked) {
 	bool wrong = partner[p] == NONE32;
-	const bool linked = (linw[p >> 4] >> (15u - (p & 15u))) & 1ull;
 	if (!wrong && linked && (p + 1 >= n || partner[p + 1] != partner[p] - 1u)) wrong = true;
-	const u64 m = __ballot(wrong);
-	if (m && __lane_id() == 0) atomicAdd(bad, (u32) __popcll(m));
+	return wrong;
 }
 
 __global__ void k_chain_jump(u64* __restrict__ pd, u32 n, const u32* __restrict__ open_prev, u32* __restrict__ open_now) {
@@ -1340,8 +1354,13 @@
 }
 __global__ void k_chain_permute(const u32* __restrict__ newidx, u32 n, const u64* __restrict__ lo, const u64* __restrict__ hi, const u32* __restrict__ gcnt,
                                 const u64* __restrict__ gfirst, const u32* __restrict__ succ, u64* __restrict__ lo2, u64* __restrict__ hi2,
-                                u32* __restrict__ gcnt2, u64* __restrict__ gfirst2, ulonglong2* __restrict__ skey2, u32* __restrict__ succ2) {
+                                u32* __restrict__ gcnt2, u64* __restrict__ gfirst2, ulonglong2* __restrict__ skey2, u32* __restrict__ succ2,
+                                ulonglong2* __restrict__ slots, u32 n_slots) {
 	const u32 v = blockIdx.x * blockDim.x + threadIdx.x;
+	if (v < n_slots) {
+		const u64 y = slots[v].y;
+		if (y) slots[v].y = (y & SLOT_HI_MASK) | ((u64) (newidx[(u32) (y >> SLOT_HI_BITS) - 1] + 1u) << SLOT_HI_BITS);
+	}
 	if (v >= n) return;
 	const u32 q = newidx[v];
 	const u64 l = lo[v], h = hi[v];
@@ -1355,20 +1374,14 @@
 	r.w = s.w == NONE32 ? NONE32 : newidx[s.w];
 	*(uint4*) &succ2[(size_t) q * 4] = r;
 }
-__global__ void k_table_remap(ulonglong2* __restrict__ slots, u32 n_slots, const u32* __restrict__ newidx) {
-	const u32 i = blockIdx.x * blockDim.x + threadIdx.x;
-	if (i >= n_slots) return;
-	const u64 y = slots[i].y;
-	if (!y) return;
-	slots[i].y = (y & SLOT_HI_MASK) | ((u64) (newidx[(u32) (y >> SLOT_HI_BITS) - 1] + 1u) << SLOT_HI_BITS);
-}
 
 __global__ void k_chain_words(const u32* __restrict__ succ, const ulonglong2* __restrict__ skey, u32 n, int k, u64* __restrict__ linw, u32* __restrict__ fbw,
-                              const u32* __restrict__ partner) {
+                              const u32* __restrict__ partner, u32* __restrict__ bad) {
 	const u32 p = blockIdx.x * blockDim.x + threadIdx.x;
 	const u32 j = p & 15u;
 	u64 w = 0;
 	u32 fb = 0;
+	if (p == 0) linw[(n + 15u) >> 4] = 0ull;
 	if (p < n) {
 		const uint4 s = *(const uint4*) &succ[(size_t) p * 4];
 		const u32 sv[4] = {s.x, s.y, s.z, s.w};
@@ -1380,6 +1393,10 @@
 		const ulonglong2 kk = skey[p];
 		const int sh = 2 * (k - 1);
 		fb = (u32) (sh < 64 ? kk.x >> sh : kk.y >> (sh - 64)) & 3u;
+	}
+	if (partner) {
+		const u64 m = __ballot(p < n && partner_wrong(partner, p, n, (w >> (15u - j)) & 1ull));
+		if (m && __lane_id() == 0) atomicAdd(bad, (u32) __popcll(m));
 	}
 	u32 fw = fb << (2 * j);
 	for (int d = 1; d < 16; d <<= 1) {
@@ -1791,9 +1808,14 @@
 	if (threadIdx.x == 0 && tot) atomicAdd(n_inst, tot);
 }
 
-__global__ void k_count_unseen(const u64* __restrict__ ufirst, u32 n, u32* __restrict__ out) {
+__global__ void k_count_unseen(const u64* __restrict__ ufirst, u32 n, u32* __restrict__ out, u64* __restrict__ edge_first) {
 	const u32 i = blockIdx.x * blockDim.x + threadIdx.x;
 	const bool un = i < n && ufirst[i] == NONE64;
+	if (i < n && edge_first) {
+		const ulonglong2 none = make_ulonglong2(NONE64, NONE64);
+		ulonglong2* e = (ulonglong2*) (edge_first + (size_t) i * 4);
+		e[0] = none; e[1] = none;
+	}
 	const u64 m = __ballot(un);
 	if (m && __lane_id() == 0) atomicAdd(out, (u32) __popcll(m));
 }
@@ -1844,10 +1866,6 @@
 	uint8_t* to_deg; u32* to_ids; uint8_t* from_deg; u32* from_ids;
 };
 
-__global__ void k_rank_keys(const u64* __restrict__ ufirst, const u32* __restrict__ gcnt, u32 n, u64* __restrict__ key, u32* __restrict__ idx) {
-	const u32 i = blockIdx.x * blockDim.x + threadIdx.x;
-	if (i < n) { key[i] = (gcnt[i] & GC_SHADOW) ? NONE64 : ufirst[i]; idx[i] = i; }
-}
 __global__ void k_rank_scatter(const u64* __restrict__ key, const u32* __restrict__ idx, u32 n, u32* __restrict__ rank) {
 	const u32 j = blockIdx.x * blockDim.x + threadIdx.x;
 	if (j >= n) return;
@@ -1968,6 +1986,23 @@
 	fprintf(stderr, "[vdjx] %s: %s\n", what, hipGetErrorString(e));
 }
 
+#define BZ_HCNT (1u << 15)
+#define BZ_DISTINCT (64 * 16 + 2)
+#define RC_RANGES_MAX (16u * 1024u)
+#define BZ_CURSOR (4 + RC_RANGES_MAX / 2)
+struct BuildZeros { u32* hcnt = nullptr; u64* distinct = nullptr; unsigned long long* cursor = nullptr; };
+template <typename A>
+int build_zeros_alloc(vdjx_ctx* c, A& db, BuildZeros* bz) {
+	u64* z;
+	const size_t n = BZ_HCNT / 2 + BZ_DISTINCT + BZ_CURSOR;
+	HIP_TRY(db.alloc(&z, n));
+	clear16_async(c->stream, z, n * 8);
+	bz->hcnt = (u32*) z;
+	bz->distinct = z + BZ_HCNT / 2;
+	bz->cursor = (unsigned long long*) (z + BZ_HCNT / 2 + BZ_DISTINCT);
+	return VDJX_OK;
+}
+
 struct GatedHist { u32 HB = 0, NBH = 0, N = 0; u32* hstart = nullptr; bool sym = false; };
 static bool build_sym(const vdjx_pool* pool, int k) {
 	return pool->sym && pool->W == 2 && (k & 1) && pool->n_records % 2 == 0;
@@ -1975,7 +2010,8 @@
 static bool sym_walk_wanted() { static const bool on = !vdjx_env_set("VDJX_NO_SYM_WALK"); return on; }
 static size_t gated_bucket_default() { static const size_t v = (size_t) vdjx_env_num("VDJX_GATED_BUCKET", 3072, 1, 1ll << 32); return v; }
 template <typename A>
-int stage_gated_hist(vdjx_ctx* c, A& db, const vdjx_pool* pool, int k, size_t per_bucket, u64 geometry_instances, GatedHist* gh, bool sym = false) {
+int stage_gated_hist(vdjx_ctx* c, A& db, const vdjx_pool* pool, int k, size_t per_bucket, u64 geometry_instances, GatedHist* gh, bool sym = false,
+                     const BuildZeros* bz = nullptr) {
 	hipStream_t st = c->stream;
 	const size_t R = sym ? pool->n_records / 2 : pool->n_records;
 	const int P = pool->rl - k + 1;
@@ -1994,9 +2030,13 @@
 	if (nblk == 0) nblk = 1;
 	size_t rpb = (R + nblk - 1) / nblk;
 	u32 *hcnt, *hstart;
-	HIP_TRY(db.alloc(&hcnt, NBH));
+	static_assert(BZ_HCNT == 1u << 15, "hb_max");
+	if (bz) hcnt = bz->hcnt;
+	else {
+		HIP_TRY(db.alloc(&hcnt, NBH));
+		clear16_async(st, hcnt, (size_t) NBH * 4);
+	}
 	HIP_TRY(db.alloc(&hstart, NBH + 1));
-	HIP_TRY(hipMemsetAsync(hcnt, 0, (size_t) NBH * 4, st));
 	const bool lng = pool->W > 2;
 	const size_t lds_hist = (size_t) NBH * 4 + (HIST_THREADS / 64) * (lng ? GL_WAVE_BYTES_LONG : GL_WAVE_BYTES);
 	HIP_TRY(hipFuncSetAttribute((const void*) k_gated_hist<false>, hipFuncAttributeMaxDynamicSharedMemorySize, (int) lds_hist));
@@ -2096,9 +2136,10 @@
 }
 
 template <typename TUP, typename A>
-int stage_gated_partition(vdjx_ctx* c, A& db, const vdjx_pool* pool, u64 rec_base, int k, size_t per_bucket, u64 geometry_instances, GTuples<TUP>* out, bool sym = false) {
+int stage_gated_partition(vdjx_ctx* c, A& db, const vdjx_pool* pool, u64 rec_base, int k, size_t per_bucket, u64 geometry_instances, GTuples<TUP>* out, bool sym = false,
+                          const BuildZeros* bz = nullptr) {
 	GatedHist gh;
-	int rc = stage_gated_hist(c, db, pool, k, per_bucket, geometry_instances, &gh, sym);
+	int rc = stage_gated_hist(c, db, pool, k, per_bucket, geometry_instances, &gh, sym, bz);
 	if (rc) return rc;
 	return stage_gated_cut<TUP>(c, db, pool, rec_base, k, per_bucket, geometry_instances, gh, out);
 }
@@ -2121,7 +2162,8 @@
 }
 
 template <typename TUP, typename A>
-int stage_gated_reduce(vdjx_ctx* c, A& db, const GTuples<TUP>& t, const PoolView& pv, u64 rec_base, int k, int mf, int mq, SurvivorsG* sv, bool sym = false) {
+int stage_gated_reduce(vdjx_ctx* c, A& db, const GTuples<TUP>& t, const PoolView& pv, u64 rec_base, int k, int mf, int mq, SurvivorsG* sv, bool sym = false,
+                       const BuildZeros* bz = nullptr) {
 	hipStream_t st = c->stream;
 	int rc = set_sub_tuples(c);
 	if (rc) return rc;
@@ -2134,11 +2176,14 @@
 	u32 *g_err, *n_surv;
 	u64* g_distinct;
 	HIP_TRY(db.alloc(&sv->lo, cap)); HIP_TRY(db.alloc(&sv->hi, cap)); HIP_TRY(db.alloc(&sv->gcnt, cap)); HIP_TRY(db.alloc(&sv->gfirst, cap));
-	HIP_TRY(db.alloc(&g_distinct, 64 * 16 + 2));
+	if (bz) g_distinct = bz->distinct;
+	else {
+		HIP_TRY(db.alloc(&g_distinct, BZ_DISTINCT));
+		clear16_async(st, g_distinct, BZ_DISTINCT * 8);
+	}
 	g_err = (u32*) (g_distinct + 64 * 16);
 	n_surv = g_err + 1;
 	u32* n_real = g_err + 2;
-	HIP_TRY(hipMemsetAsync(g_distinct, 0, (64 * 16 + 2) * 8, st));
 	SurvOutG so{sv->lo, sv->hi, sv->gcnt, sv->gfirst, n_surv, cap, n_real};
 	static const u32 rd_dbg = (u32) vdjx_env_num("VDJX_RD_DBG", 0, 0, 9);
 	if (t.N) {
@@ -2181,7 +2226,7 @@
 
 template <typename A>
 int stage_recount(vdjx_ctx* c, A& db, const vdjx_pool* pool, u64 rec_base, int k, SurvivorsG& sv, const RecountOut& ro,
-                  bool derive_edges, SurvTable* table_out = nullptr, RecountStatus* defer = nullptr, bool sym_walk = false) {
+                  bool derive_edges, SurvTable* table_out = nullptr, RecountStatus* defer = nullptr, bool sym_walk = false, const BuildZeros* bz = nullptr) {
 	hipStream_t st = c->stream;
 	const size_t R = pool->n_records;
 	const int P = pool->rl - k + 1;
@@ -2199,22 +2244,28 @@
 	u32 bloom_bits = 1u << 16;
 	while (bloom_bits < (1u << 30) && (size_t) bloom_bits < (size_t) ns * 16) bloom_bits <<= 1;
 	const u32 nb16 = (ns + 15u) >> 4;
-	const u32 n_jump = (ceil_log2_u64((u64) ns + 1) + 4) / 5 + 1;
+	const u32 n_jump = (ceil_log2_u64((u64) ns + 1) + 4) / 5;
 	{
 		auto up = [](size_t b) { return (b + 255) & ~(size_t) 255; };
-		const size_t b_bloom = up(bloom_bits / 8), b_table = up(((size_t) tmask + 1) * 16), b_pred = up((size_t) ns * 8), b_clen = up((size_t) ns * 4),
-		             b_jump = up((size_t) (n_jump + 1) * 4), b_linw = up(((size_t) nb16 + 1) * 8);
+		const size_t b_bloom = up(bloom_bits / 8), b_table = up(((size_t) tmask + 1) * 16), b_jump = up((size_t) (n_jump + 1) * 4);
 		uint8_t* z;
-		const size_t zb = b_bloom + b_table + b_pred + b_clen + b_jump + b_linw;
+		const size_t zb = b_bloom + b_table + b_jump;
 		HIP_TRY(db.alloc(&z, zb));
-		HIP_TRY(hipMemsetAsync(z, 0, zb, st));
+		clear16_async(st, z, zb);
 		table = (ulonglong2*) z; z += b_table;
 		bloom = (u32*) z; z += b_bloom;
-		pred = (unsigned long long*) z; z += b_pred;
-		clen = (u32*) z; z += b_clen;
-		jump_open = (u32*) z; z += b_jump;
-		linw = (u64*) z;
-	}
+		jump_open = (u32*) z;
+	}
+	HIP_TRY(db.alloc(&pred, ns)); HIP_TRY(db.alloc(&clen, ns));
+	HIP_TRY(db.alloc(&linw, (size_t) nb16 + 1));
+	unsigned long long* g_cursor = bz ? bz->cursor : nullptr;
+	if (!g_cursor) {
+		HIP_TRY(db.alloc(&g_cursor, BZ_CURSOR));
+		clear16_async(st, g_cursor, BZ_CURSOR * 8);
+	}
+	unsigned long long* const n_inst = g_cursor + 1;
+	u32* const g_err = (u32*) (g_cursor + 2);
+	u32* const range_cnt = (u32*) (g_cursor + 4);
 	HIP_TRY(db.alloc(&skey0, ns)); HIP_TRY(db.alloc(&skey, ns));
 	HIP_TRY(db.alloc(&succ0, (size_t) ns * 4)); HIP_TRY(db.alloc(&succ, (size_t) ns * 4));
 	HIP_TRY(db.alloc(&pd, ns)); HIP_TRY(db.alloc(&coff, (size_t) ns + 1)); HIP_TRY(db.alloc(&newidx, ns));
@@ -2228,7 +2279,7 @@
 	const dim3 gs((ns + 255) / 256), bs(256);
 	{
 		vdjx_prof_scope ps(c, "k_surv_table");
-		hipLaunchKernelGGL(k_surv_table2, gs, bs, 0, st, sv.lo, sv.hi, ns, table, tmask, skey0, bloom, bloom_bits - 1);
+		hipLaunchKernelGGL(k_surv_table2, gs, bs, 0, st, sv.lo, sv.hi, ns, table, tmask, skey0, bloom, bloom_bits - 1, pred, clen);
 		hipLaunchKernelGGL(k_succ_links2, gs, bs, 0, st, tb0, ns, k, sv.gcnt, succ0, pred, bestsucc);
 	}
 	{
@@ -2238,10 +2289,10 @@
 		hipLaunchKernelGGL(k_chain_len, gs, bs, 0, st, pd, ns, clen);
 		{ const int rc_ = vdjx_scan_wide(db, st, clen, ns, coff); if (rc_) return rc_; }
 		hipLaunchKernelGGL(k_chain_place, gs, bs, 0, st, pd, coff, ns, newidx);
-		hipLaunchKernelGGL(k_chain_permute, gs, bs, 0, st, newidx, ns, sv.lo, sv.hi, sv.gcnt, sv.gfirst, succ0, lo2, hi2, gcnt2, gfirst2, skey, succ);
-		hipLaunchKernelGGL(k_table_remap, dim3(tmask / 256 + 1), bs, 0, st, table, tmask + 1, newidx);
+		hipLaunchKernelGGL(k_chain_permute, dim3(tmask / 256 + 1), bs, 0, st, newidx, ns, sv.lo, sv.hi, sv.gcnt, sv.gfirst, succ0, lo2, hi2, gcnt2, gfirst2, skey, succ,
+		                   table, tmask + 1);
 		if (sym_walk) hipLaunchKernelGGL(k_partner, gs, bs, 0, st, tb, ns, k, partner);
-		hipLaunchKernelGGL(k_chain_words, gs, bs, 0, st, succ, skey, ns, k, linw, fbw, (const u32*) partner);
+		hipLaunchKernelGGL(k_chain_words, gs, bs, 0, st, succ, skey, ns, k, linw, fbw, (const u32*) partner, g_err + 3);
 	}
 	dbg_sync(c, "k_chain_order");
 	if (sync_debug()) {
@@ -2306,24 +2357,15 @@
 	while (blk_items > 256 && nwaves * blk_items > NI / 2 + 65536) blk_items >>= 1;
 	const u64 raw_cap = (u64) NI + (u64) NI / (blk_items / 64) + nwaves * (u64) blk_items + blk_items;
 	u64 *raw, *items;
-	unsigned long long *g_cursor, *n_inst;
-	u32 *range_cnt, *range_start, *g_err, *gcur;
+	u32 *range_start, *gcur;
+	if (n_ranges_p > RC_RANGES_MAX) { vdjx_set_error("too many survivor ranges for the walk histogram"); return VDJX_ELIMIT; }
 	const vdjx_arena::mark_t tmp_mark = db.mark();
 	HIP_TRY(db.alloc(&raw, (size_t) raw_cap));
-	HIP_TRY(db.alloc(&g_cursor, 4 + ((size_t) n_ranges_p + 1) / 2));
-	n_inst = g_cursor + 1;
-	g_err = (u32*) (g_cursor + 2);
-	range_cnt = (u32*) (g_cursor + 4);
 	HIP_TRY(db.alloc(&range_start, n_ranges_p + 1));
-	HIP_TRY(hipMemsetAsync(g_cursor, 0, 32 + (size_t) n_ranges_p * 4, st));
-	if (sym_walk) {
-		vdjx_prof_scope ps(c, "k_chain_order");
-		hipLaunchKernelGGL(k_partner_check, gs, bs, 0, st, partner, linw, ns, g_err + 3);
-	}
 	const bool lng = pool->W > 2;
 	if (lng && R >= (1ull << 27)) { vdjx_set_error("more than 2^27 records of long reads on one GPU: not supported by the recount items"); return VDJX_ELIMIT; }
 	const size_t lds_walk = (((size_t) n_ranges_p + 1) & ~(size_t) 1) * 4 + (lng ? (size_t) WALK_THREADS * GL_ROW_LONG * 8 : 0);
-	if ((size_t) n_ranges_p * 4 > 64 * 1024) { vdjx_set_error("too many survivor ranges for the walk histogram"); return VDJX_ELIMIT; }
+	static_assert(RC_RANGES_MAX * 4 == 64 * 1024, "the walk's range histogram in LDS");
 	HIP_TRY(hipFuncSetAttribute((const void*) k_walk_items<false>, hipFuncAttributeMaxDynamicSharedMemorySize, (int) lds_walk));
 	HIP_TRY(hipFuncSetAttribute((const void*) k_walk_items<true>, hipFuncAttributeMaxDynamicSharedMemorySize, (int) lds_walk));
 	HIP_TRY(hipFuncSetAttribute((const void*) k_walk_items<false, true>, hipFuncAttributeMaxDynamicSharedMemorySize, (int) lds_walk));
@@ -2418,8 +2460,7 @@
 	}
 	dbg_sync(c, "k_recount");
 	if (derive_edges) {
-		hipLaunchKernelGGL(k_count_unseen, dim3((ns + 255) / 256), dim3(256), 0, st, ro.ufirst, ns, g_err + 1);
-		HIP_TRY(hipMemsetAsync(ro.edge_first, 0xFF, (size_t) ns * 32, st));
+		hipLaunchKernelGGL(k_count_unseen, dim3((ns + 255) / 256), dim3(256), 0, st, ro.ufirst, ns, g_err + 1, ro.edge_first);
 		hipLaunchKernelGGL(k_edges_from_in, dim3((ns * 4 + 255) / 256), dim3(256), 0, st, tb, ns, k, ro.in_first, ro.in_from, ro.edge_first, ro.edge_to);
 	}
 	if (defer && !sync_debug()) {
@@ -2478,10 +2519,6 @@
 	uint8_t *d_hv, *d_hj;
 	HIP_TRY(db.alloc(&d_hv, ns));
 	HIP_TRY(db.alloc(&d_hj, ns));
-	{
-		vdjx_prof_scope ps(c, "k_node_flags");
-		hipLaunchKernelGGL(k_node_flags, dim3((ns + 255) / 256), dim3(256), 0, st, sv.lo, sv.hi, ns, k, c->d_vbits, c->d_jbits, d_hv, d_hj);
-	}
 	u64 *rk_key, *rk_key2;
 	u32 *rk_idx, *rk_idx2, *rank;
 	HIP_TRY(db.alloc(&rk_key, ns));
@@ -2489,6 +2526,11 @@
 	HIP_TRY(db.alloc(&rk_idx, ns));
 	HIP_TRY(db.alloc(&rk_idx2, ns));
 	HIP_TRY(db.alloc(&rank, ns));
+	{
+		vdjx_prof_scope ps(c, "k_node_flags");
+		hipLaunchKernelGGL(k_node_flags, dim3((ns + 255) / 256), dim3(256), 0, st, sv.lo, sv.hi, ns, k, c->d_vbits, c->d_jbits, d_hv, d_hj,
+		                   sv.ufirst, sv.gcnt, rk_key, rk_idx);
+	}
 	unsigned rk_bits = 1;
 	while (rk_bits < 64 && (1ull << rk_bits) <= ((n_records_total << ob) | 1ull)) rk_bits++;
 	auto up = [](size_t b) { return (b + 255) & ~(size_t) 255; };
@@ -2515,7 +2557,6 @@
 	g->d_roots = (u32*) carve((size_t) ns * 4);
 	{
 		vdjx_prof_scope ps(c, "k_node_order");
-		hipLaunchKernelGGL(k_rank_keys, dim3((ns + 255) / 256), dim3(256), 0, st, sv.ufirst, sv.gcnt, ns, rk_key, rk_idx);
 		{
 			size_t tb = 0;
 			int rc_ = vdjx_sort_pairs_raw(nullptr, &tb, st, rk_key, rk_key2, rk_idx, rk_idx2, ns, rk_bits);
@@ -2555,11 +2596,14 @@
 	GTuples<TUP> t;
 	const bool sym = build_sym(pool, k);
 	c->stats["kmer_build_sym"] = sym ? 1 : 0;
-	int rc = stage_gated_partition<TUP>(c, db, pool, 0, k, 0, 0, &t, sym);
+	BuildZeros bz;
+	int rc = build_zeros_alloc(c, db, &bz);
+	if (rc) return rc;
+	rc = stage_gated_partition<TUP>(c, db, pool, 0, k, 0, 0, &t, sym, &bz);
 	if (rc) return rc;
 	PoolView pv{pool->d_bases, pool->d_nmask, vdjx_qrows{pool->d_quals, pool->d_quals2, pool->q_split, pool->qstride}, pool->rl, pool->ob};
 	SurvivorsG sv;
-	rc = stage_gated_reduce<TUP>(c, db, t, pv, 0, k, mf, mq, &sv, sym);
+	rc = stage_gated_reduce<TUP>(c, db, t, pv, 0, k, mf, mq, &sv, sym, &bz);
 	if (rc) return rc;
 	vdjx_ri_open_gate(c);
 	dbg_sync(c, "gated_reduce");
@@ -2574,7 +2618,7 @@
 			const bool sym_walk = sym && sym_walk_wanted() && attempt == 0;
 			c->stats["kmer_build_sym_walk"] = sym_walk ? 1 : 0;
 			RecountStatus rs;
-			rc = stage_recount(c, db, pool, 0, k, sv, ro, true, nullptr, &rs, sym_walk);
+			rc = stage_recount(c, db, pool, 0, k, sv, ro, true, nullptr, &rs, sym_walk, attempt == 0 ? &bz : nullptr);
 			if (rc == VDJX_ESYMWALK && sym_walk) { c->stats["kmer_build_sym_walk_retries"] += 1; continue; }
 			if (rc) return rc;
 			u32* hp = (u32*) c->h_pin + 1024;
@@ -3103,7 +3147,7 @@
 		HIP_TRY(db.alloc(&ro.in_from, (size_t) a.n * 4));
 		HIP_TRY(db.alloc(&ro.edge_first, (size_t) a.n * 4));
 		HIP_TRY(db.alloc(&ro.edge_to, (size_t) a.n * 4));
-		HIP_TRY(hipMemsetAsync(ro.edge_first, 0xFF, (size_t) a.n * 32, c->stream));
+		clear16_async(c->stream, ro.edge_first, (size_t) a.n * 32, 0xFFFFFFFFu);
 		hipLaunchKernelGGL(k_edges_from_in, dim3((a.n * 4 + 255) / 256), dim3(256), 0, c->stream, s->tb, a.n, s->k, ro.in_first, ro.in_from, ro.edge_first, ro.edge_to);
 	}
 	vdjx_graph* g = new vdjx_graph();
```

Result: no change. 923.7 (median of 3 runs) (+0.8%).
